# codex-storage/nim-groth16

Hardware: AMD Instinct MI355X
Metric: proofs/sec (BN254 Groth16, 2^20-constraint circuit) (higher is better)
Workload: dtype u32 (254-bit Montgomery: 8x32-bit limbs; 9x29-bit limbs in the bucket accumulation); 1 GPU; BN254 2^20-constraint synthetic R1CS (squaring chain, m=2^20-2), full prove: buildABC + 6 NTT + 4 G1 MSM + 1 G2 MSM, snarkjs flavour, 1 proof/step/GPU (3 proofs in flight per GPU, one shared key); mode=replica, nvars=1048576, domain_log2=20

## Files before the change

include/g16hip.h:

```cpp
#ifndef G16HIP_H
#define G16HIP_H

#include <stddef.h>
#include <stdint.h>

#ifdef __cplusplus
extern "C" {
#endif

#define G16_OK 0
#define G16_EINVAL (-1)
#define G16_ENODEV (-2)
#define G16_EHIP (-3)
#define G16_ENOMEM (-4)
#define G16_ESELFTEST (-5)

typedef struct g16_ctx g16_ctx;
typedef struct g16_points g16_points;

#define G16_SCALARS_MONT 1u
#define G16_SCALARS_STD 0u
#define G16_SCALARS_DEVICE 2u
#define G16_OUT_PARTIAL 4u
#define G16_OUT_DEVICE 8u
#define G16_NO_HOST_SYNC 32u

int32_t g16_ctx_create(int32_t device, g16_ctx** out);
void g16_ctx_destroy(g16_ctx* ctx);
const char* g16_last_error(const g16_ctx* ctx);
int32_t g16_ctx_set_stream(g16_ctx* ctx, void* hip_stream);
int32_t g16_ctx_synchronize(g16_ctx* ctx);
int32_t g16_ctx_cancel(g16_ctx* ctx);
int32_t g16_selftest(g16_ctx* ctx);

int32_t g16_msm_g1(g16_ctx* ctx, const void* scalars, uint32_t scalar_flags, const void* points, size_t n,
                   void* out_affine);
int32_t g16_msm_g2(g16_ctx* ctx, const void* scalars, uint32_t scalar_flags, const void* points, size_t n,
                   void* out_affine);
int32_t g16_msm_g1_dev(g16_ctx* ctx, const void* d_scalars, uint32_t scalar_flags, const void* d_points, size_t n,
                       void* out_affine);
int32_t g16_msm_g2_dev(g16_ctx* ctx, const void* d_scalars, uint32_t scalar_flags, const void* d_points, size_t n,
                       void* out_affine);
int32_t g16_msm_g1_partial_dev(g16_ctx* ctx, const void* d_scalars, uint32_t scalar_flags, const void* d_points,
                               size_t n, void* out_xyzz);
int32_t g16_msm_g2_partial_dev(g16_ctx* ctx, const void* d_scalars, uint32_t scalar_flags, const void* d_points,
                               size_t n, void* out_xyzz);
int32_t g16_g1_sum_partials(g16_ctx* ctx, const void* xyzz, size_t count, void* out_affine);
int32_t g16_g2_sum_partials(g16_ctx* ctx, const void* xyzz, size_t count, void* out_affine);

int32_t g16_points_register_g1(g16_ctx* ctx, const void* points, size_t n, g16_points** out);
int32_t g16_points_register_g2(g16_ctx* ctx, const void* points, size_t n, g16_points** out);
int32_t g16_points_register_g1_dev(g16_ctx* ctx, const void* d_points, size_t n, g16_points** out);
int32_t g16_points_register_g2_dev(g16_ctx* ctx, const void* d_points, size_t n, g16_points** out);
void g16_points_release(g16_points* pts);
size_t g16_points_count(const g16_points* pts);
size_t g16_points_inf_count(const g16_points* pts);
int32_t g16_points_info(const g16_points* pts, uint32_t* window_bits, uint32_t* ntables);

int32_t g16_points_register_g1_lean(g16_ctx* ctx, const void* points, size_t n, uint32_t table_stride, g16_points** out);
int32_t g16_points_register_g2_lean(g16_ctx* ctx, const void* points, size_t n, uint32_t table_stride, g16_points** out);
int32_t g16_points_register_g1_lean_dev(g16_ctx* ctx, const void* d_points, size_t n, uint32_t table_stride,
                                        g16_points** out);
int32_t g16_points_register_g2_lean_dev(g16_ctx* ctx, const void* d_points, size_t n, uint32_t table_stride,
                                        g16_points** out);
int32_t g16_points_table_bytes(const g16_points* pts, size_t* bytes);
int32_t g16_points_plan(int group, size_t n, uint32_t table_stride, uint32_t* window_bits, uint32_t* ntables,
                        size_t* bytes);
int32_t g16_msm_points(g16_ctx* ctx, const g16_points* pts, const void* scalars, uint32_t flags, void* out);

int32_t g16_points_check_g1(g16_ctx* ctx, const void* points, size_t n, size_t* first_bad);
int32_t g16_points_check_g2(g16_ctx* ctx, const void* points, size_t n, size_t* first_bad);

int32_t g16_fixed_base_g1(g16_ctx* ctx, const void* scalars, uint32_t scalar_flags, size_t n, void* out_points);
int32_t g16_fixed_base_g2(g16_ctx* ctx, const void* scalars, uint32_t scalar_flags, size_t n, void* out_points);

typedef struct {
  uint32_t nvars, npubs, nconstraints;
  uint32_t flavour;
  const uint32_t* row[3];
  const uint32_t* col[3];
  const void* val[3];
  size_t nnz[3];
  uint32_t flags;
  const void *alpha, *beta, *gamma, *delta, *tau;
} g16_setup_desc;
typedef struct {
  void *alpha1, *beta1, *delta1;
  void *beta2, *gamma2, *delta2;
  void* pointsIC;
  void *pointsA1, *pointsB1;
  void* pointsB2;
  void* pointsC1;
  void* pointsH1;
} g16_setup_points;
int32_t g16_setup_log2_domain(const g16_setup_desc* desc, uint32_t* log2_domain);
int32_t g16_fake_setup(g16_ctx* ctx, const g16_setup_desc* desc, g16_setup_points* out);
int32_t g16_lagrange_fr(g16_ctx* ctx, uint32_t log2n, uint32_t first, uint32_t step, size_t count, const void* tau,
                        const void* scale, void* out);
int32_t g16_powers_fr(g16_ctx* ctx, const void* base, const void* scale, size_t count, void* out);

typedef struct g16_r1cs_desc_s g16_r1cs_desc;
typedef struct g16_ptau_desc_s g16_ptau_desc;
int32_t g16_points_intt_g1(g16_ctx* ctx, const void* points, uint32_t log2n, void* out);
int32_t g16_points_intt_g2(g16_ctx* ctx, const void* points, uint32_t log2n, void* out);
int32_t g16_circuit_setup(g16_ctx* ctx, const g16_r1cs_desc* r1cs, const g16_ptau_desc* ptau, const void* delta,
                          g16_setup_points* out);

int32_t g16_ntt_fr(g16_ctx* ctx, const void* src, void* dst, uint32_t log2n, int32_t inverse);
int32_t g16_ntt_fr_dev(g16_ctx* ctx, const void* d_src, void* d_dst, uint32_t log2n, int32_t inverse);

#define G16_FLAVOUR_JENSGROTH 0u
#define G16_FLAVOUR_SNARKJS 1u
int32_t g16_quotient(g16_ctx* ctx, const void* Az, const void* Bz, const void* Cz, uint32_t log2n, uint32_t flavour,
                     void* out);
int32_t g16_quotient_dev(g16_ctx* ctx, const void* d_Az, const void* d_Bz, const void* d_Cz, uint32_t log2n,
                         uint32_t flavour, void* d_out);

typedef struct g16_pkey g16_pkey;
typedef struct {
  uint32_t matrix;
  uint32_t row;
  uint32_t col;
  uint32_t reserved;
  uint8_t value[32];
} g16_coeff;
typedef struct {
  uint32_t nvars, npubs;
  uint32_t log2_domain;
  uint32_t flavour;
  const void *pointsA1, *pointsB1;
  const void* pointsB2;
  const void* pointsC1;
  const void* pointsH1;
  const g16_coeff* coeffs;
  size_t ncoeffs;
  const void *alpha1, *beta1, *delta1;
  const void *beta2, *delta2;
  uint32_t shard_index, shard_count;
} g16_pkey_desc;
typedef struct {
  uint8_t pi_a[64];
  uint8_t pi_b[128];
  uint8_t pi_c[64];
} g16_proof;
int32_t g16_pkey_create(g16_ctx* ctx, const g16_pkey_desc* desc, g16_pkey** out);
int32_t g16_pkey_create_zkey(g16_ctx* ctx, const g16_pkey_desc* desc, const void* section4, size_t section4_bytes,
                             g16_pkey** out);
int32_t g16_pkey_create_lean(g16_ctx* ctx, const g16_pkey_desc* desc, uint32_t table_stride, g16_pkey** out);
int32_t g16_pkey_create_zkey_lean(g16_ctx* ctx, const g16_pkey_desc* desc, const void* section4, size_t section4_bytes,
                                  uint32_t table_stride, g16_pkey** out);
void g16_pkey_destroy(g16_pkey* key);
int32_t g16_pkey_inf_counts(const g16_pkey* key, size_t out[8]);
int32_t g16_pkey_b1_fold(const g16_pkey* key, size_t out[3]);
int32_t g16_pkey_b1_sparse(const g16_pkey* key, size_t out[3]);
int32_t g16_prove(g16_ctx* ctx, const g16_pkey* key, const void* witness, uint32_t flags, const void* mask_r,
                  const void* mask_s, g16_proof* out);
#define G16_PARTIALS_BYTES 768
int32_t g16_prove_partials(g16_ctx* ctx, const g16_pkey* key, const void* witness, uint32_t flags, void* out_partials);
int32_t g16_prove_combine(g16_ctx* ctx, const g16_pkey* key, const void* partials, size_t count, uint32_t flags,
                          const void* mask_r, const void* mask_s, g16_proof* out);
int32_t g16_prove_partials_begin(g16_ctx* ctx, const g16_pkey* key, const void* witness, uint32_t flags,
                                 uint32_t task_mask, void* d_task_out);
int32_t g16_prove_partials_end(g16_ctx* ctx, const g16_pkey* key, const void* d_a1_slice, const void* d_b1_slice,
                               const void* d_c1_slice, uint32_t flags, void* out_partials);
int32_t g16_build_abc(g16_ctx* ctx, const g16_pkey* key, const void* witness, uint32_t flags, void* out_abc);
int32_t g16_pkey_abc_info(const g16_pkey* key, size_t out[11]);
int32_t g16_spmv_fr(g16_ctx* ctx, const uint32_t* row, const uint32_t* col, const void* val, size_t nnz, const void* x,
                    size_t ncols, size_t nrows, void* y);

typedef struct g16_group g16_group;
typedef struct g16_group_pkey g16_group_pkey;
int32_t g16_group_create(const int32_t* devices, int32_t ndev, g16_group** out);
void g16_group_destroy(g16_group* group);
int32_t g16_group_size(const g16_group* group);
const char* g16_group_last_error(const g16_group* group);
int32_t g16_group_pkey_create(g16_group* group, const g16_pkey_desc* desc, g16_group_pkey** out);
int32_t g16_group_pkey_create_lean(g16_group* group, const g16_pkey_desc* desc, uint32_t table_stride,
                                   g16_group_pkey** out);
void g16_group_pkey_destroy(g16_group_pkey* key);
int32_t g16_group_prove(g16_group* group, const g16_group_pkey* key, const void* witness, uint32_t flags,
                        const void* mask_r, const void* mask_s, g16_proof* out);

#define G16_EBUSY (-6)
typedef struct g16_prover g16_prover;
int32_t g16_prover_create(int32_t device, const g16_pkey* key, uint32_t depth, g16_prover** out);
void g16_prover_destroy(g16_prover* p);
const char* g16_prover_last_error(const g16_prover* p);
int32_t g16_prover_submit(g16_prover* p, const void* witness, uint32_t flags, const void* mask_r, const void* mask_s,
                          uint64_t* ticket);
int32_t g16_prover_poll(g16_prover* p, uint64_t ticket);
int32_t g16_prover_collect(g16_prover* p, uint64_t ticket, g16_proof* out);
int32_t g16_host_alloc(int32_t device, size_t bytes, void** out);
void g16_host_free(void* p);

typedef struct g16_vkey g16_vkey;
typedef struct {
  uint32_t npubs;
  const void* alpha1;
  const void* beta2;
  const void* gamma2;
  const void* delta2;
  const void* pointsIC;
} g16_vkey_desc;
#define G16_VERIFY_SUBGROUP 16u
#define G16_GT_BYTES 384
int32_t g16_vkey_create(g16_ctx* ctx, const g16_vkey_desc* desc, g16_vkey** out);
void g16_vkey_destroy(g16_vkey* key);
int32_t g16_verify(g16_ctx* ctx, const g16_vkey* key, const g16_proof* proofs, const void* public_io, uint32_t flags,
                   size_t count, int32_t* status);
int32_t g16_pairing(g16_ctx* ctx, const void* g1_points, const void* g2_points, size_t n, void* out_gt);
int32_t g16_verify_batch(g16_ctx* ctx, const g16_vkey* key, const g16_proof* proofs, const void* public_io,
                         uint32_t flags, size_t count, const void* multipliers, int32_t* result, int32_t* status);

int32_t g16_points_audit_g1(g16_ctx* ctx, const void* points, size_t n, size_t first_bad[3], size_t bad_count[3]);
int32_t g16_points_audit_g2(g16_ctx* ctx, const void* points, size_t n, size_t first_bad[3], size_t bad_count[3]);
int32_t g16_points_pairs_check(g16_ctx* ctx, const void* g1_points, const void* g2_points, size_t n,
                               const void* multipliers, int32_t* result);
#define G16_AUDIT_SECTIONS 13
enum {
  G16_SEC_ALPHA1 = 0, G16_SEC_BETA1, G16_SEC_DELTA1, G16_SEC_BETA2, G16_SEC_GAMMA2, G16_SEC_DELTA2, G16_SEC_POINTS_IC,
  G16_SEC_POINTS_A1, G16_SEC_POINTS_B1, G16_SEC_POINTS_B2, G16_SEC_POINTS_C1, G16_SEC_POINTS_H1, G16_SEC_COEFFS
};
#define G16_AUDIT_CANONICAL 1u
#define G16_AUDIT_CURVE 2u
#define G16_AUDIT_SUBGROUP 4u
#define G16_AUDIT_RELATION 8u
#define G16_AUDIT_SPEC_INFINITY 16u
typedef struct {
  uint32_t failed;
  uint32_t spec_infinity;
  int32_t relation[3];
  uint32_t reserved;
  size_t first_bad[G16_AUDIT_SECTIONS][3];
  size_t bad_count[G16_AUDIT_SECTIONS][3];
} g16_key_report;
int32_t g16_key_audit(g16_ctx* ctx, const g16_pkey_desc* desc, const g16_vkey_desc* vk, const void* section4,
                      size_t section4_bytes, const void* multipliers, g16_key_report* out);

struct g16_r1cs_desc_s {
  uint32_t nvars, npubs, nconstraints;
  uint32_t flavour;
  const uint32_t* row[3];
  const uint32_t* col[3];
  const void* val[3];
  size_t nnz[3];
  uint32_t flags;
};
struct g16_ptau_desc_s {
  uint32_t power;
  const void *tauG1, *tauG2, *alphaTauG1, *betaTauG1, *betaG2;
};
#define G16_PTAU_SECTIONS 5
#define G16_CIRCUIT_RELATIONS 9
enum {
  G16_PTAU_TAU_G1 = 0, G16_PTAU_TAU_G2, G16_PTAU_ALPHA_TAU_G1, G16_PTAU_BETA_TAU_G1, G16_PTAU_BETA_G2
};
enum {
  G16_REL_COEFFS_A = 0, G16_REL_COEFFS_B, G16_REL_SPEC, G16_REL_A1, G16_REL_B1, G16_REL_B2, G16_REL_C1, G16_REL_IC,
  G16_REL_H1
};
#define G16_CIRCUIT_KEY 1u
#define G16_CIRCUIT_PTAU 2u
#define G16_CIRCUIT_COEFFS 4u
#define G16_CIRCUIT_SPEC 8u
#define G16_CIRCUIT_POINTS 16u
typedef struct {
  g16_key_report key;
  size_t ptau_first_bad[G16_PTAU_SECTIONS][3];
  size_t ptau_bad_count[G16_PTAU_SECTIONS][3];
  int32_t relation[G16_CIRCUIT_RELATIONS];
  uint32_t failed;
  size_t first_row[2];
} g16_circuit_report;
int32_t g16_circuit_audit(g16_ctx* ctx, const g16_pkey_desc* desc, const g16_vkey_desc* vk, const void* section4,
                          size_t section4_bytes, const g16_r1cs_desc* r1cs, const g16_ptau_desc* ptau,
                          const void* wire_multipliers, const void* h_multipliers, g16_circuit_report* out);

typedef struct g16_r1cs g16_r1cs;
int32_t g16_r1cs_create(g16_ctx* ctx, const g16_r1cs_desc* desc, g16_r1cs** out);
void g16_r1cs_destroy(g16_r1cs* r);
int32_t g16_r1cs_info(const g16_r1cs* r, size_t out[4]);

#define G16_WITNESS_CANONICAL 1u
#define G16_WITNESS_ONE 2u
#define G16_WITNESS_CONSTRAINTS 4u
#define G16_WITNESS_LIST 16
typedef struct {
  uint32_t failed;
  int32_t constraints;
  size_t noncanonical_count, first_noncanonical;
  size_t bad_count;
  size_t first_bad[G16_WITNESS_LIST];
  uint8_t az[32], bz[32], cz[32];
} g16_witness_report;
int32_t g16_witness_check(g16_ctx* ctx, const g16_r1cs* r, const void* witness, uint32_t flags, g16_witness_report* out);

int32_t g16_points_scale_g1(g16_ctx* ctx, const void* points, size_t n, const void* k, uint32_t flags, void* out);
int32_t g16_points_scale_g2(g16_ctx* ctx, const void* points, size_t n, const void* k, uint32_t flags, void* out);
int32_t g16_points_scale_each_g1(g16_ctx* ctx, const void* points, size_t n, const void* scalars, uint32_t flags,
                                 void* out);
int32_t g16_points_scale_each_g2(g16_ctx* ctx, const void* points, size_t n, const void* scalars, uint32_t flags,
                                 void* out);

typedef struct {
  const void *delta1, *delta2;
  const void *pointsC1, *pointsH1;
  size_t nc1, nh1;
} g16_phase2_key;
typedef struct {
  uint8_t delta_after[64];
  uint8_t g1_s[64], g1_sx[64];
  uint8_t g2_spx[128];
} g16_contribution;
typedef struct {
  void *delta1, *delta2, *pointsC1, *pointsH1;
  g16_contribution* record;
} g16_phase2_out;
int32_t g16_key_contribute(g16_ctx* ctx, const g16_phase2_key* key, const void* d, const void* s, uint32_t flags,
                           const void* challenge_g2, g16_phase2_out* out);

#define G16_CHAIN_ARRAYS 9
enum {
  G16_CHAIN_DELTA_AFTER = 0, G16_CHAIN_G1_S, G16_CHAIN_G1_SX, G16_CHAIN_G2_SPX, G16_CHAIN_CHALLENGES,
  G16_CHAIN_FINAL_DELTA1, G16_CHAIN_FINAL_DELTA2, G16_CHAIN_FINAL_POINTS_C1, G16_CHAIN_FINAL_POINTS_H1
};
#define G16_CHAIN_RELATIONS 7
enum {
  G16_CHAIN_ELEMENTS = 0, G16_CHAIN_POK, G16_CHAIN_STEP, G16_CHAIN_LAST, G16_CHAIN_DELTA, G16_CHAIN_C1, G16_CHAIN_H1
};
typedef struct {
  uint32_t failed;
  int32_t relation[G16_CHAIN_RELATIONS];
  size_t first_record[2];
  size_t first_bad[G16_CHAIN_ARRAYS][3];
  size_t bad_count[G16_CHAIN_ARRAYS][3];
  size_t first_infinity[G16_CHAIN_ARRAYS];
} g16_chain_report;
int32_t g16_contributions_verify(g16_ctx* ctx, const g16_phase2_key* initial, const g16_phase2_key* final_,
                                 const g16_contribution* records, const void* challenges_g2, size_t count,
                                 const void* c1_multipliers, const void* h1_multipliers, g16_chain_report* out);

typedef struct {
  void *tauG1, *tauG2, *alphaTauG1, *betaTauG1, *betaG2;
} g16_ptau_out;
typedef struct {
  uint8_t g1_s[64], g1_sx[64], g2_spx[128];
} g16_ptau_pok;
typedef struct {
  uint8_t tauG1[64], alphaG1[64], betaG1[64];
  uint8_t tauG2[128], betaG2[128];
  g16_ptau_pok pok[3];
} g16_ptau_contribution;
int32_t g16_ptau_contribute(g16_ctx* ctx, const g16_ptau_desc* ptau, const void* t, const void* a, const void* b,
                            const void* s3, uint32_t flags, const void* challenges_g2, g16_ptau_out* out,
                            g16_ptau_contribution* record);

#define G16_PTAU_REPORT_ARRAYS 14
enum {
  G16_PTAUV_REC_TAU_G1 = 5, G16_PTAUV_REC_ALPHA_G1, G16_PTAUV_REC_BETA_G1, G16_PTAUV_REC_TAU_G2, G16_PTAUV_REC_BETA_G2,
  G16_PTAUV_G1_S, G16_PTAUV_G1_SX, G16_PTAUV_G2_SPX, G16_PTAUV_CHALLENGES
};
#define G16_PTAU_RELATIONS 10
enum {
  G16_PTAUV_ELEMENTS = 0, G16_PTAUV_FIRST, G16_PTAUV_TAU_G1, G16_PTAUV_TAU_G2, G16_PTAUV_ALPHA, G16_PTAUV_BETA,
  G16_PTAUV_BETA_G2, G16_PTAUV_POK, G16_PTAUV_STEP, G16_PTAUV_LAST
};
typedef struct {
  uint32_t failed;
  int32_t relation[G16_PTAU_RELATIONS];
  size_t first_record[2];
  size_t first_bad[G16_PTAU_REPORT_ARRAYS][3];
  size_t bad_count[G16_PTAU_REPORT_ARRAYS][3];
  size_t first_infinity[G16_PTAU_REPORT_ARRAYS];
} g16_ptau_report;
int32_t g16_ptau_verify(g16_ctx* ctx, const g16_ptau_desc* ptau, const g16_ptau_contribution* records,
                        const void* challenges_g2, size_t count, const void* multipliers, g16_ptau_report* out);

int32_t g16_profile_enable(g16_ctx* ctx, int32_t on);
int32_t g16_profile_reset(g16_ctx* ctx);
int32_t g16_profile_report(g16_ctx* ctx, char* buf, size_t buflen);
int32_t g16_profile_clock(g16_ctx* ctx, double* ghz);

#ifdef __cplusplus
}
#endif
#endif
```

nim_groth16_amd/_lib.py:

```python
from __future__ import annotations

import ctypes
import json
import os
import weakref

_HERE = os.path.dirname(os.path.abspath(__file__))

_R = 21888242871839275222246405745257275088548364400416034343698204186575808495617
G16_OK, G16_EINVAL, G16_ENODEV, G16_EHIP, G16_ENOMEM, G16_ESELFTEST, G16_EBUSY = 0, -1, -2, -3, -4, -5, -6
SCALARS_MONT, SCALARS_STD, SCALARS_DEVICE, OUT_PARTIAL, OUT_DEVICE, NO_HOST_SYNC = 1, 0, 2, 4, 8, 32
PARTIALS_BYTES = 768

SYMBOLS = [
    "g16_ctx_create", "g16_ctx_destroy", "g16_last_error", "g16_ctx_set_stream", "g16_ctx_synchronize",
    "g16_selftest", "g16_msm_g1", "g16_msm_g2", "g16_msm_g1_dev", "g16_msm_g2_dev",
    "g16_msm_g1_partial_dev", "g16_msm_g2_partial_dev", "g16_g1_sum_partials", "g16_g2_sum_partials",
    "g16_points_register_g1", "g16_points_register_g2", "g16_points_register_g1_dev",
    "g16_points_register_g2_dev", "g16_points_release", "g16_points_count", "g16_points_inf_count", "g16_points_info", "g16_msm_points",
    "g16_points_check_g1", "g16_points_check_g2", "g16_fixed_base_g1", "g16_fixed_base_g2", "g16_quotient", "g16_quotient_dev", "g16_pkey_create",
    "g16_pkey_create_zkey", "g16_pkey_destroy", "g16_pkey_inf_counts", "g16_prove", "g16_build_abc", "g16_pkey_abc_info", "g16_spmv_fr", "g16_prove_partials", "g16_prove_combine",
    "g16_prove_partials_begin", "g16_prove_partials_end",
    "g16_ntt_fr", "g16_ntt_fr_dev", "g16_profile_enable", "g16_profile_reset", "g16_profile_report", "g16_profile_clock",
    "g16_vkey_create", "g16_vkey_destroy", "g16_verify", "g16_verify_batch", "g16_pairing",
    "g16_ctx_cancel", "g16_group_create", "g16_group_destroy", "g16_group_size", "g16_group_last_error",
    "g16_group_pkey_create", "g16_group_pkey_destroy", "g16_group_prove",
    "g16_prover_create", "g16_prover_destroy", "g16_prover_last_error", "g16_prover_submit", "g16_prover_poll",
    "g16_prover_collect", "g16_host_alloc", "g16_host_free",
    "g16_points_register_g1_lean", "g16_points_register_g2_lean", "g16_points_register_g1_lean_dev",
    "g16_points_register_g2_lean_dev", "g16_points_table_bytes", "g16_points_plan", "g16_pkey_create_lean",
    "g16_pkey_create_zkey_lean", "g16_group_pkey_create_lean",
    "g16_setup_log2_domain", "g16_fake_setup", "g16_lagrange_fr", "g16_powers_fr",
    "g16_points_audit_g1", "g16_points_audit_g2", "g16_points_pairs_check", "g16_key_audit",
    "g16_pkey_b1_fold", "g16_pkey_b1_sparse", "g16_circuit_audit",
    "g16_points_intt_g1", "g16_points_intt_g2", "g16_circuit_setup",
    "g16_points_scale_g1", "g16_points_scale_g2", "g16_points_scale_each_g1", "g16_points_scale_each_g2",
    "g16_key_contribute", "g16_contributions_verify", "g16_ptau_contribute", "g16_ptau_verify",
    "g16_r1cs_create", "g16_r1cs_destroy", "g16_r1cs_info", "g16_witness_check",
]
VERIFY_SUBGROUP = 16
GT_BYTES = 384


class PkeyDesc(ctypes.Structure):
    _fields_ = [("nvars", ctypes.c_uint32), ("npubs", ctypes.c_uint32), ("log2_domain", ctypes.c_uint32),
                ("flavour", ctypes.c_uint32),
                ("pointsA1", ctypes.c_void_p), ("pointsB1", ctypes.c_void_p), ("pointsB2", ctypes.c_void_p),
                ("pointsC1", ctypes.c_void_p), ("pointsH1", ctypes.c_void_p),
                ("coeffs", ctypes.c_void_p), ("ncoeffs", ctypes.c_size_t),
                ("alpha1", ctypes.c_void_p), ("beta1", ctypes.c_void_p), ("delta1", ctypes.c_void_p),
                ("beta2", ctypes.c_void_p), ("delta2", ctypes.c_void_p),
                ("shard_index", ctypes.c_uint32), ("shard_count", ctypes.c_uint32)]


class VkeyDesc(ctypes.Structure):
    _fields_ = [("npubs", ctypes.c_uint32), ("alpha1", ctypes.c_void_p), ("beta2", ctypes.c_void_p),
                ("gamma2", ctypes.c_void_p), ("delta2", ctypes.c_void_p), ("pointsIC", ctypes.c_void_p)]


class SetupDesc(ctypes.Structure):
    _fields_ = [("nvars", ctypes.c_uint32), ("npubs", ctypes.c_uint32), ("nconstraints", ctypes.c_uint32),
                ("flavour", ctypes.c_uint32),
                ("row", ctypes.c_void_p * 3), ("col", ctypes.c_void_p * 3), ("val", ctypes.c_void_p * 3),
                ("nnz", ctypes.c_size_t * 3), ("flags", ctypes.c_uint32),
                ("alpha", ctypes.c_void_p), ("beta", ctypes.c_void_p), ("gamma", ctypes.c_void_p),
                ("delta", ctypes.c_void_p), ("tau", ctypes.c_void_p)]


SETUP_POINTS = ("alpha1", "beta1", "delta1", "beta2", "gamma2", "delta2", "pointsIC", "pointsA1", "pointsB1", "pointsB2",
                "pointsC1", "pointsH1")


class SetupPoints(ctypes.Structure):
    _fields_ = [(name, ctypes.c_void_p) for name in SETUP_POINTS]


AUDIT_SECTIONS = ("alpha1", "beta1", "delta1", "beta2", "gamma2", "delta2", "pointsIC", "pointsA1", "pointsB1", "pointsB2",
                  "pointsC1", "pointsH1", "coeffs")
AUDIT_CHECKS = ("canonical", "curve", "subgroup")
AUDIT_RELATIONS = ("pointsB1~pointsB2", "beta1~beta2", "delta1~delta2")
AUDIT_CANONICAL, AUDIT_CURVE, AUDIT_SUBGROUP, AUDIT_RELATION, AUDIT_SPEC_INFINITY = 1, 2, 4, 8, 16
CHECK_TEXTS = ("is not a canonical encoding", "is not on the curve", "is not in the order-r subgroup")


def _element_findings(names, first_bad, bad_count, first_infinity=None, prefix=""):
    out = []
    for a, name in enumerate(names):
        for k, what in enumerate(CHECK_TEXTS):
            if bad_count[a][k]:
                more = bad_count[a][k] - 1
                out.append(f"{prefix}{name}[{first_bad[a][k]}] {what}" + (f" (and {more} more)" if more else ""))
        if first_infinity is not None and first_infinity[a] is not None:
            out.append(f"{prefix}{name}[{first_infinity[a]}] is the point at infinity")
    return out


class KeyReportC(ctypes.Structure):
    _fields_ = [("failed", ctypes.c_uint32), ("spec_infinity", ctypes.c_uint32), ("relation", ctypes.c_int32 * 3),
                ("reserved", ctypes.c_uint32),
                ("first_bad", (ctypes.c_size_t * 3) * len(AUDIT_SECTIONS)),
                ("bad_count", (ctypes.c_size_t * 3) * len(AUDIT_SECTIONS))]


class KeyReport:

    def __init__(self, failed, spec_infinity, relation, first_bad, bad_count):
        self.failed, self.spec_infinity, self.relation = failed, spec_infinity, list(relation)
        self.first_bad, self.bad_count = first_bad, bad_count

    @property
    def ok(self) -> bool:
        return self.failed == 0

    def as_dict(self) -> dict:
        return {"failed": self.failed, "spec_infinity": self.spec_infinity, "relation": self.relation,
                "first_bad": self.first_bad, "bad_count": self.bad_count}

    def findings(self):
        out = _element_findings(AUDIT_SECTIONS, self.first_bad, self.bad_count)
        for k, name in enumerate(AUDIT_RELATIONS):
            if self.relation[k] == 0:
                out.append(f"{name}: not the same multiples of the two generators")
        for s in range(6):
            if self.spec_infinity >> s & 1:
                out.append(f"{AUDIT_SECTIONS[s]} is the point at infinity")
        return out

    def __str__(self):
        if self.ok:
            skipped = [AUDIT_RELATIONS[k] for k in range(3) if self.relation[k] < 0]
            return "key audit: ok" + (f" (not run: {', '.join(skipped)})" if skipped else "")
        return "key audit: FAILED\n" + "\n".join("  " + f for f in self.findings())


class R1csDesc(ctypes.Structure):
    _fields_ = [("nvars", ctypes.c_uint32), ("npubs", ctypes.c_uint32), ("nconstraints", ctypes.c_uint32),
                ("flavour", ctypes.c_uint32),
                ("row", ctypes.c_void_p * 3), ("col", ctypes.c_void_p * 3), ("val", ctypes.c_void_p * 3),
                ("nnz", ctypes.c_size_t * 3), ("flags", ctypes.c_uint32)]


class PtauDesc(ctypes.Structure):
    _fields_ = [("power", ctypes.c_uint32), ("tauG1", ctypes.c_void_p), ("tauG2", ctypes.c_void_p),
                ("alphaTauG1", ctypes.c_void_p), ("betaTauG1", ctypes.c_void_p), ("betaG2", ctypes.c_void_p)]


PTAU_SECTIONS = ("tauG1", "tauG2", "alphaTauG1", "betaTauG1", "betaG2")
PTAU_GROUP = {"tauG1": 1, "tauG2": 2, "alphaTauG1": 1, "betaTauG1": 1, "betaG2": 2}
CIRCUIT_RELATIONS = ("COEFFS_A", "COEFFS_B", "SPEC", "A1", "B1", "B2", "C1", "IC", "H1")
CIRCUIT_KEY, CIRCUIT_PTAU, CIRCUIT_COEFFS, CIRCUIT_SPEC, CIRCUIT_POINTS = 1, 2, 4, 8, 16


class CircuitReportC(ctypes.Structure):
    _fields_ = [("key", KeyReportC),
                ("ptau_first_bad", (ctypes.c_size_t * 3) * len(PTAU_SECTIONS)),
                ("ptau_bad_count", (ctypes.c_size_t * 3) * len(PTAU_SECTIONS)),
                ("relation", ctypes.c_int32 * len(CIRCUIT_RELATIONS)), ("failed", ctypes.c_uint32),
                ("first_row", ctypes.c_size_t * 2)]


class CircuitReport:

    def __init__(self, key: KeyReport, ptau_first_bad, ptau_bad_count, relation, failed, first_row):
        self.key, self.ptau_first_bad, self.ptau_bad_count = key, ptau_first_bad, ptau_bad_count
        self.relation, self.failed, self.first_row = list(relation), failed, list(first_row)

    @property
    def ok(self) -> bool:
        return self.failed == 0

    def as_dict(self) -> dict:
        return {"key": self.key.as_dict(), "ptau_first_bad": self.ptau_first_bad, "ptau_bad_count": self.ptau_bad_count,
                "relation": self.relation, "failed": self.failed, "first_row": self.first_row}

    def findings(self):
        out = self.key.findings() + _element_findings(PTAU_SECTIONS, self.ptau_first_bad, self.ptau_bad_count, prefix="ptau ")
        for m in range(2):
            if self.relation[m] == 0:
                out.append(f"coeffs: matrix {'AB'[m]} differs from the r1cs first at row {self.first_row[m]}")
        if self.relation[2] == 0:
            out.append("alpha1 / beta1 / beta2 are not those of the powers of tau (or its first powers are not the generators)")
        for k in range(3, len(CIRCUIT_RELATIONS)):
            if self.relation[k] == 0:
                out.append(f"points{CIRCUIT_RELATIONS[k]} does not belong to the circuit")
        return out

    def __str__(self):
        if self.ok:
            skipped = [AUDIT_RELATIONS[k] for k in range(3) if self.key.relation[k] < 0]
            skipped += [CIRCUIT_RELATIONS[k] for k in range(len(CIRCUIT_RELATIONS)) if self.relation[k] < 0]
            return "circuit audit: ok" + (f" (not run: {', '.join(skipped)})" if skipped else "")
        return "circuit audit: FAILED\n" + "\n".join("  " + f for f in self.findings())


WITNESS_CANONICAL, WITNESS_ONE, WITNESS_CONSTRAINTS = 1, 2, 4
WITNESS_LIST = 16


class WitnessReportC(ctypes.Structure):
    _fields_ = [("failed", ctypes.c_uint32), ("constraints", ctypes.c_int32),
                ("noncanonical_count", ctypes.c_size_t), ("first_noncanonical", ctypes.c_size_t),
                ("bad_count", ctypes.c_size_t), ("first_bad", ctypes.c_size_t * WITNESS_LIST),
                ("az", ctypes.c_uint8 * 32), ("bz", ctypes.c_uint8 * 32), ("cz", ctypes.c_uint8 * 32)]


class WitnessReport:

    def __init__(self, failed, constraints, noncanonical_count, first_noncanonical, bad_count, first_bad, az, bz, cz):
        self.failed, self.constraints = failed, constraints
        self.noncanonical_count, self.first_noncanonical = noncanonical_count, first_noncanonical
        self.bad_count, self.first_bad = bad_count, list(first_bad)
        self.az, self.bz, self.cz = az, bz, cz

    @property
    def ok(self) -> bool:
        return self.failed == 0

    def as_dict(self) -> dict:
        return {"failed": self.failed, "constraints": self.constraints, "noncanonical_count": self.noncanonical_count,
                "first_noncanonical": self.first_noncanonical, "bad_count": self.bad_count, "first_bad": self.first_bad,
                "az": self.az, "bz": self.bz, "cz": self.cz}

    def findings(self):
        out = []
        if self.noncanonical_count:
            more = self.noncanonical_count - 1
            out.append(f"witness[{self.first_noncanonical}] is not canonical (>= r)" + (f" (and {more} more)" if more else ""))
        if self.failed & WITNESS_ONE:
            out.append("witness[0] is not 1")
        if self.bad_count:
            ab = self.az * self.bz % _R
            out.append(f"constraint {self.first_bad[0]}: (A z)(B z) = {ab:#x}, C z = {self.cz:#x}")
            rest = self.first_bad[1:]
            if rest:
                more = self.bad_count - len(self.first_bad)
                out.append("also failing: constraints " + ", ".join(map(str, rest)) + (f" (and {more} more)" if more else ""))
        return out

    def __str__(self):
        if self.ok:
            return "witness check: ok"
        return "witness check: FAILED\n" + "\n".join("  " + f for f in self.findings())


class Phase2Key(ctypes.Structure):
    _fields_ = [("delta1", ctypes.c_void_p), ("delta2", ctypes.c_void_p), ("pointsC1", ctypes.c_void_p),
                ("pointsH1", ctypes.c_void_p), ("nc1", ctypes.c_size_t), ("nh1", ctypes.c_size_t)]


class ContributionC(ctypes.Structure):
    _fields_ = [("delta_after", ctypes.c_uint8 * 64), ("g1_s", ctypes.c_uint8 * 64), ("g1_sx", ctypes.c_uint8 * 64),
                ("g2_spx", ctypes.c_uint8 * 128)]


CONTRIBUTION_BYTES = 320
assert ctypes.sizeof(ContributionC) == CONTRIBUTION_BYTES


class Phase2Out(ctypes.Structure):
    _fields_ = [("delta1", ctypes.c_void_p), ("delta2", ctypes.c_void_p), ("pointsC1", ctypes.c_void_p),
                ("pointsH1", ctypes.c_void_p), ("record", ctypes.POINTER(ContributionC))]


class PtauOut(ctypes.Structure):
    _fields_ = [(name, ctypes.c_void_p) for name in PTAU_SECTIONS]


class PtauPokC(ctypes.Structure):
    _fields_ = [("g1_s", ctypes.c_uint8 * 64), ("g1_sx", ctypes.c_uint8 * 64), ("g2_spx", ctypes.c_uint8 * 128)]


class PtauContributionC(ctypes.Structure):
    _fields_ = [("tauG1", ctypes.c_uint8 * 64), ("alphaG1", ctypes.c_uint8 * 64), ("betaG1", ctypes.c_uint8 * 64),
                ("tauG2", ctypes.c_uint8 * 128), ("betaG2", ctypes.c_uint8 * 128), ("pok", PtauPokC * 3)]


PTAU_CONTRIBUTION_BYTES = 1216
assert ctypes.sizeof(PtauContributionC) == PTAU_CONTRIBUTION_BYTES


PTAU_REPORT_ARRAYS = PTAU_SECTIONS + ("record tauG1", "record alphaG1", "record betaG1", "record tauG2", "record betaG2",
                                      "g1_s", "g1_sx", "g2_spx", "challenges")
PTAU_RELATIONS = ("ELEMENTS", "FIRST", "TAU_G1", "TAU_G2", "ALPHA", "BETA", "BETA_G2", "POK", "STEP", "LAST")


class PtauReportC(ctypes.Structure):
    _fields_ = [("failed", ctypes.c_uint32), ("relation", ctypes.c_int32 * len(PTAU_RELATIONS)),
                ("first_record", ctypes.c_size_t * 2),
                ("first_bad", (ctypes.c_size_t * 3) * len(PTAU_REPORT_ARRAYS)),
                ("bad_count", (ctypes.c_size_t * 3) * len(PTAU_REPORT_ARRAYS)),
                ("first_infinity", ctypes.c_size_t * len(PTAU_REPORT_ARRAYS))]


class PtauReport:

    def __init__(self, failed, relation, first_record, first_bad, bad_count, first_infinity):
        self.failed, self.relation, self.first_record = failed, list(relation), list(first_record)
        self.first_bad, self.bad_count, self.first_infinity = first_bad, bad_count, list(first_infinity)

    @property
    def ok(self) -> bool:
        return self.failed == 0

    def as_dict(self) -> dict:
        return {"failed": self.failed, "relation": self.relation, "first_record": self.first_record,
                "first_bad": self.first_bad, "bad_count": self.bad_count, "first_infinity": self.first_infinity}

    def findings(self):
        out = _element_findings(PTAU_REPORT_ARRAYS, self.first_bad, self.bad_count, self.first_infinity)
        for k, name in enumerate(PTAU_RELATIONS):
            if k and self.relation[k] == 0:
                rec = f" (first at record {self.first_record[k - 7]})" if name in ("POK", "STEP") else ""
                out.append(f"{name} fails{rec}")
        return out

    def __str__(self):
        rel = "  ".join(f"{n} {'ok' if v == 1 else 'FAILS' if v == 0 else 'not run'}" for n, v in zip(PTAU_RELATIONS, self.relation))
        return rel + "".join("\n  " + f for f in self.findings())


CHAIN_ARRAYS = ("delta_after", "g1_s", "g1_sx", "g2_spx", "challenges", "final delta1", "final delta2", "final pointsC1",
                "final pointsH1")
CHAIN_RELATIONS = ("ELEMENTS", "POK", "STEP", "LAST", "DELTA", "C1", "H1")


class ChainReportC(ctypes.Structure):
    _fields_ = [("failed", ctypes.c_uint32), ("relation", ctypes.c_int32 * len(CHAIN_RELATIONS)),
                ("first_record", ctypes.c_size_t * 2),
                ("first_bad", (ctypes.c_size_t * 3) * len(CHAIN_ARRAYS)),
                ("bad_count", (ctypes.c_size_t * 3) * len(CHAIN_ARRAYS)),
                ("first_infinity", ctypes.c_size_t * len(CHAIN_ARRAYS))]


class ChainReport:

    def __init__(self, failed, relation, first_record, first_bad, bad_count, first_infinity, transcript=None):
        self.failed, self.relation, self.first_record = failed, list(relation), list(first_record)
        self.first_bad, self.bad_count, self.first_infinity = first_bad, bad_count, list(first_infinity)
        self.transcript = transcript

    @property
    def ok(self) -> bool:
        return self.failed == 0 and self.transcript != 0

    def as_dict(self) -> dict:
        return {"failed": self.failed, "relation": self.relation, "first_record": self.first_record,
                "first_bad": self.first_bad, "bad_count": self.bad_count, "first_infinity": self.first_infinity,
                "transcript": self.transcript}

    def findings(self):
        out = []
        if self.transcript == 0:
            out.append("the transcript hashes are not those of the initial key and the records")
        out += _element_findings(CHAIN_ARRAYS, self.first_bad, self.bad_count, self.first_infinity)
        if self.relation[1] == 0:
            out.append(f"record {self.first_record[0]}: the proof of knowledge does not hold")
        if self.relation[2] == 0:
            out.append(f"record {self.first_record[1]}: delta_after is not the contribution's multiple of the delta before")
        if self.relation[3] == 0:
            out.append("the final delta1 is not the last record's delta_after")
        if self.relation[4] == 0:
            out.append("the final delta1 / delta2 are not the same multiple of the two generators")
        for k in (5, 6):
            if self.relation[k] == 0:
                out.append(f"the final points{CHAIN_RELATIONS[k]} is not the initial one rescaled by the deltas")
        return out

    def __str__(self):
        if self.ok:
            skipped = [CHAIN_RELATIONS[k] for k in range(len(CHAIN_RELATIONS)) if self.relation[k] < 0]
            return "contribution chain: ok" + (f" (not run: {', '.join(skipped)})" if skipped else "")
        return "contribution chain: FAILED\n" + "\n".join("  " + f for f in self.findings())


class G16Error(RuntimeError):
    def __init__(self, code, msg):
        super().__init__(f"g16hip error {code}: {msg}")
        self.code = code


def lib_path() -> str:
    return os.environ.get("G16HIP_LIB", os.path.join(_HERE, "csrc", "libg16hip.so"))


def device_code_sha16(path: str = None) -> str:
    import hashlib
    import struct
    b = open(path or lib_path(), "rb").read()
    h = hashlib.sha256()
    try:
        assert b[:4] == b"\x7fELF" and b[4] == 2
        shoff = struct.unpack_from("<Q", b, 0x28)[0]
        shentsize, shnum, shstrndx = struct.unpack_from("<HHH", b, 0x3A)

        def sh(i):
            name, _typ, _flags, _addr, off, size = struct.unpack_from("<IIQQQQ", b, shoff + i * shentsize)
            return name, off, size
        _, stro, _ = sh(shstrndx)
        hit = False
        for i in range(shnum):
            n, off, size = sh(i)
            if b[stro + n: b.index(b"\0", stro + n)] == b".hip_fatbin":
                h.update(b[off: off + size])
                hit = True
        assert hit
    except Exception:
        h = hashlib.sha256(b)
    return h.hexdigest()[:16]


_lib = None


def load_library():
    global _lib
    if _lib is not None:
        return _lib
    path = lib_path()
    if not os.path.exists(path):
        raise G16Error(G16_ENODEV, f"{path} not found: build it with `make -C nim_groth16_amd/csrc` "
                                   "(or __graft_entry__.build()); there is no CPU fallback")
    try:
        import torch
    except ImportError:
        pass
    lib = ctypes.CDLL(path)
    vp, u32, i32, sz = ctypes.c_void_p, ctypes.c_uint32, ctypes.c_int32, ctypes.c_size_t
    lib.g16_ctx_create.argtypes = [i32, ctypes.POINTER(vp)]
    lib.g16_ctx_destroy.argtypes = [vp]
    lib.g16_ctx_destroy.restype = None
    lib.g16_last_error.argtypes = [vp]
    lib.g16_last_error.restype = ctypes.c_char_p
    lib.g16_ctx_set_stream.argtypes = [vp, vp]
    lib.g16_ctx_synchronize.argtypes = [vp]
    lib.g16_selftest.argtypes = [vp]
    for name in ("g16_msm_g1", "g16_msm_g2", "g16_msm_g1_dev", "g16_msm_g2_dev",
                 "g16_msm_g1_partial_dev", "g16_msm_g2_partial_dev"):
        getattr(lib, name).argtypes = [vp, vp, u32, vp, sz, vp]
    for name in ("g16_g1_sum_partials", "g16_g2_sum_partials"):
        getattr(lib, name).argtypes = [vp, vp, sz, vp]
    for name in ("g16_points_register_g1", "g16_points_register_g2", "g16_points_register_g1_dev",
                 "g16_points_register_g2_dev"):
        getattr(lib, name).argtypes = [vp, vp, sz, ctypes.POINTER(vp)]
    for name in ("g16_points_register_g1_lean", "g16_points_register_g2_lean", "g16_points_register_g1_lean_dev",
                 "g16_points_register_g2_lean_dev"):
        getattr(lib, name).argtypes = [vp, vp, sz, u32, ctypes.POINTER(vp)]
    lib.g16_points_table_bytes.argtypes = [vp, ctypes.POINTER(sz)]
    lib.g16_points_plan.argtypes = [ctypes.c_int, sz, u32, ctypes.POINTER(u32), ctypes.POINTER(u32), ctypes.POINTER(sz)]
    lib.g16_pkey_create_lean.argtypes = [vp, ctypes.POINTER(PkeyDesc), u32, ctypes.POINTER(vp)]
    lib.g16_pkey_create_zkey_lean.argtypes = [vp, ctypes.POINTER(PkeyDesc), vp, sz, u32, ctypes.POINTER(vp)]
    lib.g16_group_pkey_create_lean.argtypes = [vp, ctypes.POINTER(PkeyDesc), u32, ctypes.POINTER(vp)]
    lib.g16_points_release.argtypes = [vp]
    lib.g16_points_release.restype = None
    lib.g16_points_count.argtypes = [vp]
    lib.g16_points_count.restype = sz
    lib.g16_points_inf_count.argtypes = [vp]
    lib.g16_points_inf_count.restype = sz
    lib.g16_pkey_inf_counts.argtypes = [vp, ctypes.POINTER(sz)]
    lib.g16_pkey_b1_fold.argtypes = [vp, ctypes.POINTER(sz)]
    lib.g16_pkey_b1_sparse.argtypes = [vp, ctypes.POINTER(sz)]
    lib.g16_points_info.argtypes = [vp, ctypes.POINTER(u32), ctypes.POINTER(u32)]
    lib.g16_msm_points.argtypes = [vp, vp, vp, u32, vp]
    lib.g16_points_check_g1.argtypes = [vp, vp, sz, ctypes.POINTER(sz)]
    lib.g16_points_check_g2.argtypes = [vp, vp, sz, ctypes.POINTER(sz)]
    lib.g16_fixed_base_g1.argtypes = [vp, vp, u32, sz, vp]
    lib.g16_fixed_base_g2.argtypes = [vp, vp, u32, sz, vp]
    lib.g16_quotient.argtypes = [vp, vp, vp, vp, u32, u32, vp]
    lib.g16_quotient_dev.argtypes = [vp, vp, vp, vp, u32, u32, vp]
    lib.g16_pkey_create.argtypes = [vp, ctypes.POINTER(PkeyDesc), ctypes.POINTER(vp)]
    lib.g16_pkey_create_zkey.argtypes = [vp, ctypes.POINTER(PkeyDesc), vp, sz, ctypes.POINTER(vp)]
    lib.g16_pkey_destroy.argtypes = [vp]
    lib.g16_pkey_destroy.restype = None
    lib.g16_prove.argtypes = [vp, vp, vp, u32, vp, vp, vp]
    lib.g16_build_abc.argtypes = [vp, vp, vp, u32, vp]
    lib.g16_pkey_abc_info.argtypes = [vp, ctypes.POINTER(sz)]
    lib.g16_spmv_fr.argtypes = [vp, vp, vp, vp, sz, vp, sz, sz, vp]
    lib.g16_prove_partials.argtypes = [vp, vp, vp, u32, vp]
    lib.g16_prove_combine.argtypes = [vp, vp, vp, sz, u32, vp, vp, vp]
    lib.g16_prove_partials_begin.argtypes = [vp, vp, vp, u32, u32, vp]
    lib.g16_prove_partials_end.argtypes = [vp, vp, vp, vp, vp, u32, vp]
    lib.g16_ntt_fr.argtypes = [vp, vp, vp, u32, i32]
    lib.g16_ntt_fr_dev.argtypes = [vp, vp, vp, u32, i32]
    lib.g16_vkey_create.argtypes = [vp, ctypes.POINTER(VkeyDesc), ctypes.POINTER(vp)]
    lib.g16_vkey_destroy.argtypes = [vp]
    lib.g16_vkey_destroy.restype = None
    lib.g16_verify.argtypes = [vp, vp, vp, vp, u32, sz, ctypes.POINTER(i32)]
    lib.g16_verify_batch.argtypes = [vp, vp, vp, vp, u32, sz, vp, ctypes.POINTER(i32), ctypes.POINTER(i32)]
    lib.g16_pairing.argtypes = [vp, vp, vp, sz, vp]
    lib.g16_ctx_cancel.argtypes = [vp]
    lib.g16_group_create.argtypes = [ctypes.POINTER(i32), i32, ctypes.POINTER(vp)]
    lib.g16_group_destroy.argtypes = [vp]
    lib.g16_group_destroy.restype = None
    lib.g16_group_size.argtypes = [vp]
    lib.g16_group_last_error.argtypes = [vp]
    lib.g16_group_last_error.restype = ctypes.c_char_p
    lib.g16_group_pkey_create.argtypes = [vp, ctypes.POINTER(PkeyDesc), ctypes.POINTER(vp)]
    lib.g16_group_pkey_destroy.argtypes = [vp]
    lib.g16_group_pkey_destroy.restype = None
    lib.g16_group_prove.argtypes = [vp, vp, vp, u32, vp, vp, vp]
    lib.g16_prover_create.argtypes = [i32, vp, u32, ctypes.POINTER(vp)]
    lib.g16_prover_destroy.argtypes = [vp]
    lib.g16_prover_destroy.restype = None
    lib.g16_prover_last_error.argtypes = [vp]
    lib.g16_prover_last_error.restype = ctypes.c_char_p
    lib.g16_prover_submit.argtypes = [vp, vp, u32, vp, vp, ctypes.POINTER(ctypes.c_uint64)]
    lib.g16_prover_poll.argtypes = [vp, ctypes.c_uint64]
    lib.g16_prover_collect.argtypes = [vp, ctypes.c_uint64, vp]
    lib.g16_host_alloc.argtypes = [i32, sz, ctypes.POINTER(vp)]
    lib.g16_host_free.argtypes = [vp]
    lib.g16_host_free.restype = None
    lib.g16_profile_enable.argtypes = [vp, i32]
    lib.g16_profile_reset.argtypes = [vp]
    lib.g16_profile_report.argtypes = [vp, ctypes.c_char_p, sz]
    lib.g16_profile_clock.argtypes = [vp, ctypes.POINTER(ctypes.c_double)]
    lib.g16_setup_log2_domain.argtypes = [ctypes.POINTER(SetupDesc), ctypes.POINTER(u32)]
    lib.g16_fake_setup.argtypes = [vp, ctypes.POINTER(SetupDesc), ctypes.POINTER(SetupPoints)]
    lib.g16_lagrange_fr.argtypes = [vp, u32, u32, u32, sz, vp, vp, vp]
    lib.g16_powers_fr.argtypes = [vp, vp, vp, sz, vp]
    lib.g16_points_audit_g1.argtypes = [vp, vp, sz, ctypes.POINTER(sz), ctypes.POINTER(sz)]
    lib.g16_points_audit_g2.argtypes = [vp, vp, sz, ctypes.POINTER(sz), ctypes.POINTER(sz)]
    lib.g16_points_pairs_check.argtypes = [vp, vp, vp, sz, vp, ctypes.POINTER(i32)]
    lib.g16_key_audit.argtypes = [vp, ctypes.POINTER(PkeyDesc), ctypes.POINTER(VkeyDesc), vp, sz, vp,
                                  ctypes.POINTER(KeyReportC)]
    lib.g16_circuit_audit.argtypes = [vp, ctypes.POINTER(PkeyDesc), ctypes.POINTER(VkeyDesc), vp, sz,
                                      ctypes.POINTER(R1csDesc), ctypes.POINTER(PtauDesc), vp, vp,
                                      ctypes.POINTER(CircuitReportC)]
    lib.g16_points_intt_g1.argtypes = [vp, vp, u32, vp]
    lib.g16_points_intt_g2.argtypes = [vp, vp, u32, vp]
    lib.g16_circuit_setup.argtypes = [vp, ctypes.POINTER(R1csDesc), ctypes.POINTER(PtauDesc), vp,
                                      ctypes.POINTER(SetupPoints)]
    lib.g16_points_scale_g1.argtypes = [vp, vp, sz, vp, u32, vp]
    lib.g16_points_scale_g2.argtypes = [vp, vp, sz, vp, u32, vp]
    lib.g16_points_scale_each_g1.argtypes = [vp, vp, sz, vp, u32, vp]
    lib.g16_points_scale_each_g2.argtypes = [vp, vp, sz, vp, u32, vp]
    lib.g16_key_contribute.argtypes = [vp, ctypes.POINTER(Phase2Key), vp, vp, u32, vp, ctypes.POINTER(Phase2Out)]
    lib.g16_contributions_verify.argtypes = [vp, ctypes.POINTER(Phase2Key), ctypes.POINTER(Phase2Key),
                                             ctypes.POINTER(ContributionC), vp, sz, vp, vp, ctypes.POINTER(ChainReportC)]
    lib.g16_ptau_contribute.argtypes = [vp, ctypes.POINTER(PtauDesc), vp, vp, vp, vp, u32, vp, ctypes.POINTER(PtauOut),
                                        ctypes.POINTER(PtauContributionC)]
    lib.g16_ptau_verify.argtypes = [vp, ctypes.POINTER(PtauDesc), ctypes.POINTER(PtauContributionC), vp, sz, vp,
                                    ctypes.POINTER(PtauReportC)]
    lib.g16_r1cs_create.argtypes = [vp, ctypes.POINTER(R1csDesc), ctypes.POINTER(vp)]
    lib.g16_r1cs_destroy.argtypes = [vp]
    lib.g16_r1cs_destroy.restype = None
    lib.g16_r1cs_info.argtypes = [vp, ctypes.POINTER(sz)]
    lib.g16_witness_check.argtypes = [vp, vp, vp, u32, ctypes.POINTER(WitnessReportC)]
    for name in SYMBOLS:
        if name not in ("g16_ctx_destroy", "g16_r1cs_destroy", "g16_last_error", "g16_points_release", "g16_points_count",
                        "g16_points_inf_count",
                        "g16_pkey_destroy", "g16_vkey_destroy", "g16_group_destroy", "g16_group_last_error",
                        "g16_group_pkey_destroy", "g16_prover_destroy", "g16_prover_last_error", "g16_host_free"):
            getattr(lib, name).restype = i32
    _lib = lib
    return lib


def _buf(b):
    if isinstance(b, int):
        return ctypes.c_void_p(b)
    if isinstance(b, (bytes, bytearray)):
        return ctypes.cast(ctypes.c_char_p(bytes(b)), ctypes.c_void_p) if isinstance(b, bytes) else \
            ctypes.cast((ctypes.c_char * len(b)).from_buffer(b), ctypes.c_void_p)
    if hasattr(b, "ctypes"):
        return ctypes.c_void_p(b.ctypes.data)
    raise TypeError(type(b))


class Context:

    def __init__(self, device: int = 0):
        self._lib = load_library()
        h = ctypes.c_void_p()
        rc = self._lib.g16_ctx_create(device, ctypes.byref(h))
        if rc != G16_OK:
            raise G16Error(rc, "g16_ctx_create failed (no usable HIP device?)")
        self._h = h
        self.device = device
        self._children = weakref.WeakSet()

    def close(self, release_children: bool = False):
        if getattr(self, "_h", None):
            if release_children:
                for child in list(self._children):
                    child._free()
            self._lib.g16_ctx_destroy(self._h)
            self._h = None

    def __del__(self):
        try:
            self.close()
        except Exception:
            pass

    def _check(self, rc):
        if rc != G16_OK:
            raise G16Error(rc, self._lib.g16_last_error(self._h).decode())

    def selftest(self):
        self._check(self._lib.g16_selftest(self._h))

    def set_stream(self, stream_ptr):
        self._check(self._lib.g16_ctx_set_stream(self._h, ctypes.c_void_p(stream_ptr)))

    def synchronize(self):
        self._check(self._lib.g16_ctx_synchronize(self._h))

    def cancel(self):
        self._check(self._lib.g16_ctx_cancel(self._h))

    def msm(self, group: int, scalars, points, n: int, mont: bool = True, device: bool = False,
            partial: bool = False) -> bytes:
        psz = 64 if group == 1 else 128
        out = ctypes.create_string_buffer(2 * psz if partial else psz)
        if partial:
            fn = self._lib.g16_msm_g1_partial_dev if group == 1 else self._lib.g16_msm_g2_partial_dev
        elif device:
            fn = self._lib.g16_msm_g1_dev if group == 1 else self._lib.g16_msm_g2_dev
        else:
            fn = self._lib.g16_msm_g1 if group == 1 else self._lib.g16_msm_g2
        s = _buf(scalars) if n else None
        p = _buf(points) if n else None
        self._check(fn(self._h, s, SCALARS_MONT if mont else SCALARS_STD, p, n, out))
        return out.raw

    def register_points(self, group: int, points, n: int, device: bool = False, table_stride: int = 0) -> "PointSet":
        h = ctypes.c_void_p()
        p = _buf(points) if n else None
        if table_stride:
            name = f"g16_points_register_g{group}_lean" + ("_dev" if device else "")
            self._check(getattr(self._lib, name)(self._h, p, n, table_stride, ctypes.byref(h)))
        else:
            name = f"g16_points_register_g{group}" + ("_dev" if device else "")
            self._check(getattr(self._lib, name)(self._h, p, n, ctypes.byref(h)))
        return PointSet(self, h, group, n)

    def msm_points(self, pts: "PointSet", scalars, mont: bool = True, device: bool = False,
                   partial: bool = False) -> bytes:
        psz = 64 if pts.group == 1 else 128
        out = ctypes.create_string_buffer(2 * psz if partial else psz)
        flags = (SCALARS_MONT if mont else 0) | (SCALARS_DEVICE if device else 0) | (OUT_PARTIAL if partial else 0)
        self._check(self._lib.g16_msm_points(self._h, pts._h, _buf(scalars) if pts.n else None, flags, out))
        return out.raw

    def points_check(self, group: int, points: bytes):
        psz = 64 if group == 1 else 128
        n = len(points) // psz
        bad = ctypes.c_size_t()
        fn = self._lib.g16_points_check_g1 if group == 1 else self._lib.g16_points_check_g2
        self._check(fn(self._h, _buf(points) if n else None, n, ctypes.byref(bad)))
        return None if bad.value == ctypes.c_size_t(-1).value else bad.value

    def points_audit(self, group: int, points: bytes):
        psz = 64 if group == 1 else 128
        assert len(points) % psz == 0
        n = len(points) // psz
        first, count = (ctypes.c_size_t * 3)(), (ctypes.c_size_t * 3)()
        fn = self._lib.g16_points_audit_g1 if group == 1 else self._lib.g16_points_audit_g2
        self._check(fn(self._h, _buf(points) if n else None, n, first, count))
        none = ctypes.c_size_t(-1).value
        return [None if f == none else f for f in first], list(count)

    def pairs_check(self, g1_points: bytes, g2_points: bytes, multipliers) -> bool:
        n = len(g1_points) // 64
        assert len(g1_points) == 64 * n and len(g2_points) == 128 * n and len(multipliers) == n
        zs = b"".join(int(z).to_bytes(16, "little") for z in multipliers)
        res = ctypes.c_int32(-1)
        self._check(self._lib.g16_points_pairs_check(self._h, _buf(g1_points) if n else None,
                                                     _buf(g2_points) if n else None, n, _buf(zs) if n else None,
                                                     ctypes.byref(res)))
        return res.value == 1

    def key_audit(self, desc: PkeyDesc, vk: VkeyDesc = None, section4: bytes = None, multipliers=None) -> KeyReport:
        zs = None
        if isinstance(multipliers, (bytes, bytearray)):
            assert len(multipliers) == 16 * desc.nvars, "one multiplier per wire"
            zs = bytes(multipliers)
        elif multipliers is not None:
            assert len(multipliers) == desc.nvars, "one multiplier per wire"
            zs = b"".join(int(z).to_bytes(16, "little") for z in multipliers)
        rep = KeyReportC()
        self._check(self._lib.g16_key_audit(self._h, ctypes.byref(desc), ctypes.byref(vk) if vk is not None else None,
                                            _buf(section4) if section4 is not None else None,
                                            len(section4) if section4 is not None else 0,
                                            _buf(zs) if zs is not None else None, ctypes.byref(rep)))
        none = ctypes.c_size_t(-1).value
        return KeyReport(rep.failed, rep.spec_infinity, list(rep.relation),
                         [[None if f == none else f for f in row] for row in rep.first_bad],
                         [list(row) for row in rep.bad_count])

    def circuit_audit(self, desc: PkeyDesc, vk, section4, r1cs: R1csDesc, ptau: PtauDesc, wire_multipliers,
                      h_multipliers) -> CircuitReport:
        def enc(zs, n, what):
            if isinstance(zs, (bytes, bytearray)):
                assert len(zs) == 16 * n, f"one {what} multiplier of 16 bytes each"
                return bytes(zs)
            assert len(zs) == n, f"{n} {what} multipliers"
            return b"".join(int(z).to_bytes(16, "little") for z in zs)
        zw = enc(wire_multipliers, desc.nvars, "wire")
        zh = enc(h_multipliers, 1 << min(desc.log2_domain, 28), "h")
        rep = CircuitReportC()
        self._check(self._lib.g16_circuit_audit(self._h, ctypes.byref(desc), ctypes.byref(vk) if vk is not None else None,
                                                _buf(section4) if section4 is not None else None,
                                                len(section4) if section4 is not None else 0,
                                                ctypes.byref(r1cs), ctypes.byref(ptau), _buf(zw), _buf(zh),
                                                ctypes.byref(rep)))
        none = ctypes.c_size_t(-1).value
        fix = lambda rows: [[None if f == none else f for f in row] for row in rows]
        key = KeyReport(rep.key.failed, rep.key.spec_infinity, list(rep.key.relation), fix(rep.key.first_bad),
                        [list(row) for row in rep.key.bad_count])
        return CircuitReport(key, fix(rep.ptau_first_bad), [list(row) for row in rep.ptau_bad_count], list(rep.relation),
                             rep.failed, [None if f == none else f for f in rep.first_row])

    def r1cs_load(self, desc: R1csDesc, keepalive=None) -> "R1csSystem":
        return R1csSystem(self, desc, keepalive)

    def fixed_base(self, group: int, scalars: bytes, mont: bool = True) -> bytes:
        n = len(scalars) // 32
        psz = 64 if group == 1 else 128
        out = ctypes.create_string_buffer(max(n, 1) * psz)
        fn = self._lib.g16_fixed_base_g1 if group == 1 else self._lib.g16_fixed_base_g2
        self._check(fn(self._h, _buf(scalars) if n else None, SCALARS_MONT if mont else 0, n, out))
        return out.raw[: n * psz]

    def spmv(self, row, col, val, x: bytes, nrows: int) -> bytes:
        import numpy as np
        row = np.ascontiguousarray(row, dtype=np.uint32)
        col = np.ascontiguousarray(col, dtype=np.uint32)
        nnz = len(row)
        if not isinstance(val, (bytes, bytearray)):
            val = np.ascontiguousarray(val, dtype=np.uint8)
        assert len(col) == nnz and (len(val) if isinstance(val, (bytes, bytearray)) else val.size) == 32 * nnz
        out = ctypes.create_string_buffer(max(1, 32 * nrows))
        self._check(self._lib.g16_spmv_fr(self._h, _buf(row) if nnz else None, _buf(col) if nnz else None,
                                          _buf(val) if nnz else None, nnz, _buf(x) if len(x) else None, len(x) // 32,
                                          nrows, out))
        return out.raw[: 32 * nrows]

    def lagrange(self, log2n: int, tau: bytes, first: int = 0, step: int = 1, count: int = None,
                 scale: bytes = None) -> bytes:
        if count is None:
            count = ((1 << log2n) - first + step - 1) // step if step else 1
        out = ctypes.create_string_buffer(max(1, 32 * count))
        self._check(self._lib.g16_lagrange_fr(self._h, log2n, first, step, count, _buf(tau),
                                              _buf(scale) if scale is not None else None, out))
        return out.raw[: 32 * count]

    def powers(self, base: bytes, count: int, scale: bytes = None) -> bytes:
        out = ctypes.create_string_buffer(max(1, 32 * count))
        self._check(self._lib.g16_powers_fr(self._h, _buf(base), _buf(scale) if scale is not None else None, count, out))
        return out.raw[: 32 * count]

    def fake_setup(self, nvars: int, npubs: int, nconstraints: int, flavour: int, matrices, toxic, mont: bool = True):
        import numpy as np
        d = SetupDesc()
        d.nvars, d.npubs, d.nconstraints, d.flavour = nvars, npubs, nconstraints, flavour
        d.flags = SCALARS_MONT if mont else SCALARS_STD
        keep = []
        for k, (rows, wires, vals) in enumerate(matrices):
            rows = np.ascontiguousarray(rows, dtype=np.uint32)
            wires = np.ascontiguousarray(wires, dtype=np.uint32)
            if not isinstance(vals, (bytes, bytearray)):
                vals = np.ascontiguousarray(vals, dtype=np.uint8)
            nnz = len(rows)
            assert len(wires) == nnz and (len(vals) if isinstance(vals, (bytes, bytearray)) else vals.size) == 32 * nnz
            keep += [rows, wires, vals]
            d.nnz[k] = nnz
            if nnz:
                d.row[k], d.col[k], d.val[k] = (_buf(x).value for x in (rows, wires, vals))
        toxic = [bytes(t) for t in toxic]
        d.alpha, d.beta, d.gamma, d.delta, d.tau = (_buf(t).value for t in toxic)
        log2 = ctypes.c_uint32()
        rc = self._lib.g16_setup_log2_domain(ctypes.byref(d), ctypes.byref(log2))
        if rc != G16_OK:
            raise G16Error(rc, "g16_setup_log2_domain failed")
        sizes = dict(alpha1=64, beta1=64, delta1=64, beta2=128, gamma2=128, delta2=128, pointsIC=64 * (npubs + 1),
                     pointsA1=64 * nvars, pointsB1=64 * nvars, pointsB2=128 * nvars,
                     pointsC1=64 * max(0, nvars - npubs - 1), pointsH1=64 << min(log2.value, 40))
        if log2.value + (1 if flavour == 1 else 0) > 28:
            sizes = dict.fromkeys(sizes, 0)
        o = SetupPoints()
        bufs = {}
        for name, nbytes in sizes.items():
            bufs[name] = ctypes.create_string_buffer(max(1, nbytes))
            setattr(o, name, ctypes.cast(bufs[name], ctypes.c_void_p).value)
        self._check(self._lib.g16_fake_setup(self._h, ctypes.byref(d), ctypes.byref(o)))
        return log2.value, {name: bufs[name].raw[: sizes[name]] for name in SETUP_POINTS}

    def points_intt(self, group: int, points: bytes, log2n: int) -> bytes:
        psz = 64 if group == 1 else 128
        assert len(points) == psz << log2n, f"2^{log2n} points of {psz} bytes"
        out = ctypes.create_string_buffer(len(points))
        fn = self._lib.g16_points_intt_g1 if group == 1 else self._lib.g16_points_intt_g2
        self._check(fn(self._h, _buf(points), log2n, out))
        return out.raw

    def circuit_setup(self, r1cs: R1csDesc, ptau: PtauDesc, delta: bytes = None):
        nvars, npubs = r1cs.nvars, r1cs.npubs
        log2 = max(0, (r1cs.nconstraints + npubs).bit_length())
        sizes = dict(alpha1=64, beta1=64, delta1=64, beta2=128, gamma2=128, delta2=128, pointsIC=64 * (npubs + 1),
                     pointsA1=64 * nvars, pointsB1=64 * nvars, pointsB2=128 * nvars,
                     pointsC1=64 * max(0, nvars - npubs - 1), pointsH1=64 << log2)
        if log2 > 24:
            sizes = dict.fromkeys(sizes, 0)
        o = SetupPoints()
        bufs = {}
        for name, nbytes in sizes.items():
            bufs[name] = ctypes.create_string_buffer(max(1, nbytes))
            setattr(o, name, ctypes.cast(bufs[name], ctypes.c_void_p).value)
        self._check(self._lib.g16_circuit_setup(self._h, ctypes.byref(r1cs), ctypes.byref(ptau),
                                                _buf(bytes(delta)) if delta is not None else None, ctypes.byref(o)))
        return log2, {name: bufs[name].raw[: sizes[name]] for name in SETUP_POINTS}

    def points_scale(self, group: int, points: bytes, k: bytes, mont: bool = True) -> bytes:
        psz = 64 if group == 1 else 128
        assert len(points) % psz == 0 and len(k) == 32, f"points of {psz} bytes and a 32-byte scalar"
        out = ctypes.create_string_buffer(max(1, len(points)))
        fn = self._lib.g16_points_scale_g1 if group == 1 else self._lib.g16_points_scale_g2
        self._check(fn(self._h, _buf(bytes(points)), len(points) // psz, _buf(bytes(k)),
                       SCALARS_MONT if mont else SCALARS_STD, out))
        return out.raw[: len(points)]

    def points_scale_each(self, group: int, points: bytes, scalars: bytes, mont: bool = True) -> bytes:
        psz = 64 if group == 1 else 128
        assert len(points) % psz == 0 and len(scalars) == 32 * (len(points) // psz), \
            f"points of {psz} bytes and one 32-byte scalar for each"
        out = ctypes.create_string_buffer(max(1, len(points)))
        fn = self._lib.g16_points_scale_each_g1 if group == 1 else self._lib.g16_points_scale_each_g2
        self._check(fn(self._h, _buf(bytes(points)), len(points) // psz, _buf(bytes(scalars)),
                       SCALARS_MONT if mont else SCALARS_STD, out))
        return out.raw[: len(points)]

    @staticmethod
    def _phase2_key(key: dict):
        assert len(key["delta1"]) == 64 and len(key["delta2"]) == 128, "delta1: 64 bytes, delta2: 128 bytes"
        assert len(key["pointsC1"]) % 64 == 0 and len(key["pointsH1"]) % 64 == 0, "G1 points of 64 bytes"
        keep = {name: bytes(key[name]) for name in ("delta1", "delta2", "pointsC1", "pointsH1")}
        pk = Phase2Key()
        for name, b in keep.items():
            setattr(pk, name, ctypes.cast(ctypes.c_char_p(b), ctypes.c_void_p).value if b else None)
        pk.nc1, pk.nh1 = len(keep["pointsC1"]) // 64, len(keep["pointsH1"]) // 64
        return pk, keep

    def key_contribute(self, key: dict, d: bytes, s: bytes, challenge_g2: bytes, mont: bool = True):
        assert len(d) == 32 and len(s) == 32 and len(challenge_g2) == 128
        pk, keep = self._phase2_key(key)
        bufs = {name: ctypes.create_string_buffer(max(1, len(b))) for name, b in keep.items()}
        rec = ContributionC()
        o = Phase2Out()
        for name in bufs:
            setattr(o, name, ctypes.cast(bufs[name], ctypes.c_void_p).value)
        o.record = ctypes.pointer(rec)
        self._check(self._lib.g16_key_contribute(self._h, ctypes.byref(pk), _buf(bytes(d)), _buf(bytes(s)),
                                                 SCALARS_MONT if mont else SCALARS_STD, _buf(bytes(challenge_g2)),
                                                 ctypes.byref(o)))
        return {name: bufs[name].raw[: len(keep[name])] for name in keep}, bytes(rec)

    def ptau_contribute(self, ptau: dict, t: bytes, a: bytes, b: bytes, s3: bytes, challenges_g2: bytes, mont: bool = True,
                        power: int = None):
        assert len(t) == len(a) == len(b) == 32 and len(s3) == 96 and len(challenges_g2) == 384
        keep = {name: bytes(ptau[name]) for name in PTAU_SECTIONS}
        if power is None:
            power = max(0, (len(keep["tauG2"]) // 128).bit_length() - 1)
            assert [len(keep[n]) for n in PTAU_SECTIONS] == [64 * ((2 << power) - 1), 128 << power, 64 << power,
                                                             64 << power, 128], "not the arrays of one power"
        desc = PtauDesc(power, *[ctypes.cast(ctypes.c_char_p(keep[n]), ctypes.c_void_p) if keep[n] else None
                                 for n in PTAU_SECTIONS])
        bufs = {name: ctypes.create_string_buffer(max(1, len(v))) for name, v in keep.items()}
        o = PtauOut(*[ctypes.cast(bufs[n], ctypes.c_void_p) for n in PTAU_SECTIONS])
        rec = PtauContributionC()
        self._check(self._lib.g16_ptau_contribute(self._h, ctypes.byref(desc), _buf(bytes(t)), _buf(bytes(a)), _buf(bytes(b)),
                                                  _buf(bytes(s3)), SCALARS_MONT if mont else SCALARS_STD,
                                                  _buf(bytes(challenges_g2)), ctypes.byref(o), ctypes.byref(rec)))
        return {name: bufs[name].raw[: len(keep[name])] for name in PTAU_SECTIONS}, bytes(rec)

    def ptau_verify(self, ptau: dict, records, challenges_g2, multipliers, power: int = None) -> PtauReport:
        keep = {name: bytes(ptau[name]) for name in PTAU_SECTIONS}
        if power is None:
            power = max(0, (len(keep["tauG2"]) // 128).bit_length() - 1)
            assert [len(keep[n]) for n in PTAU_SECTIONS] == [64 * ((2 << power) - 1), 128 << power, 64 << power,
                                                             64 << power, 128], "not the arrays of one power"
        desc = PtauDesc(power, *[ctypes.cast(ctypes.c_char_p(keep[n]), ctypes.c_void_p) for n in PTAU_SECTIONS])
        m = (2 << power) - 2
        if isinstance(multipliers, (bytes, bytearray)):
            zs = bytes(multipliers)
        else:
            zs = b"".join(int(z).to_bytes(16, "little") for z in multipliers)
        assert len(zs) == 16 * m or not 1 <= power <= 25, f"{m} multipliers of 16 bytes each"
        recs, ch, count = None, None, 0
        if records is not None:
            count = len(records)
            assert all(len(r) == PTAU_CONTRIBUTION_BYTES for r in records)
            recs = (PtauContributionC * max(1, count)).from_buffer_copy(b"".join(records) or bytes(PTAU_CONTRIBUTION_BYTES))
            ch = b"".join(challenges_g2)
            assert len(ch) == 384 * count, "three 128-byte challenge points per record"
        rep = PtauReportC()
        self._check(self._lib.g16_ptau_verify(self._h, ctypes.byref(desc), recs, _buf(ch) if ch else None, count, _buf(zs),
                                              ctypes.byref(rep)))
        none = ctypes.c_size_t(-1).value
        opt = lambda row: [None if f == none else f for f in row]
        return PtauReport(rep.failed, list(rep.relation), opt(rep.first_record), [opt(row) for row in rep.first_bad],
                          [list(row) for row in rep.bad_count], opt(rep.first_infinity))

    def contributions_verify(self, initial: dict, final: dict, records, challenges_g2, c1_multipliers,
                             h1_multipliers) -> ChainReport:
        def enc(zs, n, what):
            if isinstance(zs, (bytes, bytearray)):
                assert len(zs) == 16 * n, f"one {what} multiplier of 16 bytes each"
                return bytes(zs)
            assert len(zs) == n, f"{n} {what} multipliers"
            return b"".join(int(z).to_bytes(16, "little") for z in zs)
        records, challenges_g2 = list(records), list(challenges_g2)
        assert len(records) == len(challenges_g2) and all(len(r) == CONTRIBUTION_BYTES for r in records) and \
            all(len(c) == 128 for c in challenges_g2), "one 320-byte record and one 128-byte challenge per contribution"
        ki, keep_i = self._phase2_key(initial)
        kf, keep_f = self._phase2_key(final)
        zc, zh = enc(c1_multipliers, kf.nc1, "c1"), enc(h1_multipliers, kf.nh1, "h1")
        recs = (ContributionC * max(1, len(records))).from_buffer_copy(b"".join(records) or bytes(CONTRIBUTION_BYTES))
        ch = b"".join(challenges_g2)
        rep = ChainReportC()
        self._check(self._lib.g16_contributions_verify(self._h, ctypes.byref(ki), ctypes.byref(kf), recs,
                                                       _buf(ch) if ch else None, len(records),
                                                       _buf(zc) if zc else None, _buf(zh) if zh else None,
                                                       ctypes.byref(rep)))
        none = ctypes.c_size_t(-1).value
        opt = lambda row: [None if f == none else f for f in row]
        return ChainReport(rep.failed, list(rep.relation), opt(rep.first_record), [opt(row) for row in rep.first_bad],
                           [list(row) for row in rep.bad_count], opt(rep.first_infinity))

    def quotient(self, Az, Bz, Cz, log2n: int, flavour: int, out=None, device: bool = False):
        if device:
            self._check(self._lib.g16_quotient_dev(self._h, _buf(Az), _buf(Bz), _buf(Cz), log2n, flavour, _buf(out)))
            return None
        res = ctypes.create_string_buffer(32 << log2n)
        self._check(self._lib.g16_quotient(self._h, _buf(Az), _buf(Bz), _buf(Cz), log2n, flavour, res))
        return res.raw

    def sum_partials(self, group: int, xyzz: bytes, count: int) -> bytes:
        psz = 64 if group == 1 else 128
        out = ctypes.create_string_buffer(psz)
        fn = self._lib.g16_g1_sum_partials if group == 1 else self._lib.g16_g2_sum_partials
        self._check(fn(self._h, _buf(xyzz) if count else None, count, out))
        return out.raw

    def ntt(self, src, log2n: int, inverse: bool, dst=None, device: bool = False):
        n = 1 << log2n
        if device:
            self._check(self._lib.g16_ntt_fr_dev(self._h, _buf(src), _buf(dst), log2n, 1 if inverse else 0))
            return None
        out = ctypes.create_string_buffer(32 * n)
        self._check(self._lib.g16_ntt_fr(self._h, _buf(src), out, log2n, 1 if inverse else 0))
        return out.raw

    def pairing(self, g1_points: bytes, g2_points: bytes) -> bytes:
        n = len(g1_points) // 64
        assert len(g1_points) == 64 * n and len(g2_points) == 128 * n
        out = ctypes.create_string_buffer(max(1, GT_BYTES * n))
        self._check(self._lib.g16_pairing(self._h, _buf(g1_points) if n else None, _buf(g2_points) if n else None,
                                          n, out))
        return out.raw[:GT_BYTES * n]

    def profile(self, on):
        self._check(self._lib.g16_profile_enable(self._h, int(on)))

    def profile_reset(self):
        self._check(self._lib.g16_profile_reset(self._h))

    def profile_clock(self) -> float:
        g = ctypes.c_double()
        self._check(self._lib.g16_profile_clock(self._h, ctypes.byref(g)))
        return g.value

    def profile_report(self) -> dict:
        buf = ctypes.create_string_buffer(1 << 16)
        self._check(self._lib.g16_profile_report(self._h, buf, len(buf)))
        return json.loads(buf.value.decode())


class ProvingKey:

    def __init__(self, ctx: Context, desc: PkeyDesc, keepalive, section4: bytes = None, table_stride: int = 0):
        self.ctx = ctx
        h = ctypes.c_void_p()
        if table_stride and section4 is not None:
            ctx._check(ctx._lib.g16_pkey_create_zkey_lean(ctx._h, ctypes.byref(desc), _buf(section4), len(section4),
                                                          table_stride, ctypes.byref(h)))
        elif table_stride:
            ctx._check(ctx._lib.g16_pkey_create_lean(ctx._h, ctypes.byref(desc), table_stride, ctypes.byref(h)))
        elif section4 is not None:
            ctx._check(ctx._lib.g16_pkey_create_zkey(ctx._h, ctypes.byref(desc), _buf(section4), len(section4),
                                                     ctypes.byref(h)))
        else:
            ctx._check(ctx._lib.g16_pkey_create(ctx._h, ctypes.byref(desc), ctypes.byref(h)))
        self._h = h
        self.nvars, self.npubs, self.log2n = desc.nvars, desc.npubs, desc.log2_domain
        ctx._children.add(self)
        del keepalive

    def _check_len(self, witness):
        if isinstance(witness, (bytes, bytearray)) and len(witness) != 32 * self.nvars:
            raise ValueError(f"wrong witness length: {len(witness)} bytes, expected {32 * self.nvars}")

    def prove(self, witness, mont: bool = True, r: bytes = None, s: bytes = None, device: bool = False, ctx=None):
        c = ctx or self.ctx
        self._check_len(witness)
        out = ctypes.create_string_buffer(256)
        flags = (SCALARS_MONT if mont else 0) | (SCALARS_DEVICE if device else 0)
        c._check(c._lib.g16_prove(c._h, self._h, _buf(witness), flags, _buf(r) if r else None,
                                  _buf(s) if s else None, out))
        raw = out.raw
        return raw[0:64], raw[64:192], raw[192:256]

    def prove_partials(self, witness, mont: bool = True, device: bool = False, out=None, ctx=None):
        c = ctx or self.ctx
        self._check_len(witness)
        flags = (SCALARS_MONT if mont else 0) | (SCALARS_DEVICE if device else 0)
        if out is not None:
            c._check(c._lib.g16_prove_partials(c._h, self._h, _buf(witness), flags | OUT_DEVICE, _buf(out)))
            return None
        buf = ctypes.create_string_buffer(PARTIALS_BYTES)
        c._check(c._lib.g16_prove_partials(c._h, self._h, _buf(witness), flags, buf))
        return buf.raw

    def prove_partials_begin(self, witness, task_mask: int, task_out=None, mont: bool = True, device: bool = False,
                             ctx=None, nosync: bool = False):
        c = ctx or self.ctx
        self._check_len(witness)
        flags = (SCALARS_MONT if mont else 0) | (SCALARS_DEVICE if device else 0) | (NO_HOST_SYNC if nosync else 0)
        c._check(c._lib.g16_prove_partials_begin(c._h, self._h, _buf(witness), flags, task_mask,
                                                 _buf(task_out) if task_out is not None else None))

    def prove_partials_end(self, a1, b1, c1, out=None, ctx=None, nosync: bool = False):
        c = ctx or self.ctx
        ptr = lambda x: _buf(x) if x is not None else None
        if out is not None:
            c._check(c._lib.g16_prove_partials_end(c._h, self._h, ptr(a1), ptr(b1), ptr(c1),
                                                   OUT_DEVICE | (NO_HOST_SYNC if nosync else 0), _buf(out)))
            return None
        buf = ctypes.create_string_buffer(PARTIALS_BYTES)
        c._check(c._lib.g16_prove_partials_end(c._h, self._h, ptr(a1), ptr(b1), ptr(c1), 0, buf))
        return buf.raw

    def prove_combine(self, partials, count: int, r: bytes = None, s: bytes = None, device: bool = False, ctx=None):
        c = ctx or self.ctx
        out = ctypes.create_string_buffer(256)
        c._check(c._lib.g16_prove_combine(c._h, self._h, _buf(partials), count, SCALARS_DEVICE if device else 0,
                                          _buf(r) if r else None, _buf(s) if s else None, out))
        raw = out.raw
        return raw[0:64], raw[64:192], raw[192:256]

    def inf_counts(self) -> dict:
        out = (ctypes.c_size_t * 8)()
        self.ctx._check(self.ctx._lib.g16_pkey_inf_counts(self._h, out))
        v = list(out)
        return {"A1": v[0], "B1": v[1], "B2": v[2], "C1": v[3], "H1": v[4], "B1_and_B2": v[5],
                "compact_A": bool(v[6]), "compact_B": bool(v[7])}

    def b1_fold(self) -> dict:
        out = (ctypes.c_size_t * 3)()
        self.ctx._check(self.ctx._lib.g16_pkey_b1_fold(self._h, out))
        return {"form": ("PLAIN", "EMPTY", "DELTA")[out[0]], "live_b1": out[1], "live_delta": out[2]}

    def b1_sparse(self) -> dict:
        out = (ctypes.c_size_t * 3)()
        self.ctx._check(self.ctx._lib.g16_pkey_b1_sparse(self._h, out))
        return {"sparse": bool(out[0]), "live": out[1], "max": out[2]}

    def abc_info(self) -> dict:
        out = (ctypes.c_size_t * 11)()
        self.ctx._check(self.ctx._lib.g16_pkey_abc_info(self._h, out))
        v = list(out)
        names = ("L<=1", "L=2", "L<=4", "L<=8", "L<=16", "L<=32", "L<=64", "L<=128", "L>128")
        return {"ncoeffs": v[0], "dict_values": v[1], "rows_by_terms": dict(zip(names, v[2:]))}

    def build_abc(self, witness: bytes, mont: bool = True, ctx=None):
        c = ctx or self.ctx
        self._check_len(witness)
        n = 1 << self.log2n
        out = ctypes.create_string_buffer(3 * n * 32)
        c._check(c._lib.g16_build_abc(c._h, self._h, _buf(witness), SCALARS_MONT if mont else 0, out))
        raw = out.raw
        return raw[: 32 * n], raw[32 * n: 64 * n], raw[64 * n:]

    def _free(self):
        if self._h:
            self.ctx._lib.g16_pkey_destroy(self._h)
        self._h = None

    destroy = _free

    def __del__(self):
        try:
            self._free()
        except Exception:
            pass


class R1csSystem:

    def __init__(self, ctx: Context, desc: R1csDesc, keepalive=None):
        self.ctx = ctx
        self._h = None
        h = ctypes.c_void_p()
        ctx._check(ctx._lib.g16_r1cs_create(ctx._h, ctypes.byref(desc), ctypes.byref(h)))
        self._h = h
        self.nvars, self.nconstraints = desc.nvars, desc.nconstraints
        ctx._children.add(self)
        del keepalive

    def info(self) -> dict:
        out = (ctypes.c_size_t * 4)()
        self.ctx._check(self.ctx._lib.g16_r1cs_info(self._h, out))
        return {"nvars": out[0], "nconstraints": out[1], "nnz": out[2], "dict_values": out[3]}

    def check(self, witness, mont: bool = True, device: bool = False, ctx=None) -> WitnessReport:
        c = ctx or self.ctx
        if isinstance(witness, (bytes, bytearray)) and len(witness) != 32 * self.nvars:
            raise ValueError(f"wrong witness length: {len(witness)} bytes, expected {32 * self.nvars}")
        rep = WitnessReportC()
        flags = (SCALARS_MONT if mont else 0) | (SCALARS_DEVICE if device else 0)
        c._check(c._lib.g16_witness_check(c._h, self._h, _buf(witness), flags, ctypes.byref(rep)))
        none = ctypes.c_size_t(-1).value
        le = lambda a: int.from_bytes(bytes(a), "little")
        return WitnessReport(rep.failed, rep.constraints, rep.noncanonical_count,
                             None if rep.first_noncanonical == none else rep.first_noncanonical, rep.bad_count,
                             [f for f in rep.first_bad if f != none], le(rep.az), le(rep.bz), le(rep.cz))

    def _free(self):
        if self._h:
            self.ctx._lib.g16_r1cs_destroy(self._h)
        self._h = None

    destroy = _free

    def __del__(self):
        try:
            self._free()
        except Exception:
            pass


class DeviceGroup:

    def __init__(self, devices):
        self._lib = load_library()
        arr = (ctypes.c_int32 * len(devices))(*devices)
        h = ctypes.c_void_p()
        rc = self._lib.g16_group_create(arr, len(devices), ctypes.byref(h))
        if rc != G16_OK:
            raise G16Error(rc, "g16_group_create failed")
        self._h, self.devices = h, list(devices)

    def _check(self, rc):
        if rc != G16_OK:
            raise G16Error(rc, self._lib.g16_group_last_error(self._h).decode())

    def size(self) -> int:
        return self._lib.g16_group_size(self._h)

    def load_key(self, desc: PkeyDesc, keepalive=None, table_stride: int = 0) -> "GroupKey":
        h = ctypes.c_void_p()
        if table_stride:
            self._check(self._lib.g16_group_pkey_create_lean(self._h, ctypes.byref(desc), table_stride, ctypes.byref(h)))
        else:
            self._check(self._lib.g16_group_pkey_create(self._h, ctypes.byref(desc), ctypes.byref(h)))
        return GroupKey(self, h, desc.nvars)

    def close(self):
        if getattr(self, "_h", None):
            self._lib.g16_group_destroy(self._h)
            self._h = None

    def __del__(self):
        try:
            self.close()
        except Exception:
            pass


class GroupKey:
    def __init__(self, group: DeviceGroup, handle, nvars: int):
        self.group, self._h, self.nvars = group, handle, nvars

    def prove(self, witness: bytes, mont: bool = True, r: bytes = None, s: bytes = None):
        if len(witness) != 32 * self.nvars:
            raise ValueError(f"wrong witness length: {len(witness)} bytes, expected {32 * self.nvars}")
        out = ctypes.create_string_buffer(256)
        g = self.group
        g._check(g._lib.g16_group_prove(g._h, self._h, _buf(witness), SCALARS_MONT if mont else 0,
                                        _buf(r) if r else None, _buf(s) if s else None, out))
        raw = out.raw
        return raw[0:64], raw[64:192], raw[192:256]

    def destroy(self):
        if self._h:
            self.group._lib.g16_group_pkey_destroy(self._h)
        self._h = None

    def __del__(self):
        try:
            self.destroy()
        except Exception:
            pass


class ProverPool:

    def __init__(self, pkey: ProvingKey, depth: int = 3, device: int = 0):
        self._lib = load_library()
        self.pkey, self.depth, self.device = pkey, depth, device
        h = ctypes.c_void_p()
        rc = self._lib.g16_prover_create(device, pkey._h, depth, ctypes.byref(h))
        if rc != G16_OK:
            raise G16Error(rc, "g16_prover_create failed (sharded key, key of another device, or depth not in 1..8)")
        self._h = h
        self._witness = {}

    def _check(self, rc):
        if rc == G16_EBUSY:
            raise G16Error(rc, f"{self.depth + 1} proofs outstanding: collect one first")
        if rc < 0:
            raise G16Error(rc, self._lib.g16_prover_last_error(self._h).decode())
        return rc

    def submit(self, witness, mont: bool = True, r: bytes = None, s: bytes = None, device: bool = False) -> int:
        self.pkey._check_len(witness)
        if isinstance(witness, HostBuffer) and witness.nbytes < 32 * self.pkey.nvars:
            raise ValueError("host buffer shorter than the witness")
        ptr = ctypes.c_void_p(witness.data_ptr()) if device and hasattr(witness, "data_ptr") else _buf(witness)
        t = ctypes.c_uint64()
        flags = (SCALARS_MONT if mont else 0) | (SCALARS_DEVICE if device else 0)
        self._check(self._lib.g16_prover_submit(self._h, ptr, flags, _buf(r) if r else None,
                                                _buf(s) if s else None, ctypes.byref(t)))
        self._witness[t.value] = witness
        return t.value

    def poll(self, ticket: int) -> bool:
        return self._check(self._lib.g16_prover_poll(self._h, ticket)) == 1

    def collect(self, ticket: int):
        out = ctypes.create_string_buffer(256)
        self._check(self._lib.g16_prover_collect(self._h, ticket, out))
        self._witness.pop(ticket, None)
        raw = out.raw
        return raw[0:64], raw[64:192], raw[192:256]

    def close(self):
        if getattr(self, "_h", None):
            self._lib.g16_prover_destroy(self._h)
            self._h = None
            self._witness.clear()

    def __del__(self):
        try:
            self.close()
        except Exception:
            pass


class HostBuffer:

    def __init__(self, nbytes: int, device: int = 0):
        import numpy as np
        self._lib = load_library()
        p = ctypes.c_void_p()
        rc = self._lib.g16_host_alloc(device, nbytes, ctypes.byref(p))
        if rc != G16_OK:
            raise G16Error(rc, "g16_host_alloc failed")
        self._p, self.nbytes = p, nbytes
        self.array = np.ctypeslib.as_array((ctypes.c_uint8 * nbytes).from_address(p.value))
        self.ctypes = self.array.ctypes

    @classmethod
    def from_bytes(cls, data: bytes, device: int = 0) -> "HostBuffer":
        import numpy as np
        b = cls(len(data), device)
        b.array[:] = np.frombuffer(data, dtype=np.uint8)
        return b

    def __len__(self):
        return self.nbytes

    def free(self):
        if getattr(self, "_p", None):
            self.array = self.ctypes = None
            self._lib.g16_host_free(self._p)
            self._p = None

    def __del__(self):
        try:
            self.free()
        except Exception:
            pass


class VerifyingKey:

    def __init__(self, ctx: Context, npubs: int, alpha1: bytes, beta2: bytes, gamma2: bytes, delta2: bytes,
                 pointsIC: bytes):
        assert len(alpha1) == 64 and len(beta2) == len(gamma2) == len(delta2) == 128
        assert len(pointsIC) == 64 * (npubs + 1), "pointsIC must hold npubs + 1 points"
        self.ctx, self.npubs = ctx, npubs
        bufs = [ctypes.create_string_buffer(x, len(x)) for x in (alpha1, beta2, gamma2, delta2, pointsIC)]
        a = [ctypes.cast(b, ctypes.c_void_p) for b in bufs]
        desc = VkeyDesc(npubs, a[0], a[1], a[2], a[3], a[4])
        h = ctypes.c_void_p()
        ctx._check(ctx._lib.g16_vkey_create(ctx._h, ctypes.byref(desc), ctypes.byref(h)))
        self._h = h
        ctx._children.add(self)

    def verify(self, proofs, public_io: bytes, mont: bool = True, subgroup: bool = False):
        n = len(proofs)
        assert len(public_io) == 32 * n * (self.npubs + 1)
        raw = b"".join(a + b + c for a, b, c in proofs)
        assert len(raw) == 256 * n
        st = (ctypes.c_int32 * max(n, 1))()
        flags = (SCALARS_MONT if mont else 0) | (VERIFY_SUBGROUP if subgroup else 0)
        self.ctx._check(self.ctx._lib.g16_verify(self.ctx._h, self._h, _buf(raw) if n else None,
                                                 _buf(public_io) if n else None, flags, n, st))
        return list(st)[:n]

    def verify_batch(self, proofs, public_io: bytes, mont: bool = True, multipliers=None, want_status: bool = False):
        n = len(proofs)
        assert len(public_io) == 32 * n * (self.npubs + 1)
        raw = b"".join(a + b + c for a, b, c in proofs)
        assert len(raw) == 256 * n
        if multipliers is None:
            import secrets
            multipliers = [secrets.randbelow((1 << 128) - 1) + 1 for _ in range(n)]
        assert len(multipliers) == n, "one multiplier per proof"
        zs = b"".join(int(z).to_bytes(16, "little") for z in multipliers)
        res = ctypes.c_int32(-1)
        st = (ctypes.c_int32 * max(n, 1))() if want_status else None
        flags = SCALARS_MONT if mont else 0
        self.ctx._check(self.ctx._lib.g16_verify_batch(self.ctx._h, self._h, _buf(raw) if n else None,
                                                       _buf(public_io) if n else None, flags, n,
                                                       _buf(zs) if n else None, ctypes.byref(res), st))
        return (res.value == 1, list(st)[:n]) if want_status else res.value == 1

    def _free(self):
        if self._h:
            self.ctx._lib.g16_vkey_destroy(self._h)
        self._h = None

    destroy = _free

    def __del__(self):
        try:
            self._free()
        except Exception:
            pass


def points_plan(group: int, n: int, table_stride: int = 0):
    lib = load_library()
    c, t, b = ctypes.c_uint32(), ctypes.c_uint32(), ctypes.c_size_t()
    rc = lib.g16_points_plan(group, n, table_stride, ctypes.byref(c), ctypes.byref(t), ctypes.byref(b))
    if rc != G16_OK:
        raise G16Error(rc, "g16_points_plan: bad group, or too many points for 31-bit entry indices")
    return c.value, t.value, b.value


class PointSet:

    def __init__(self, ctx: Context, handle, group: int, n: int):
# ... 40 lines not shown
```

nim_groth16_amd/csrc/g16_env.hpp:

```cpp
#pragma once

struct G16Env {
  int msm_window = 0;
  int table_window = 0;
  int msm_seg = 0;
  char msm_sort = 0;
  int g1_lanes[3] = {3, 2, 0};
  char stream_prio[7] = "lhllln";
  int red_slice_log2 = 0;
  int inf_compact_pct = 10;
  int r2_width = -1;
  int ntt_tile = 2048;
  int quotient_first = 1;
  int lanes_after_quotient = 0;
  int g1_batch = 0;
  int mtab = 2;
  int chain_ch = 1;
  int tail_quad = 1;
  int red_chunk = 0;
  int cu_split = 0;
  int heavy_grid = 0;
  int cz_on_the_fly = 1;
  int abc_dict = 1;
  int g2_first = -1;
  int b1_fold = 1;
};
```

nim_groth16_amd/csrc/g16_internal.hpp:

```cpp
#pragma once
#include "../../include/g16hip.h"

#include <hip/hip_runtime.h>

#include <cstdio>
#include <cstring>
#include <map>
#include <string>
#include <vector>


#include "g16_env.hpp"
#include "hip_owners.hpp"
#include "msm_params.hpp"
#include "circuit_setup_plan.hpp"
#include "msm_plan.hpp"
#include "proof_plan.hpp"

const G16Env& g16_env();

struct ProfEntry {
  const char* name;
  Event e0, e1;
};

struct g16_ctx {
  int device = 0;
  hipStream_t stream = nullptr;
  Stream own_stream;
  std::string err;
  struct Buf {
    DevMem<> mem;
    size_t bytes = 0;
    void* p() const { return mem.get(); }
  };
  struct MsmSort {
    Buf buf;
    g16::MsmParams P;
    bool narrow_tail = false;
    uint32_t *count = nullptr, *cursor = nullptr, *offset = nullptr, *xoff = nullptr, *heavy = nullptr,
             *info = nullptr, *entries = nullptr, *perm = nullptr, *ghist = nullptr, *blk_base = nullptr, *tile_hist = nullptr;
    uint2* tmp = nullptr;
    uint32_t* slice_hist = nullptr;
    uint2* tiles2 = nullptr;
    uint2* tiles = nullptr;
    uint2* xseg = nullptr;
  };
  struct MsmLane {
    Stream stream;
    Event done;
    Buf acc;
  };
  MsmSort sort[4];
  MsmLane lane[5];
  Event ev[g16::EV_COUNT];
  Buf stage_s;
  Buf stage_p;
  Buf stage_p29;
  Buf stage_o;
  Buf ntt_tw;
  Buf ntt_tmp;
  Buf coset[2];
  Buf quot;
  Buf prove;
  Buf fb_table[2];
  bool fb_ready[2] = {false, false};
  DevMem<unsigned long long> clk_buf;
  const void* shard_begun = nullptr;
  uint32_t tw_log2n = 0xffffffffu;
  uint32_t coset_log2n[2] = {0xffffffffu, 0xffffffffu};
  bool profiling = false;
  bool prof_accum_only = false;
  std::vector<ProfEntry> prof;
  std::vector<Event> free_events;
};

inline int32_t g16_hip_check(std::string& err, const char* call, hipError_t e) {
  if (e == hipSuccess) return G16_OK;
  err = std::string(call) + ": " + hipGetErrorString(e);
  (void)hipGetLastError();
  return e == hipErrorOutOfMemory ? G16_ENOMEM : G16_EHIP;
}
#define HIPCHK(ctx, call)                                                          \
  do {                                                                             \
    if (int32_t hiprc__ = g16_hip_check((ctx)->err, #call, (call))) return hiprc__; \
  } while (0)

inline void ctx_quiesce(g16_ctx* ctx) {
  if (ctx->stream) (void)hipStreamSynchronize(ctx->stream);
  for (auto& l : ctx->lane)
    if (l.stream) (void)hipStreamSynchronize(l.stream.get());
}
struct SyncOnExit {
  hipStream_t stream;
  ~SyncOnExit() { (void)hipStreamSynchronize(stream); }
};

inline int32_t ctx_enter(g16_ctx* ctx, bool keep_shard = false) {
  HIPCHK(ctx, hipSetDevice(ctx->device));
  if (ctx->shard_begun && !keep_shard) {
    ctx_quiesce(ctx);
    ctx->shard_begun = nullptr;
  }
  return G16_OK;
}
#define CTX_ENTER(ctx)                              \
  do {                                              \
    if (int32_t rc__ = ctx_enter(ctx)) return rc__; \
  } while (0)
#define CTX_ENTER_KEEP(ctx)                               \
  do {                                                    \
    if (int32_t rc__ = ctx_enter(ctx, true)) return rc__; \
  } while (0)

inline int32_t ensure(g16_ctx* ctx, g16_ctx::Buf& b, size_t bytes) {
  if (b.bytes >= bytes) return G16_OK;
  HIPCHK(ctx, hipSetDevice(ctx->device));
  if (b.mem) {
    ctx_quiesce(ctx);
    b.mem.reset();
    b.bytes = 0;
  }
  size_t want = bytes + bytes / 8 + 4096;
  HIPCHK(ctx, dev_alloc(b.mem, want));
  b.bytes = want;
  return G16_OK;
}

#define G16_COMBINE_RES_BYTES 384
constexpr size_t STAGE_O_RESULT = 0, STAGE_O_RESULT_BYTES = G16_PARTIALS_BYTES;
constexpr size_t STAGE_O_COUNTERS = STAGE_O_RESULT + STAGE_O_RESULT_BYTES, STAGE_O_COUNTER_WORDS = 2;
constexpr size_t STAGE_O_COMBINE = 1024;
constexpr size_t STAGE_O_BYTES = 2048;
static_assert(STAGE_O_COUNTERS % 4 == 0 && STAGE_O_COUNTERS + 4 * STAGE_O_COUNTER_WORDS <= STAGE_O_COMBINE &&
                  STAGE_O_COMBINE % 128 == 0 && STAGE_O_COMBINE + G16_COMBINE_RES_BYTES <= STAGE_O_BYTES,
              "the pieces of stage_o overlap or do not fit");
inline int32_t ensure_stage_o(g16_ctx* ctx) { return ensure(ctx, ctx->stage_o, STAGE_O_BYTES); }
inline char* stage_o_at(g16_ctx* ctx, size_t offset) { return (char*)ctx->stage_o.p() + offset; }

template <class Launch>
inline int32_t counted_launch(g16_ctx* ctx, int fill, uint32_t* words, size_t nwords, Launch&& launch) {
  if (int32_t rc = ensure_stage_o(ctx)) return rc;
  uint32_t* d_words = (uint32_t*)stage_o_at(ctx, STAGE_O_COUNTERS);
  HIPCHK(ctx, hipMemsetAsync(d_words, fill, 4 * nwords, ctx->stream));
  if (int32_t rc = launch(d_words)) return rc;
  HIPCHK(ctx, hipMemcpyAsync(words, d_words, 4 * nwords, hipMemcpyDeviceToHost, ctx->stream));
  HIPCHK(ctx, hipStreamSynchronize(ctx->stream));
  return G16_OK;
}

struct ProfScope {
  g16_ctx* ctx;
  bool on;
  ProfEntry e;
  hipStream_t st;
  ProfScope(g16_ctx* c, const char* name, hipStream_t stream = nullptr)
      : ctx(c), on(c->profiling && (!c->prof_accum_only || strncmp(name, "msm_accum", 9) == 0)),
        st(stream ? stream : c->stream) {
    if (!on) return;
    e.name = name;
    auto get = [&](Event& ev) {
      if (!ctx->free_events.empty()) {
        ev = std::move(ctx->free_events.back());
        ctx->free_events.pop_back();
      } else {
        (void)event_create(ev, hipEventDefault);
      }
    };
    get(e.e0);
    get(e.e1);
    (void)hipEventRecord(e.e0.get(), st);
  }
  ~ProfScope() {
    if (!on) return;
    (void)hipEventRecord(e.e1.get(), st);
    ctx->prof.push_back(std::move(e));
  }
};
#define KLAUNCH_ON(ctx, stream_, name, kernel, grid, block, shmem, ...)                        \
  do {                                                                                         \
    ProfScope ps__(ctx, name, stream_);                                                        \
    hipLaunchKernelGGL(kernel, dim3(grid), dim3(block), shmem, stream_, __VA_ARGS__);          \
  } while (0)
#define KLAUNCH(ctx, name, kernel, grid, block, shmem, ...) \
  KLAUNCH_ON(ctx, (ctx)->stream, name, kernel, grid, block, shmem, __VA_ARGS__)


struct g16_points {
  int device = 0;
  int group = 1;
  size_t n = 0;
  uint32_t c = 0, nwin = 0;
  uint32_t mtab = 1;
  uint32_t stride = 1;
  uint32_t ntables() const { return mtab * ((nwin + stride - 1) / stride); }
  uint32_t cfg() const { return g16::msm_table_cfg(c, mtab, stride); }
  DevMem<> d_tables;
  DevMem<uint32_t> d_live;
  size_t n_inf = 0;
};
const uint32_t* g16_points_live_if_sparse(const g16_points* p);
int32_t g16_msm_sort(g16_ctx* ctx, hipStream_t stream, const void* d_scalars, uint32_t flags, size_t n,
                     uint32_t table_c, g16_ctx::MsmSort& sort, const uint32_t* d_live = nullptr);
struct g16_msm_sparse {
  const void* d_scalars;
  const uint32_t* d_wires;
  uint32_t nlive;
  const uint32_t* d_info;
};
struct g16_msm_run {
  const g16_ctx::MsmSort* sort;
  g16_ctx::Buf* acc;
  const void* d_points;
  void* d_out_aff;
  void* d_out_acc;
  const void* init_partial;
  const g16_msm_sparse* sparse = nullptr;
};
int32_t g16_msm_batch(g16_ctx* ctx, hipStream_t stream, int group, const g16_msm_run* runs, int n_accum, int n_tail,
                      hipEvent_t after_heavy);
inline const void* g16_msm_partial_ptr(const g16_ctx::Buf& acc) { return acc.p(); }
int32_t g16_lanes_init(g16_ctx* ctx);
int32_t g16_bitmap_or_device(g16_ctx* ctx, uint32_t* d_out, const uint32_t* d_a, const uint32_t* d_b, size_t n,
                             uint32_t* d_n_dead);

namespace g16 {
template <class C>
struct MsmBatch;
}
template <class C>
int32_t msm_device(g16_ctx* ctx, const void* d_scalars, uint32_t flags, const void* d_points, size_t n, void* d_out_aff,
                   void* d_out_acc, uint32_t table_c, const uint32_t* d_live = nullptr);
template <class C>
int32_t stage_accum(g16_ctx* ctx, hipStream_t st, const g16::MsmParams& P, const g16::MsmBatch<C>& B, uint32_t ny);
template <class C>
int32_t stage_accum_sparse(g16_ctx* ctx, hipStream_t st, const g16::MsmParams& P, const g16_msm_sparse& sp,
                           const void* d_points, void* d_partial, bool own_entry);
template <class C>
int32_t stage_heavy(g16_ctx* ctx, hipStream_t st, const g16::MsmParams& P, const g16::MsmTailPlan& T,
                    const g16::MsmBatch<C>& B, uint32_t ny);
template <class C>
int32_t stage_reduce1(g16_ctx* ctx, hipStream_t st, const g16::MsmParams& P, const g16::MsmTailPlan& T,
                      const g16::MsmBatch<C>& B, uint32_t ny);
template <class C>
int32_t stage_reduce2_fold(g16_ctx* ctx, hipStream_t st, const g16::MsmParams& P, const g16::MsmTailPlan& T,
                           const g16::MsmBatch<C>& B, uint32_t ny);
template <class C>
int32_t to29_device(g16_ctx* ctx, hipStream_t st, const void* d_points, size_t n, void* d_out);
template <class C>
int32_t precompute_device(g16_ctx* ctx, const void* d_points, size_t n, uint32_t c, uint32_t mtab, uint32_t stride,
                          void* d_tables);
template <class C>
int32_t fixed_base_device(g16_ctx* ctx, void* d_table, bool table_ready, const void* d_scalars, uint32_t mont, size_t n,
                          void* d_out);
template <class C>
int32_t on_curve_device(g16_ctx* ctx, const void* d_points, size_t n, uint32_t* d_first_bad);
template <class C>
int32_t live_bitmap_device(g16_ctx* ctx, const void* d_points, size_t n, uint32_t* d_bitmap, uint32_t* d_n_inf);
template <class C>
int32_t sum_partials_device(g16_ctx* ctx, const void* d_parts, uint32_t count, void* d_out_aff);

struct g16_spmat;
int32_t g16_spmat_create(g16_ctx* ctx, uint32_t nmat, uint32_t nrows, size_t nnz, const uint32_t* vrow,
                         size_t vrow_stride, const uint32_t* col, size_t col_stride, const void* val_base,
                         size_t val_stride, g16_spmat** out, bool values_r2 = false);
void g16_spmat_destroy(g16_spmat* m);
void g16_spmat_info(const g16_spmat* m, size_t out[10]);
int32_t g16_spmat_apply(g16_ctx* ctx, const g16_spmat* m, const void* d_x, uint32_t x_mont, void* d_out,
                        bool need_cz = true);
int32_t g16_ntt_device(g16_ctx* ctx, const void* d_src, void* d_dst, uint32_t log2n, int inverse);
int32_t g16_quotient_device(g16_ctx* ctx, const void* d_a, const void* d_b, const void* d_c, uint32_t log2n,
                            int flavour, void* d_out, int c_from_ab = 0);
int32_t g16_coset_pipeline_device(g16_ctx* ctx, const void* d_in, uint32_t log2n, void* d_out);
int32_t g16_abc_pointwise_device(g16_ctx* ctx, const void* d_a, const void* d_b, const void* d_c, size_t count,
                                 void* d_out);

int32_t g16_widen_multipliers(g16_ctx* ctx, const char* who, const void* multipliers, size_t n, std::vector<uint64_t>& out);
int32_t g16_key_audit_body(g16_ctx* ctx, const g16_pkey_desc* d, const g16_vkey_desc* vk, const void* section4,
                           size_t section4_bytes, const void* multipliers, g16_key_report* out);
struct g16_audit_section {
  int group;
  const void* p;
  size_t n;
};
struct g16_audit_coeffs {
  const void* base;
  size_t count, stride, value_offset;
};
int32_t g16_audit_sections(g16_ctx* ctx, const g16_audit_section* sec, int nsec, size_t (*first_bad)[3],
                           size_t (*bad_count)[3], const g16_audit_coeffs* coeffs = nullptr);

int32_t g16_pairing_products4(g16_ctx* ctx, const void* d_P, const void* d_Q, uint32_t count, uint32_t neg_mask,
                              int32_t* d_result);

namespace g16 {
struct u256;
}
int32_t g16_setup_geometric(g16_ctx* ctx, bool lagrange, const g16::u256& w0, const g16::u256& s, const g16::u256& c,
                            const g16::u256& tau, size_t count, g16::u256* d_out, uint32_t* d_first_zero);
namespace g16 {
template <class C>
int32_t cs_term_device(g16_ctx* ctx, const void* d_pts, const uint32_t* d_src, const void* d_val, const uint32_t* d_ord,
                       uint32_t vstride, uint32_t mont, uint32_t log2rev, size_t count, void* d_out_acc);
template <class C>
int32_t cs_butterflies_device(g16_ctx* ctx, void* d_v, const void* d_tw, uint32_t log2n);
template <class C>
int32_t cs_segsum_device(g16_ctx* ctx, const void* d_terms, const uint32_t* d_off, const uint32_t* d_wires,
                         const CsSumPlan& plan, void* d_out_aff);
template <class C>
int32_t cs_to_affine_device(g16_ctx* ctx, const void* d_acc, size_t count, void* d_out_aff);
template <class C>
int32_t cs_diff_device(g16_ctx* ctx, const void* d_p, const void* d_q, size_t count, void* d_out_aff);
}

namespace g16 {
struct ScalePlan;
struct ScaleJob;
template <class C>
int32_t scale_uniform_device(g16_ctx* ctx, const void* d_pts, size_t n, const ScaleJob& job, void* d_out_aff);
template <class C>
int32_t scale_each_device(g16_ctx* ctx, const void* d_pts, size_t n, const void* d_scalars, uint32_t mont, void* d_out_aff);
}
int32_t g16_scale_job(g16_ctx* ctx, const g16::u256& k_std, g16::ScalePlan& plan, uint32_t* d_steps, g16::ScaleJob& job);

struct g16_combine_pre {
  unsigned char r_std[32], s_std[32];
  unsigned char a_pre[64], b_pre[128], c_pre[64];
};
int32_t g16_combine_enqueue(g16_ctx* ctx, const g16_pkey* k, const void* partials, size_t count, uint32_t flags,
                            const void* mask_r, const void* mask_s, void* res_host, hipEvent_t done,
                            g16_combine_pre* pre);
void g16_combine_finish(const g16_combine_pre* pre, const void* res_host, g16_proof* out);
```

nim_groth16_amd/csrc/g16hip.hip:

```cpp
#include "g16_internal.hpp"
#include "ec.cuh"

using namespace g16;

static G16Env read_env() {
  G16Env e;
  auto num = [](const char* name, int lo, int hi) {
    const char* v = getenv(name);
    if (!v) return 0;
    int x = atoi(v);
    return x >= lo && x <= hi ? x : 0;
  };
  e.msm_window = num("G16_MSM_WINDOW", 5, 22);
  e.table_window = num("G16_TABLE_WINDOW", 5, 22);
  e.msm_seg = num("G16_MSM_SEG", 8, 4096);
  e.red_slice_log2 = num("G16_RED_SLICE", 8, 11);
  e.cu_split = num("G16_CU_SPLIT", 1, 24);
  e.heavy_grid = num("G16_HEAVY_GRID", 1, 4096);
  if (const char* v = getenv("G16_INF_COMPACT")) e.inf_compact_pct = atoi(v) < 0 ? 0 : atoi(v) > 101 ? 101 : atoi(v);
  if (const char* v = getenv("G16_R2_WIDTH")) e.r2_width = v[0] == '0' ? 0 : v[0] == '2' ? 2 : 1;
  if (const char* v = getenv("G16_LANES_AFTER_QUOTIENT")) e.lanes_after_quotient = v[0] != '0';
  if (const char* v = getenv("G16_QUOTIENT_FIRST")) e.quotient_first = v[0] != '0';
  if (const char* v = getenv("G16_G1_BATCH")) e.g1_batch = v[0] != '0';
  if (const char* v = getenv("G16_CHAIN_CH")) e.chain_ch = v[0] != '0';
  if (const char* v = getenv("G16_ABC_DICT")) e.abc_dict = v[0] != '0';
  if (const char* v = getenv("G16_CZ_FLY")) e.cz_on_the_fly = v[0] != '0';
  if (const char* v = getenv("G16_RED_CHUNK")) e.red_chunk = atoi(v) == 2 || atoi(v) == 4 || atoi(v) == 8 || atoi(v) == 16 ? atoi(v) : 0;
  if (const char* v = getenv("G16_TAIL_QUAD")) e.tail_quad = v[0] != '0';
  if (const char* v = getenv("G16_G2_FIRST")) e.g2_first = v[0] == '2' ? 2 : v[0] != '0';
  if (const char* v = getenv("G16_B1_FOLD")) e.b1_fold = v[0] != '0';
  if (const char* v = getenv("G16_MTAB")) e.mtab = v[0] == '1' ? 1 : 2;
  if (const char* v = getenv("G16_NTT_TILE")) e.ntt_tile = atoi(v) == 1024 ? 1024 : atoi(v) == 4096 ? 4096 : 2048;
  if (const char* v = getenv("G16_MSM_SORT")) e.msm_sort = v[0];
  if (const char* v = getenv("G16_G1_LANES"))
    if (strlen(v) == 3 && strspn(v, "023") == 3)
      for (int i = 0; i < 3; ++i) e.g1_lanes[i] = v[i] - '0';
  if (const char* v = getenv("G16_STREAM_PRIO"))
    if (strlen(v) >= 6 && strspn(v, "hnl") >= 6) memcpy(e.stream_prio, v, 6);
  return e;
}
const G16Env& g16_env() {
  static const G16Env env = read_env();
  return env;
}

static hipError_t ctx_stream_create(Stream& out, int prio_index, bool front) {
  hipStream_t st = nullptr;
  hipError_t e;
  if (g16_env().cu_split <= 0) {
    int lo = 0, hi = 0;
    (void)hipDeviceGetStreamPriorityRange(&lo, &hi);
    e = hipStreamCreateWithPriority(&st, hipStreamNonBlocking, stream_priority(g16_env(), prio_index, lo, hi));
  } else {
    uint32_t mask[8];
    stream_cu_mask(g16_env(), front, mask);
    e = hipExtStreamCreateWithCUMask(&st, 8, mask);
  }
  out.reset(st);
  return e;
}

extern "C" int32_t g16_ctx_create(int32_t device, g16_ctx** out) {
  if (!out) return G16_EINVAL;
  *out = nullptr;
  (void)g16_env();
  int ndev = 0;
  if (hipGetDeviceCount(&ndev) != hipSuccess || ndev <= 0) return G16_ENODEV;
  if (device < 0 || device >= ndev) return G16_EINVAL;
  if (hipSetDevice(device) != hipSuccess) return G16_ENODEV;
  Building<g16_ctx, g16_ctx_destroy> ctx(new (std::nothrow) g16_ctx());
  if (!ctx) return G16_ENOMEM;
  ctx->device = device;
  if (ctx_stream_create(ctx->own_stream, 5, true) != hipSuccess) return G16_ENODEV;
  ctx->stream = ctx->own_stream.get();
  if (g16_lanes_init(ctx.get()) != G16_OK) return G16_ENODEV;
  *out = ctx.release();
  return G16_OK;
}

int32_t g16_lanes_init(g16_ctx* ctx) {
  for (int i = 0; i < 5; ++i) {
    auto& l = ctx->lane[i];
    HIPCHK(ctx, ctx_stream_create(l.stream, i, false));
    HIPCHK(ctx, event_create(l.done));
  }
  for (Event& e : ctx->ev) HIPCHK(ctx, event_create(e));
  return G16_OK;
}

extern "C" void g16_ctx_destroy(g16_ctx* ctx) {
  if (!ctx) return;
  (void)hipSetDevice(ctx->device);
  ctx_quiesce(ctx);
  delete ctx;
}

extern "C" const char* g16_last_error(const g16_ctx* ctx) { return ctx ? ctx->err.c_str() : "null context"; }

extern "C" int32_t g16_ctx_set_stream(g16_ctx* ctx, void* hip_stream) {
  if (!ctx) return G16_EINVAL;
  CTX_ENTER(ctx);
  HIPCHK(ctx, hipStreamSynchronize(ctx->stream));
  ctx->own_stream.reset();
  if (!hip_stream) HIPCHK(ctx, stream_create(ctx->own_stream));
  ctx->stream = hip_stream ? (hipStream_t)hip_stream : ctx->own_stream.get();
  return G16_OK;
}

extern "C" int32_t g16_ctx_cancel(g16_ctx* ctx) {
  if (!ctx) return G16_EINVAL;
  HIPCHK(ctx, hipSetDevice(ctx->device));
  ctx_quiesce(ctx);
  ctx->shard_begun = nullptr;
  return G16_OK;
}

extern "C" int32_t g16_ctx_synchronize(g16_ctx* ctx) {
  if (!ctx) return G16_EINVAL;
  CTX_ENTER_KEEP(ctx);
  HIPCHK(ctx, hipStreamSynchronize(ctx->stream));
  return G16_OK;
}

extern "C" int32_t g16_profile_enable(g16_ctx* ctx, int32_t on) {
  if (!ctx) return G16_EINVAL;
  CTX_ENTER_KEEP(ctx);
  if (on && !ctx->clk_buf) {
    HIPCHK(ctx, dev_alloc(ctx->clk_buf, 16));
    HIPCHK(ctx, hipMemset(ctx->clk_buf.get(), 0, 16));
  }
  ctx->profiling = on != 0;
  ctx->prof_accum_only = on == 2;
  return G16_OK;
}
extern "C" int32_t g16_profile_reset(g16_ctx* ctx) {
  if (!ctx) return G16_EINVAL;
  CTX_ENTER_KEEP(ctx);
  HIPCHK(ctx, hipStreamSynchronize(ctx->stream));
  for (auto& e : ctx->prof) {
    ctx->free_events.push_back(std::move(e.e0));
    ctx->free_events.push_back(std::move(e.e1));
  }
  ctx->prof.clear();
  return G16_OK;
}
extern "C" int32_t g16_profile_report(g16_ctx* ctx, char* buf, size_t buflen) {
  if (!ctx || !buf || buflen < 3) return G16_EINVAL;
  CTX_ENTER_KEEP(ctx);
  HIPCHK(ctx, hipStreamSynchronize(ctx->stream));
  std::map<std::string, std::pair<int, double>> agg;
  for (auto& e : ctx->prof) {
    float ms = 0;
    if (hipEventElapsedTime(&ms, e.e0.get(), e.e1.get()) == hipSuccess) {
      auto& a = agg[e.name];
      a.first++;
      a.second += ms;
    }
  }
  std::string s = "{";
  bool first = true;
  for (auto& kv : agg) {
    char tmp[256];
    snprintf(tmp, sizeof tmp, "%s\"%s\": {\"calls\": %d, \"total_ms\": %.6f}", first ? "" : ", ", kv.first.c_str(),
             kv.second.first, kv.second.second);
    s += tmp;
    first = false;
  }
  s += "}";
  if (s.size() + 1 > buflen) return G16_EINVAL;
  memcpy(buf, s.c_str(), s.size() + 1);
  return G16_OK;
}

extern "C" int32_t g16_profile_clock(g16_ctx* ctx, double* ghz) {
  if (!ctx || !ghz) return G16_EINVAL;
  CTX_ENTER_KEEP(ctx);
  *ghz = 0.0;
  if (!ctx->clk_buf) return G16_OK;
  ctx_quiesce(ctx);
  unsigned long long h[2] = {0, 0};
  HIPCHK(ctx, hipMemcpy(h, ctx->clk_buf.get(), 16, hipMemcpyDeviceToHost));
  HIPCHK(ctx, hipMemset(ctx->clk_buf.get(), 0, 16));
  if (h[1]) *ghz = (double)h[0] / (double)h[1] * 0.1;
  return G16_OK;
}

template <class C>
constexpr int group_of = sizeof(typename C::Aff) == sizeof(g1_aff) ? 1 : 2;

template <class C>
static int32_t msm_entry(g16_ctx* ctx, const void* scalars, uint32_t flags, const void* points, size_t n, void* out,
                         bool on_device, bool partial) {
  if (!ctx) return G16_EINVAL;
  if (!out || (n > 0 && (!scalars || !points))) {
    ctx->err = "null pointer argument";
    return G16_EINVAL;
  }
  if (n >= (size_t(1) << 27)) {
    ctx->err = "n too large (must be < 2^27)";
    return G16_EINVAL;
  }
  CTX_ENTER(ctx);
  const size_t out_bytes = partial ? sizeof(typename C::Acc) : sizeof(typename C::Aff);
  if (n == 0) {
    memset(out, 0, out_bytes);
    return G16_OK;
  }
  const void* d_s = scalars;
  const void* d_p = points;
  int32_t rc;
  if (!on_device) {
    if ((rc = ensure(ctx, ctx->stage_s, n * 32))) return rc;
    if ((rc = ensure(ctx, ctx->stage_p, n * sizeof(typename C::Aff)))) return rc;
    HIPCHK(ctx, hipMemcpyAsync(ctx->stage_s.p(), scalars, n * 32, hipMemcpyHostToDevice, ctx->stream));
    HIPCHK(ctx, hipMemcpyAsync(ctx->stage_p.p(), points, n * sizeof(typename C::Aff), hipMemcpyHostToDevice,
                               ctx->stream));
    d_s = ctx->stage_s.p();
    d_p = ctx->stage_p.p();
  }
  if ((rc = ensure_stage_o(ctx))) return rc;
  auto* d_aff = partial ? nullptr : (typename C::Aff*)ctx->stage_o.p();
  auto* d_acc = partial ? (typename C::Acc*)ctx->stage_o.p() : nullptr;
  if ((rc = msm_device<C>(ctx, d_s, flags, d_p, n, d_aff, d_acc, 0))) return rc;
  HIPCHK(ctx, hipMemcpyAsync(out, ctx->stage_o.p(), out_bytes, hipMemcpyDeviceToHost, ctx->stream));
  HIPCHK(ctx, hipStreamSynchronize(ctx->stream));
  return G16_OK;
}

template <class C>
static int32_t points_register(g16_ctx* ctx, const void* points, size_t n, bool on_device, uint32_t table_stride,
                               g16_points** out) {
  if (!ctx) return G16_EINVAL;
  if (!out || (n && !points) || n >= (size_t(1) << 26)) {
    ctx->err = "bad argument";
    return G16_EINVAL;
  }
  *out = nullptr;
  CTX_ENTER(ctx);
  Building<g16_points, g16_points_release> h(new (std::nothrow) g16_points());
  if (!h) return G16_ENOMEM;
  h->device = ctx->device;
  h->group = group_of<C>;
  h->n = n;
  const MsmTableChoice choice = msm_table_choice(n, table_stride, g16_env());
  h->c = choice.c;
  h->nwin = 254 / h->c + 1;
  h->mtab = choice.mtab;
  h->stride = choice.stride;
  constexpr size_t psz = sizeof(typename C::Aff);
  if (!choice.fits) {
    ctx->err = "point set too large for 31-bit table indices";
    return G16_EINVAL;
  }
  if (n) {
    if (h->mtab == 2 && dev_alloc(h->d_tables, (size_t)h->ntables() * n * psz) != hipSuccess) {
      (void)hipGetLastError();
      h->mtab = 1;
    }
    if (!h->d_tables) HIPCHK(ctx, dev_alloc(h->d_tables, (size_t)h->ntables() * n * psz));
    const void* d_src = points;
    int32_t rc;
    if (!on_device) {
      if ((rc = ensure(ctx, ctx->stage_p, n * psz))) return rc;
      HIPCHK(ctx, hipMemcpyAsync(ctx->stage_p.p(), points, n * psz, hipMemcpyHostToDevice, ctx->stream));
      d_src = ctx->stage_p.p();
    }
    if ((rc = precompute_device<C>(ctx, d_src, n, h->c, h->mtab, h->stride, h->d_tables.get()))) return rc;
    uint32_t n_inf = 0;
    HIPCHK(ctx, dev_alloc(h->d_live, ((n + 31) / 32 + 1) * 4));
    rc = counted_launch(ctx, 0, &n_inf, 1, [&](uint32_t* d_n_inf) {
      return live_bitmap_device<C>(ctx, d_src, n, h->d_live.get(), d_n_inf);
    });
    if (rc) return rc;
    h->n_inf = n_inf;
  }
  *out = h.release();
  return G16_OK;
}
extern "C" int32_t g16_points_register_g1(g16_ctx* ctx, const void* points, size_t n, g16_points** out) {
  return points_register<G1>(ctx, points, n, false, 0, out);
}
extern "C" int32_t g16_points_register_g2(g16_ctx* ctx, const void* points, size_t n, g16_points** out) {
  return points_register<G2>(ctx, points, n, false, 0, out);
}
extern "C" int32_t g16_points_register_g1_dev(g16_ctx* ctx, const void* d_points, size_t n, g16_points** out) {
  return points_register<G1>(ctx, d_points, n, true, 0, out);
}
extern "C" int32_t g16_points_register_g2_dev(g16_ctx* ctx, const void* d_points, size_t n, g16_points** out) {
  return points_register<G2>(ctx, d_points, n, true, 0, out);
}
extern "C" int32_t g16_points_register_g1_lean(g16_ctx* ctx, const void* points, size_t n, uint32_t table_stride,
                                               g16_points** out) {
  return points_register<G1>(ctx, points, n, false, table_stride, out);
}
extern "C" int32_t g16_points_register_g2_lean(g16_ctx* ctx, const void* points, size_t n, uint32_t table_stride,
                                               g16_points** out) {
  return points_register<G2>(ctx, points, n, false, table_stride, out);
}
extern "C" int32_t g16_points_register_g1_lean_dev(g16_ctx* ctx, const void* d_points, size_t n, uint32_t table_stride,
                                                   g16_points** out) {
  return points_register<G1>(ctx, d_points, n, true, table_stride, out);
}
extern "C" int32_t g16_points_register_g2_lean_dev(g16_ctx* ctx, const void* d_points, size_t n, uint32_t table_stride,
                                                   g16_points** out) {
  return points_register<G2>(ctx, d_points, n, true, table_stride, out);
}
extern "C" int32_t g16_points_plan(int group, size_t n, uint32_t table_stride, uint32_t* window_bits, uint32_t* ntables,
                                   size_t* bytes) {
  if ((group != 1 && group != 2) || n >= (size_t(1) << 26)) return G16_EINVAL;
  const MsmTableChoice choice = msm_table_choice(n, table_stride, g16_env());
  if (!choice.fits) return G16_EINVAL;
  if (window_bits) *window_bits = choice.c;
  if (ntables) *ntables = choice.ntables;
  if (bytes) *bytes = (size_t)choice.ntables * n * (group == 1 ? sizeof(g1_aff) : sizeof(g2_aff));
  return G16_OK;
}
extern "C" int32_t g16_points_table_bytes(const g16_points* h, size_t* bytes) {
  if (!h || !bytes) return G16_EINVAL;
  *bytes = (size_t)h->ntables() * h->n * (h->group == 1 ? sizeof(g1_aff) : sizeof(g2_aff));
  return G16_OK;
}
extern "C" void g16_points_release(g16_points* h) {
  if (!h) return;
  if (h->d_tables) {
    (void)hipSetDevice(h->device);
    (void)hipDeviceSynchronize();
  }
  delete h;
}
extern "C" size_t g16_points_inf_count(const g16_points* h) { return h ? h->n_inf : 0; }
const uint32_t* g16_points_live_if_sparse(const g16_points* p) {
  return p && p->d_live && p->n && points_sparse(p->n_inf, p->n, g16_env()) ? p->d_live.get() : nullptr;
}
// ... 250 lines not shown
```

nim_groth16_amd/csrc/ntt.cuh:

```cuda
#pragma once
#include "ff.cuh"

namespace g16 {

__device__ __forceinline__ u256 ntt_gen28() {
  u256 g;
  g.v[0] = 0x725b19f0u; g.v[1] = 0x9bd61b6eu; g.v[2] = 0x41112ed4u; g.v[3] = 0x402d111eu;
  g.v[4] = 0x8ef62abcu; g.v[5] = 0x00e0a7ebu; g.v[6] = 0xa58a7e85u; g.v[7] = 0x2a3c09f0u;
  return Fr::to_mont(g);
}
__device__ __forceinline__ u256 ntt_omega(uint32_t log2n) {
  u256 w = ntt_gen28();
  for (uint32_t i = log2n; i < 28; ++i) w = Fr::sqr(w);
  return w;
}
__device__ __forceinline__ u256 fr_pow_u32(u256 b, uint32_t e) {
  u256 r = Fr::one();
  while (e) {
    if (e & 1) r = Fr::mul(r, b);
    b = Fr::sqr(b);
    e >>= 1;
  }
  return r;
}

static __global__ void __launch_bounds__(256) ntt_make_twiddles(u256* __restrict__ tw, uint32_t log2n) {
  const uint32_t half = log2n ? (1u << (log2n - 1)) : 0u;
  uint32_t i = blockIdx.x * 256 + threadIdx.x;
  if (i < half) {
    tw[i] = fr_pow_u32(ntt_omega(log2n), i);
  } else if (i == half) {
    u256 h = Fr::one();
    for (uint32_t k = 0; k < log2n; ++k) h = Fr::div2(h);
    tw[half] = h;
  }
}

__device__ __forceinline__ u256 ntt_tw(const u256* __restrict__ tw, uint32_t e, uint32_t log2n, int inverse) {
  const uint32_t n = 1u << log2n, half = n >> 1;
  if (inverse && e) e = n - e;
  if (e < half) return tw[e];
  return Fr::neg(tw[e - half]);
}

constexpr int NTT_BLOCK = 1024;
constexpr int NTT_TILE = 4096;
constexpr uint32_t NTT_MAX_RHO = 10;
constexpr int NTT_BLOCK_SMALL = 256;
constexpr int NTT_TILE_SMALL = 1024;
constexpr uint32_t NTT_MAX_RHO_SMALL = 8;
constexpr int NTT_BLOCK_MID = 512;
constexpr int NTT_TILE_MID = 2048;

__device__ __forceinline__ uint32_t bitrev(uint32_t x, uint32_t bits) { return bits ? __brev(x) >> (32 - bits) : 0u; }

__device__ __forceinline__ uint32_t ntt_tile_of_block(uint32_t bid, uint32_t ntiles) {
  return (ntiles & 7u) ? bid : (bid & 7u) * (ntiles >> 3) + (bid >> 3);
}

template <int BLOCK>
__device__ __forceinline__ void ntt_tile_stages(u256* lds, const u256* twl, uint32_t rho, uint32_t log2b,
                                                uint32_t tile) {
  const uint32_t tid = threadIdx.x, B = 1u << log2b;
  uint32_t lh = rho;
  if (lh & 1u) {
    --lh;
    const uint32_t h = 1u << lh;
    for (uint32_t bf = tid; bf < (tile >> 1); bf += BLOCK) {
      uint32_t b = bf & (B - 1), pi = bf >> log2b;
      uint32_t p = pi & (h - 1);
      uint32_t i = ((pi >> lh) << (lh + 1)) | p;
      uint32_t ia = (i << log2b) | b, ib = ((i + h) << log2b) | b;
      u256 a = lds[ia], c = lds[ib];
      u256 sum = Fr::add(a, c), dif = Fr::sub(a, c);
      if (p) dif = Fr::mul(dif, twl[p << (rho - lh - 1)]);
      lds[ia] = sum;
      lds[ib] = dif;
    }
    __syncthreads();
  }
  while (lh >= 2) {
    lh -= 2;
    const uint32_t hh = 1u << lh, h = hh << 1;
    const uint32_t sA = rho - lh - 2;
    for (uint32_t g = tid; g < (tile >> 2); g += BLOCK) {
      const uint32_t b = g & (B - 1), pi = g >> log2b;
      const uint32_t p = pi & (hh - 1);
      const uint32_t i = ((pi >> lh) << (lh + 2)) | p;
      const uint32_t i0 = (i << log2b) | b, i1 = ((i + hh) << log2b) | b, i2 = ((i + h) << log2b) | b,
                     i3 = ((i + h + hh) << log2b) | b;
      const u256 x0 = lds[i0], x1 = lds[i1], x2 = lds[i2], x3 = lds[i3];
      u256 a0 = Fr::add(x0, x2), a2 = Fr::sub(x0, x2);
      u256 a1 = Fr::add(x1, x3), a3 = Fr::sub(x1, x3);
      if (p) a2 = Fr::mul(a2, twl[p << sA]);
      a3 = Fr::mul(a3, twl[(p + hh) << sA]);
      u256 b0 = Fr::add(a0, a1), b1 = Fr::sub(a0, a1);
      u256 b2 = Fr::add(a2, a3), b3 = Fr::sub(a2, a3);
      if (p) {
        const u256 tb = twl[p << (sA + 1)];
        b1 = Fr::mul(b1, tb);
        b3 = Fr::mul(b3, tb);
      }
      lds[i0] = b0;
      lds[i1] = b1;
      lds[i2] = b2;
      lds[i3] = b3;
    }
    __syncthreads();
  }
}

template <int BLOCK>
static __global__ void __launch_bounds__(BLOCK) ntt_pass(const u256* __restrict__ x, u256* __restrict__ y,
                                                      const u256* __restrict__ tw, uint32_t log2n, uint32_t log2s,
                                                      uint32_t rho, uint32_t log2b, int inverse, int last,
                                                      size_t xstride, size_t ystride,
                                                      const u256* __restrict__ scale, int mul_src) {
  extern __shared__ __align__(16) unsigned char smem[];
  u256* lds = reinterpret_cast<u256*>(smem);
  x += xstride * blockIdx.y;
  y += ystride * blockIdx.y;
  const uint32_t R = 1u << rho, B = 1u << log2b;
  const uint32_t nR = 1u << (log2n - rho);
  const uint32_t base0 = ntt_tile_of_block(blockIdx.x, gridDim.x) << log2b;
  const uint32_t tile = R << log2b;
  const uint32_t tid = threadIdx.x;

  u256* twl = lds + tile;
  for (uint32_t t = tid; t < (R >> 1); t += BLOCK) twl[t] = ntt_tw(tw, t << (log2n - rho), log2n, inverse);
  if (mul_src && blockIdx.y == 2) {
    const u256* xa = x - 2 * xstride;
    const u256* xb = x - xstride;
    for (uint32_t e = tid; e < tile; e += BLOCK) {
      uint32_t b = e & (B - 1), r = e >> log2b;
      const size_t gi = (size_t)base0 + b + (size_t)nR * r;
      lds[e] = Fr::mul(xa[gi], xb[gi]);
    }
  } else {
    for (uint32_t e = tid; e < tile; e += BLOCK) {
      uint32_t b = e & (B - 1), r = e >> log2b;
      lds[e] = x[(size_t)base0 + b + (size_t)nR * r];
    }
  }
  __syncthreads();

  ntt_tile_stages<BLOCK>(lds, twl, rho, log2b, tile);

  const uint32_t s_mask = (1u << log2s) - 1;
  for (uint32_t e = tid; e < tile; e += BLOCK) {
    uint32_t b = e & (B - 1), q = e >> log2b;
    uint32_t base = base0 + b;
    uint32_t k = base & s_mask, j = base >> log2s;
    u256 v = lds[(bitrev(q, rho) << log2b) | b];
    if (!last) {
      uint64_t ex = ((uint64_t)j * q) << log2s;
      uint32_t em = (uint32_t)(ex & ((1ull << log2n) - 1));
      if (em) v = Fr::mul(v, ntt_tw(tw, em, log2n, inverse));
    }
    const size_t oi = (size_t)k + ((size_t)(((size_t)j << rho) + q) << log2s);
    if (last) {
      if (scale) v = Fr::mul(v, scale[oi]);
      else if (inverse) v = Fr::mul(v, tw[(1u << log2n) >> 1]);
    }
    y[oi] = v;
  }
}

template <int BLOCK, int TILE>
static __global__ void __launch_bounds__(BLOCK) ntt_last_pass_abc(const u256* __restrict__ x, u256* __restrict__ out,
                                                               const u256* __restrict__ tw, uint32_t log2n,
                                                               uint32_t log2s, uint32_t rho, uint32_t log2b,
                                                               size_t xstride, int mul_invz) {
  extern __shared__ __align__(16) unsigned char smem[];
  u256* lds = reinterpret_cast<u256*>(smem);
  constexpr int PER = TILE / BLOCK;
  const uint32_t R = 1u << rho, B = 1u << log2b;
  const uint32_t nR = 1u << (log2n - rho);
  const uint32_t base0 = ntt_tile_of_block(blockIdx.x, gridDim.x) << log2b;
  const uint32_t tile = R << log2b;
  const uint32_t tid = threadIdx.x;
  u256* twl = lds + tile;
  for (uint32_t t = tid; t < (R >> 1); t += BLOCK) twl[t] = ntt_tw(tw, t << (log2n - rho), log2n, 0);
  u256 acc[PER];
#pragma unroll 1
  for (int v = 0; v < 3; ++v) {
    const u256* xv = x + xstride * v;
    for (uint32_t e = tid; e < tile; e += BLOCK) {
      uint32_t b = e & (B - 1), r = e >> log2b;
      lds[e] = xv[(size_t)base0 + b + (size_t)nR * r];
    }
    __syncthreads();
    ntt_tile_stages<BLOCK>(lds, twl, rho, log2b, tile);
#pragma unroll
    for (int i = 0; i < PER; ++i) {
      const uint32_t e = tid + i * BLOCK;
      if (e < tile) {
        uint32_t b = e & (B - 1), q = e >> log2b;
        u256 z = lds[(bitrev(q, rho) << log2b) | b];
        acc[i] = v == 0 ? z : v == 1 ? Fr::mul(acc[i], z) : Fr::sub(acc[i], z);
      }
    }
    __syncthreads();
  }
  const uint32_t s_mask = (1u << log2s) - 1;
#pragma unroll
  for (int i = 0; i < PER; ++i) {
    const uint32_t e = tid + i * BLOCK;
    if (e < tile) {
      uint32_t b = e & (B - 1), q = e >> log2b;
      uint32_t base = base0 + b;
      uint32_t k = base & s_mask, j = base >> log2s;
      const size_t oi = (size_t)k + ((size_t)(((size_t)j << rho) + q) << log2s);
      u256 r = acc[i];
      if (mul_invz) r = Fr::neg(Fr::div2(r));
      out[oi] = r;
    }
  }
}

static __global__ void __launch_bounds__(256) ntt_make_coset_table(u256* __restrict__ tab, uint32_t log2n, int mode) {
  uint32_t i = blockIdx.x * 256 + threadIdx.x;
  const uint32_t n = 1u << log2n;
  if (i >= n) return;
  u256 ninv = Fr::one();
  for (uint32_t k = 0; k < log2n; ++k) ninv = Fr::div2(ninv);
  u256 eta = ntt_omega(log2n + 1);
  uint32_t e = mode ? (2 * n - i) % (2 * n) : i;
  tab[i] = Fr::mul(fr_pow_u32(eta, e), ninv);
}

static __global__ void __launch_bounds__(256) fr_abc_pointwise(const u256* __restrict__ a, const u256* __restrict__ b,
                                                        const u256* __restrict__ c, u256* __restrict__ out,
                                                        uint32_t n) {
  uint32_t j = blockIdx.x * 256 + threadIdx.x;
  if (j >= n) return;
  out[j] = Fr::sub(Fr::mul(a[j], b[j]), c[j]);
}

}
```

nim_groth16_amd/csrc/ntt.hip:

```cpp
#include <atomic>
#include <mutex>

#include "g16_internal.hpp"
#include "ntt.cuh"
#include "ntt_plan.hpp"

using namespace g16;

static int32_t ensure_twiddles(g16_ctx* ctx, uint32_t log2n) {
  if (ctx->tw_log2n == log2n) return G16_OK;
  const size_t n = size_t(1) << log2n;
  int32_t rc;
  if ((rc = ensure(ctx, ctx->ntt_tw, (n / 2 + 1) * 32))) return rc;
  KLAUNCH(ctx, "ntt_twiddles", ntt_make_twiddles, (uint32_t)((n / 2 + 1 + 255) / 256), 256, 0, (u256*)ctx->ntt_tw.p(),
          log2n);
  ctx->tw_log2n = log2n;
  return G16_OK;
}

static_assert(ntt_geom(NTT_TILE_SMALL).max_rho == NTT_MAX_RHO_SMALL &&
                  (1 << ntt_geom(NTT_TILE_SMALL).log2tile) == NTT_TILE_SMALL,
              "ntt_plan.hpp and ntt.cuh disagree on the 1024 geometry");
static_assert(ntt_geom(NTT_TILE_MID).max_rho == NTT_MAX_RHO && (1 << ntt_geom(NTT_TILE_MID).log2tile) == NTT_TILE_MID,
              "ntt_plan.hpp and ntt.cuh disagree on the 2048 geometry");
static_assert(ntt_geom(NTT_TILE).max_rho == NTT_MAX_RHO && (1 << ntt_geom(NTT_TILE).log2tile) == NTT_TILE,
              "ntt_plan.hpp and ntt.cuh disagree on the 4096 geometry");
static_assert(ntt_optin_shmem() == ntt_pass_shmem(NTT_MAX_RHO, 2), "the opt-in covers the largest pass");
static int32_t ntt_kernels_init(g16_ctx* ctx) {
  static std::atomic<bool> done_on[64];
  static std::mutex mu;
  std::atomic<bool>& done = done_on[ctx->device & 63];
  if (done.load(std::memory_order_acquire)) return G16_OK;
  std::lock_guard<std::mutex> lock(mu);
  if (done.load(std::memory_order_relaxed)) return G16_OK;
  const int max_shmem = (int)ntt_optin_shmem();
  static_assert((size_t(32) * NTT_TILE) + (size_t(16) << NTT_MAX_RHO) <= 160 * 1024, "tile + twiddles must fit the LDS");
  HIPCHK(ctx, hipFuncSetAttribute(reinterpret_cast<const void*>(&ntt_pass<NTT_BLOCK>),
                                  hipFuncAttributeMaxDynamicSharedMemorySize, max_shmem));
  HIPCHK(ctx, hipFuncSetAttribute(reinterpret_cast<const void*>(&ntt_last_pass_abc<NTT_BLOCK, NTT_TILE>),
                                  hipFuncAttributeMaxDynamicSharedMemorySize, max_shmem));
  HIPCHK(ctx, hipFuncSetAttribute(reinterpret_cast<const void*>(&ntt_pass<NTT_BLOCK_MID>),
                                  hipFuncAttributeMaxDynamicSharedMemorySize, max_shmem));
  HIPCHK(ctx, hipFuncSetAttribute(reinterpret_cast<const void*>(&ntt_last_pass_abc<NTT_BLOCK_MID, NTT_TILE_MID>),
                                  hipFuncAttributeMaxDynamicSharedMemorySize, max_shmem));
  done.store(true, std::memory_order_release);
  return G16_OK;
}

struct NttKernels {
  uint32_t block;
  decltype(&ntt_last_pass_abc<NTT_BLOCK, NTT_TILE>) last_pass_abc;
  decltype(&ntt_pass<NTT_BLOCK>) pass;
};
static const NttKernels ntt_kernels[3] = {
    {NTT_BLOCK_SMALL, ntt_last_pass_abc<NTT_BLOCK_SMALL, NTT_TILE_SMALL>, ntt_pass<NTT_BLOCK_SMALL>},
    {NTT_BLOCK_MID, ntt_last_pass_abc<NTT_BLOCK_MID, NTT_TILE_MID>, ntt_pass<NTT_BLOCK_MID>},
    {NTT_BLOCK, ntt_last_pass_abc<NTT_BLOCK, NTT_TILE>, ntt_pass<NTT_BLOCK>},
};

static int32_t ntt_batched(g16_ctx* ctx, const u256* in, size_t in_stride, u256* out, size_t out_stride,
                           uint32_t batch, uint32_t log2n, int inverse, const u256* scale, int fuse_abc = 0,
                           int c_from_ab = 0) {
  const size_t n = size_t(1) << log2n;
  int32_t rc;
  if ((rc = ensure_twiddles(ctx, log2n))) return rc;
  if ((rc = ntt_kernels_init(ctx))) return rc;
  if (log2n == 0 && !fuse_abc) {
    for (uint32_t b = 0; b < batch; ++b)
      HIPCHK(ctx, hipMemcpyAsync(out + b * out_stride, in + b * in_stride, 32, hipMemcpyDeviceToDevice, ctx->stream));
    return G16_OK;
  }
  const int tile = g16_env().ntt_tile;
  const NttGeom geom = ntt_geom(tile);
  const NttKernels& K = ntt_kernels[tile == NTT_TILE_SMALL ? 0 : tile == NTT_TILE_MID ? 1 : 2];
  const uint32_t npass = ntt_npass(geom, log2n);
  u256 *tmpA = nullptr, *tmpB = nullptr;
  if (npass > 1) {
    if ((rc = ensure(ctx, ctx->ntt_tmp, (npass > 2 ? 2 : 1) * n * 32 * batch))) return rc;
    tmpA = (u256*)ctx->ntt_tmp.p();
    tmpB = tmpA + n * batch;
  }
  const u256* src = in;
  size_t src_stride = in_stride;
  for (uint32_t p = 0; p < npass; ++p) {
    const NttPass plan = ntt_pass_plan(geom, log2n, p);
    const bool last = p + 1 == npass;
    if (last && fuse_abc) {
      KLAUNCH(ctx, "ntt_last_pass_abc", K.last_pass_abc, plan.ntiles, K.block, plan.shmem, src, out,
              (const u256*)ctx->ntt_tw.p(), log2n, plan.log2s, plan.rho, plan.log2b, src_stride, fuse_abc == 2 ? 1 : 0);
      break;
    }
    u256* dst = last ? out : ((p & 1) ? tmpB : tmpA);
    const size_t dst_stride = last ? out_stride : n;
    KLAUNCH(ctx, inverse ? "ntt_pass_inv" : "ntt_pass_fwd", K.pass, dim3(plan.ntiles, batch), K.block, plan.shmem, src, dst,
            (const u256*)ctx->ntt_tw.p(), log2n, plan.log2s, plan.rho, plan.log2b, inverse, last ? 1 : 0, src_stride,
            dst_stride, last ? scale : (const u256*)nullptr, p == 0 ? c_from_ab : 0);
    src = dst;
    src_stride = dst_stride;
  }
  HIPCHK(ctx, hipGetLastError());
  return G16_OK;
}

int32_t g16_ntt_device(g16_ctx* ctx, const void* d_src, void* d_dst, uint32_t log2n, int inverse) {
  if (d_src == d_dst && ntt_one_pass(ntt_geom(g16_env().ntt_tile), log2n) && log2n > 0) {
    int32_t rc = ensure(ctx, ctx->ntt_tmp, (size_t(32) << log2n));
    if (rc) return rc;
    if ((rc = ntt_batched(ctx, (const u256*)d_src, 0, (u256*)ctx->ntt_tmp.p(), 0, 1, log2n, inverse, nullptr))) return rc;
    HIPCHK(ctx, hipMemcpyAsync(d_dst, ctx->ntt_tmp.p(), size_t(32) << log2n, hipMemcpyDeviceToDevice, ctx->stream));
    return G16_OK;
  }
  return ntt_batched(ctx, (const u256*)d_src, 0, (u256*)d_dst, 0, 1, log2n, inverse, nullptr);
}

static int32_t ensure_coset(g16_ctx* ctx, uint32_t log2n, int mode) {
  if (ctx->coset_log2n[mode] == log2n) return G16_OK;
  const size_t n = size_t(1) << log2n;
  int32_t rc;
  if ((rc = ensure(ctx, ctx->coset[mode], n * 32))) return rc;
  KLAUNCH(ctx, "ntt_coset_table", ntt_make_coset_table, (uint32_t)((n + 255) / 256), 256, 0,
          (u256*)ctx->coset[mode].p(), log2n, mode);
  ctx->coset_log2n[mode] = log2n;
  return G16_OK;
}

int32_t g16_quotient_device(g16_ctx* ctx, const void* d_a, const void* d_b, const void* d_c, uint32_t log2n,
                            int flavour, void* d_out, int c_from_ab) {
  if (log2n > 27) {
    ctx->err = "quotient needs the 2n domain: log2n <= 27";
    return G16_EINVAL;
  }
  const size_t n = size_t(1) << log2n;
  int32_t rc;
  if ((rc = ensure(ctx, ctx->quot, 4 * n * 32))) return rc;
  if ((rc = ensure_coset(ctx, log2n, 0))) return rc;
  u256* X = (u256*)ctx->quot.p();
  u256* Y = X + 3 * n;
  const u256* in = (const u256*)d_a;
  if (c_from_ab && ((const u256*)d_b != in + n || (const u256*)d_c != in + 2 * n || log2n == 0)) {
    ctx->err = "quotient: Cz can only be formed on the fly from contiguous Az | Bz | Cz";
    return G16_EINVAL;
  }
  if ((const u256*)d_b != in + n || (const u256*)d_c != in + 2 * n) {
    HIPCHK(ctx, hipMemcpyAsync(X, d_a, n * 32, hipMemcpyDeviceToDevice, ctx->stream));
    HIPCHK(ctx, hipMemcpyAsync(X + n, d_b, n * 32, hipMemcpyDeviceToDevice, ctx->stream));
    HIPCHK(ctx, hipMemcpyAsync(X + 2 * n, d_c, n * 32, hipMemcpyDeviceToDevice, ctx->stream));
    in = X;
    if (ntt_one_pass(ntt_geom(g16_env().ntt_tile), log2n)) {
      if ((rc = ensure(ctx, ctx->ntt_tmp, 3 * n * 32))) return rc;
      HIPCHK(ctx, hipMemcpyAsync(ctx->ntt_tmp.p(), X, 3 * n * 32, hipMemcpyDeviceToDevice, ctx->stream));
      in = (const u256*)ctx->ntt_tmp.p();
    }
  }
  if ((rc = ntt_batched(ctx, in, n, X, n, 3, log2n, 1, (const u256*)ctx->coset[0].p(), 0, c_from_ab))) return rc;
  if (flavour == 1) {
    if ((rc = ntt_batched(ctx, X, n, (u256*)d_out, 0, 3, log2n, 0, nullptr, 1))) return rc;
  } else {
    if ((rc = ensure_coset(ctx, log2n, 1))) return rc;
    if ((rc = ntt_batched(ctx, X, n, Y, 0, 3, log2n, 0, nullptr, 2))) return rc;
    if ((rc = ntt_batched(ctx, Y, n, (u256*)d_out, n, 1, log2n, 1, (const u256*)ctx->coset[1].p()))) return rc;
  }
  HIPCHK(ctx, hipGetLastError());
  return G16_OK;
}

int32_t g16_coset_pipeline_device(g16_ctx* ctx, const void* d_in, uint32_t log2n, void* d_out) {
  if (log2n > 27) {
    ctx->err = "quotient needs the 2n domain: log2n <= 27";
    return G16_EINVAL;
  }
  const size_t n = size_t(1) << log2n;
  int32_t rc;
  if ((rc = ensure(ctx, ctx->quot, 4 * n * 32))) return rc;
  if ((rc = ensure_coset(ctx, log2n, 0))) return rc;
  u256* X = (u256*)ctx->quot.p();
  if ((rc = ntt_batched(ctx, (const u256*)d_in, n, X, n, 1, log2n, 1, (const u256*)ctx->coset[0].p()))) return rc;
  return ntt_batched(ctx, X, n, (u256*)d_out, n, 1, log2n, 0, nullptr);
}

int32_t g16_abc_pointwise_device(g16_ctx* ctx, const void* d_a, const void* d_b, const void* d_c, size_t count,
                                 void* d_out) {
  if (count)
    KLAUNCH(ctx, "fr_abc_pointwise", fr_abc_pointwise, (uint32_t)((count + 255) / 256), 256, 0, (const u256*)d_a,
            (const u256*)d_b, (const u256*)d_c, (u256*)d_out, (uint32_t)count);
  HIPCHK(ctx, hipGetLastError());
  return G16_OK;
}
```

nim_groth16_amd/csrc/pkey.hip:

```cpp
#include <algorithm>
#include <cstddef>
#include <new>

#include "pkey.hpp"
#include "b1_fold.cuh"

using namespace g16;

extern "C" void g16_pkey_destroy(g16_pkey* k) {
  if (!k) return;
  for (g16_points* p : {k->A1, k->B1, k->B2, k->C1, k->H1}) g16_points_release(p);
  (void)hipSetDevice(k->device);
  (void)hipDeviceSynchronize();
  g16_spmat_destroy(k->abc);
  delete k;
}

extern "C" int32_t g16_pkey_inf_counts(const g16_pkey* k, size_t out[8]) {
  if (!k || !out) return G16_EINVAL;
  out[0] = k->A1->n_inf, out[1] = k->b1_inf, out[2] = k->B2->n_inf, out[4] = k->H1->n_inf;
  out[3] = k->C1->n_inf - c1_padding(k->w, k->npubs);
  out[5] = k->deadB, out[6] = k->liveA ? 1 : 0, out[7] = k->liveB ? 1 : 0;
  return G16_OK;
}

extern "C" int32_t g16_pkey_b1_fold(const g16_pkey* k, size_t out[3]) {
  if (!k || !out) return G16_EINVAL;
  out[0] = (size_t)k->b1_form, out[1] = k->live_b1, out[2] = k->live_delta;
  return G16_OK;
}

extern "C" int32_t g16_pkey_b1_sparse(const g16_pkey* k, size_t out[3]) {
  if (!k || !out) return G16_EINVAL;
  out[0] = k->b1_sparse ? 1 : 0, out[1] = k->b1_nlive, out[2] = B1_SPARSE_MAX;
  return G16_OK;
}

extern "C" int32_t g16_pkey_abc_info(const g16_pkey* k, size_t out[11]) {
  if (!k || !out) return G16_EINVAL;
  out[0] = k->ncoeffs;
  g16_spmat_info(k->abc, out + 1);
  return G16_OK;
}

struct CoeffSource {
  const unsigned char* base = nullptr;
  size_t count = 0, stride = 0, value_off = 0;
  bool values_r2 = false;
};
static inline uint32_t rd32(const unsigned char* p) {
  uint32_t v;
  memcpy(&v, p, 4);
  return v;
}

static __global__ void __launch_bounds__(256) b1_compare_kernel(const uint4* __restrict__ a1, const uint4* __restrict__ b1,
                                                                uint32_t n, uint32_t* __restrict__ cnt) {
  const uint32_t i = blockIdx.x * 256 + threadIdx.x;
  bool live = false, differs = false;
  if (i < n) {
    uint32_t any = 0, diff = 0;
#pragma unroll
    for (int q = 0; q < 4; ++q) {
      const uint4 a = a1[(size_t)i * 4 + q], b = b1[(size_t)i * 4 + q];
      any |= b.x | b.y | b.z | b.w;
      diff |= (a.x ^ b.x) | (a.y ^ b.y) | (a.z ^ b.z) | (a.w ^ b.w);
    }
    live = any != 0, differs = diff != 0;
  }
  const uint32_t nl = (uint32_t)__popcll(__ballot(live)), nd = (uint32_t)__popcll(__ballot(differs));
  if ((threadIdx.x & 63) == 0) {
    if (nl) atomicAdd(&cnt[0], nl);
    if (nd) atomicAdd(&cnt[1], nd);
  }
}
static __global__ void __launch_bounds__(256) b1_delta_kernel(const g1_aff* __restrict__ a1, g1_aff* __restrict__ b1,
                                                              uint32_t n) {
  const uint32_t i = blockIdx.x * 256 + threadIdx.x;
  if (i >= n) return;
  b1[i] = point_difference<G1>(b1[i], a1[i]);
}

static bool desc_well_formed(const g16_pkey_desc* d) {
  return d->log2_domain <= 27 && d->nvars != 0 && d->npubs + 1 <= d->nvars && d->flavour <= 1 && d->pointsA1 &&
         d->pointsB1 && d->pointsB2 && d->pointsH1 && (d->nvars - d->npubs - 1 == 0 || d->pointsC1) && d->alpha1 &&
         d->beta1 && d->delta1 && d->beta2 && d->delta2;
}

static int32_t key_layout(g16_ctx* ctx, const g16_pkey_desc* d, g16_pkey* k) {
  k->device = ctx->device;
  k->nvars = d->nvars;
  k->npubs = d->npubs;
  k->log2n = d->log2_domain;
  k->flavour = d->flavour;
  memcpy(&k->alpha1, d->alpha1, 64);
  memcpy(&k->beta1, d->beta1, 64);
  memcpy(&k->delta1, d->delta1, 64);
  memcpy(&k->beta2, d->beta2, 128);
  memcpy(&k->delta2, d->delta2, 128);
  k->shard_count = d->shard_count ? d->shard_count : 1;
  k->shard_index = d->shard_index;
  if (k->shard_index >= k->shard_count) {
    ctx->err = "shard_index >= shard_count";
    return G16_EINVAL;
  }
  k->w = shard_range(d->nvars, k->shard_index, k->shard_count);
  k->h = shard_range(size_t(1) << d->log2_domain, k->shard_index, k->shard_count);
  return G16_OK;
}

static int32_t b1_form_of_whole_arrays(g16_ctx* ctx, const g16_pkey_desc* d, g16_pkey* k) {
  const size_t nv = d->nvars;
  uint32_t cnt[2] = {0, 0};
  if (g16_env().b1_fold) {
    constexpr size_t CHUNK = size_t(1) << 16;
    const size_t step = std::min(nv, CHUNK);
    DevMem<g1_aff> c_a1, c_b1;
    SyncOnExit sync{ctx->stream};
    HIPCHK(ctx, dev_alloc(c_a1, step * sizeof(g1_aff)));
    HIPCHK(ctx, dev_alloc(c_b1, step * sizeof(g1_aff)));
    const int32_t rc = counted_launch(ctx, 0, cnt, 2, [&](uint32_t* d_cnt) -> int32_t {
      for (size_t lo = 0; lo < nv; lo += step) {
        const size_t m = std::min(step, nv - lo);
        HIPCHK(ctx, hipMemcpyAsync(c_a1.get(), (const char*)d->pointsA1 + 64 * lo, m * 64, hipMemcpyHostToDevice, ctx->stream));
        HIPCHK(ctx, hipMemcpyAsync(c_b1.get(), (const char*)d->pointsB1 + 64 * lo, m * 64, hipMemcpyHostToDevice, ctx->stream));
        hipLaunchKernelGGL(b1_compare_kernel, dim3((uint32_t)((m + 255) / 256)), dim3(256), 0, ctx->stream,
                           (const uint4*)c_a1.get(), (const uint4*)c_b1.get(), (uint32_t)m, d_cnt);
        HIPCHK(ctx, hipGetLastError());
      }
      return G16_OK;
    });
    if (rc) return rc;
  }
  k->live_b1 = cnt[0], k->live_delta = cnt[1];
  k->b1_form = b1_fold_form(cnt[0], cnt[1], nv, g16_env());
  return G16_OK;
}

static int32_t b1_live_wires(g16_ctx* ctx, g16_pkey* k) {
  if (!b1_sparse_run(k->live_delta)) return G16_OK;
  const size_t nw = k->w.size(), words = (nw + 31) / 32;
  std::vector<uint32_t> bitmap(words), list(g16_pkey::B1_VIEW_WORDS, 0u);
  HIPCHK(ctx, hipMemcpyAsync(bitmap.data(), k->B1->d_live.get(), words * 4, hipMemcpyDeviceToHost, ctx->stream));
  HIPCHK(ctx, hipStreamSynchronize(ctx->stream));
  for (size_t i = 0; i < nw; ++i)
    if ((bitmap[i >> 5] >> (i & 31)) & 1u) list.push_back((uint32_t)i);
  const size_t nlive = list.size() - g16_pkey::B1_VIEW_WORDS;
  if (nlive > B1_SPARSE_MAX || nlive != nw - k->B1->n_inf) {
    ctx->err = "the live differences of pointsB1 do not match their count";
    return G16_EINVAL;
  }
  list.push_back(0u);
  HIPCHK(ctx, dev_alloc(k->b1_sparse, list.size() * 4));
  HIPCHK(ctx, hipMemcpyAsync(k->b1_sparse.get(), list.data(), list.size() * 4, hipMemcpyHostToDevice, ctx->stream));
  HIPCHK(ctx, hipStreamSynchronize(ctx->stream));
  k->b1_nlive = (uint32_t)nlive;
  return G16_OK;
}

static int32_t register_b1(g16_ctx* ctx, const g16_pkey_desc* d, uint32_t table_stride, g16_pkey* k) {
  const size_t nw = k->w.size();
  int32_t rc;
  if (k->b1_form != B1_DELTA || !nw) {
    if ((rc = g16_points_register_g1_lean(ctx, (const char*)d->pointsB1 + 64 * k->w.lo, nw, table_stride, &k->B1))) return rc;
    k->b1_inf = k->B1->n_inf;
    return G16_OK;
  }
  DevMem<g1_aff> d_a1, d_b1;
  DevMem<uint32_t> scratch_live;
  SyncOnExit sync{ctx->stream};
  HIPCHK(ctx, dev_alloc(d_a1, nw * sizeof(g1_aff)));
  HIPCHK(ctx, dev_alloc(d_b1, nw * sizeof(g1_aff)));
  HIPCHK(ctx, hipMemcpyAsync(d_a1.get(), (const char*)d->pointsA1 + 64 * k->w.lo, nw * 64, hipMemcpyHostToDevice, ctx->stream));
  HIPCHK(ctx, hipMemcpyAsync(d_b1.get(), (const char*)d->pointsB1 + 64 * k->w.lo, nw * 64, hipMemcpyHostToDevice, ctx->stream));
  HIPCHK(ctx, dev_alloc(scratch_live, ((nw + 31) / 32 + 1) * 4));
  uint32_t n_inf = 0;
  rc = counted_launch(ctx, 0, &n_inf, 1, [&](uint32_t* d_n_inf) -> int32_t {
    if (int32_t e = live_bitmap_device<G1>(ctx, d_b1.get(), nw, scratch_live.get(), d_n_inf)) return e;
    hipLaunchKernelGGL(b1_delta_kernel, dim3((uint32_t)((nw + 255) / 256)), dim3(256), 0, ctx->stream,
                       (const g1_aff*)d_a1.get(), d_b1.get(), (uint32_t)nw);
    HIPCHK(ctx, hipGetLastError());
    return G16_OK;
  });
  if (rc) return rc;
  k->b1_inf = n_inf;
  if ((rc = g16_points_register_g1_lean_dev(ctx, d_b1.get(), nw, table_stride, &k->B1))) return rc;
  return b1_live_wires(ctx, k);
}

static std::vector<unsigned char> c1_wire_aligned(const g16_pkey_desc* d, const g16_pkey* k) {
  std::vector<unsigned char> c1pad(k->w.size() * 64, 0);
  for (size_t wI = k->w.lo + c1_padding(k->w, d->npubs); wI < k->w.hi; ++wI)
    memcpy(&c1pad[(wI - k->w.lo) * 64], (const char*)d->pointsC1 + 64 * (wI - d->npubs - 1), 64);
  return c1pad;
}

static int32_t live_lists(g16_ctx* ctx, g16_pkey* k) {
  const size_t nw = k->w.size(), bitmap_bytes = ((nw + 31) / 32 + 1) * 4;
  k->liveA = g16_points_live_if_sparse(k->A1);
  const LiveSource source = live_b_source(k->b1_form, nw, (bool)k->B1->d_live, (bool)k->B2->d_live);
  if (source == LIVE_B2) {
    k->deadB = k->B2->n_inf;
    if (live_b_kept(source, k->deadB, nw, g16_env())) {
      HIPCHK(ctx, dev_alloc(k->liveB, bitmap_bytes));
      HIPCHK(ctx, hipMemcpyAsync(k->liveB.get(), k->B2->d_live.get(), bitmap_bytes, hipMemcpyDeviceToDevice, ctx->stream));
      HIPCHK(ctx, hipStreamSynchronize(ctx->stream));
    }
  } else if (source == LIVE_UNION) {
    uint32_t dead = 0;
    HIPCHK(ctx, dev_alloc(k->liveB, bitmap_bytes));
    const int32_t rc = counted_launch(ctx, 0, &dead, 1, [&](uint32_t* d_dead) {
      return g16_bitmap_or_device(ctx, k->liveB.get(), k->B1->d_live.get(), k->B2->d_live.get(), nw, d_dead);
    });
    if (rc) return rc;
    k->deadB = dead;
    if (!live_b_kept(source, dead, nw, g16_env())) k->liveB.reset();
  }
  return G16_OK;
}

static int32_t bin_coefficients(g16_ctx* ctx, const g16_pkey_desc* d, const CoeffSource& cs, g16_pkey* k) {
  const size_t n = size_t(1) << d->log2_domain;
  std::vector<uint32_t> vrow;
  try {
    vrow.resize(cs.count ? cs.count : 1);
  } catch (const std::bad_alloc&) {
    ctx->err = "out of host memory";
    return G16_ENOMEM;
  }
  for (size_t e = 0; e < cs.count; ++e) {
    const unsigned char* ent = cs.base + e * cs.stride;
    const uint32_t matrix = rd32(ent), row = rd32(ent + 4), col = rd32(ent + 8);
    if (matrix > 1 || row >= n || col >= d->nvars) {
      ctx->err = "coefficient entry out of range (matrix must be 0=A or 1=B)";
      return G16_EINVAL;
    }
    vrow[e] = 2 * row + matrix;
  }
  k->ncoeffs = cs.count;
  return g16_spmat_create(ctx, 2, (uint32_t)n, cs.count, vrow.data(), 4, (const uint32_t*)(cs.count ? cs.base + 8 : nullptr),
                          cs.stride, cs.count ? cs.base + cs.value_off : nullptr, cs.stride, &k->abc, cs.values_r2);
}

static int32_t pkey_create(g16_ctx* ctx, const g16_pkey_desc* d, const CoeffSource& cs, uint32_t table_stride,
                           g16_pkey** out) {
  if (!desc_well_formed(d)) {
    ctx->err = "bad proving-key description";
    return G16_EINVAL;
  }
  CTX_ENTER(ctx);
  Building<g16_pkey, g16_pkey_destroy> k(new (std::nothrow) g16_pkey());
  if (!k) return G16_ENOMEM;
  const uint32_t ts = table_stride;
  int32_t rc;
  if ((rc = key_layout(ctx, d, k.get()))) return rc;
  const std::vector<unsigned char> c1pad = c1_wire_aligned(d, k.get());
  if ((rc = g16_points_register_g1_lean(ctx, (const char*)d->pointsA1 + 64 * k->w.lo, k->w.size(), ts, &k->A1))) return rc;
  if ((rc = b1_form_of_whole_arrays(ctx, d, k.get()))) return rc;
  if ((rc = register_b1(ctx, d, ts, k.get()))) return rc;
  if ((rc = g16_points_register_g2_lean(ctx, (const char*)d->pointsB2 + 128 * k->w.lo, k->w.size(), ts, &k->B2))) return rc;
  if ((rc = g16_points_register_g1_lean(ctx, c1pad.data(), k->w.size(), ts, &k->C1))) return rc;
  if ((rc = g16_points_register_g1_lean(ctx, (const char*)d->pointsH1 + 64 * k->h.lo, k->h.size(), ts, &k->H1))) return rc;
  if ((rc = live_lists(ctx, k.get()))) return rc;
  if ((rc = bin_coefficients(ctx, d, cs, k.get()))) return rc;
  *out = k.release();
  return G16_OK;
}

extern "C" int32_t g16_pkey_create_lean(g16_ctx* ctx, const g16_pkey_desc* d, uint32_t table_stride, g16_pkey** out) {
  if (!ctx) return G16_EINVAL;
  if (!d || !out || (d->ncoeffs && !d->coeffs)) {
    ctx->err = "null argument";
    return G16_EINVAL;
  }
  *out = nullptr;
  static_assert(sizeof(g16_coeff) == 48 && offsetof(g16_coeff, value) == 16, "g16_coeff layout");
  CoeffSource cs;
  cs.base = (const unsigned char*)d->coeffs, cs.count = d->ncoeffs, cs.stride = sizeof(g16_coeff), cs.value_off = 16;
  return pkey_create(ctx, d, cs, table_stride, out);
}
extern "C" int32_t g16_pkey_create(g16_ctx* ctx, const g16_pkey_desc* d, g16_pkey** out) {
  return g16_pkey_create_lean(ctx, d, 0, out);
}

extern "C" int32_t g16_pkey_create_zkey_lean(g16_ctx* ctx, const g16_pkey_desc* d, const void* section4,
                                             size_t section4_bytes, uint32_t table_stride, g16_pkey** out) {
  if (!ctx) return G16_EINVAL;
  if (!d || !out || !section4 || section4_bytes < 4 || d->coeffs || d->ncoeffs) {
    ctx->err = "bad argument (section 4 of the .zkey in, desc.coeffs = NULL, desc.ncoeffs = 0)";
    return G16_EINVAL;
  }
  *out = nullptr;
  const unsigned char* p = (const unsigned char*)section4;
  const size_t count = rd32(p);
  if (section4_bytes != 4 + count * 44) {
    ctx->err = "unexpected length of the coefficient section (4 + 44 * count bytes)";
    return G16_EINVAL;
  }
  CoeffSource cs;
  cs.base = p + 4, cs.count = count, cs.stride = 44, cs.value_off = 12, cs.values_r2 = true;
  return pkey_create(ctx, d, cs, table_stride, out);
}
extern "C" int32_t g16_pkey_create_zkey(g16_ctx* ctx, const g16_pkey_desc* d, const void* section4, size_t section4_bytes,
                                        g16_pkey** out) {
  return g16_pkey_create_zkey_lean(ctx, d, section4, section4_bytes, 0, out);
}
```

nim_groth16_amd/csrc/pkey.hpp:

```cpp
#pragma once
#include "g16_internal.hpp"
#include "ec.cuh"

struct g16_pkey {
  int device = 0;
  uint32_t nvars = 0, npubs = 0, log2n = 0, flavour = 1;
  uint32_t shard_index = 0, shard_count = 1;
  g16::KeyRange w{0, 0};
  g16::KeyRange h{0, 0};
  g16_points *A1 = nullptr, *B1 = nullptr, *B2 = nullptr, *C1 = nullptr, *H1 = nullptr;
  g16_spmat* abc = nullptr;
  size_t ncoeffs = 0;
  g16::g1_aff alpha1, beta1, delta1;
  g16::g2_aff beta2, delta2;
  const uint32_t* liveA = nullptr;
  DevMem<uint32_t> liveB;
  size_t deadB = 0;
  int b1_form = g16::B1_PLAIN;
  size_t b1_inf = 0;
  size_t live_b1 = 0, live_delta = 0;
  static constexpr size_t B1_VIEW_WORDS = 16;
  DevMem<uint32_t> b1_sparse;
  uint32_t b1_nlive = 0;
};
```

nim_groth16_amd/csrc/prover.hip:

```cpp
#include "pkey.hpp"
#include "host_curve.hpp"

using namespace g16;

static int32_t build_abc_device(g16_ctx* ctx, const g16_pkey* k, const u256* d_wit, uint32_t wit_mont, u256* d_abc,
                                bool need_cz = true) {
  return g16_spmat_apply(ctx, k->abc, d_wit, wit_mont, d_abc, need_cz);
}

extern "C" int32_t g16_build_abc(g16_ctx* ctx, const g16_pkey* k, const void* witness, uint32_t flags, void* out_abc) {
  if (!ctx) return G16_EINVAL;
  if (!k || !witness || !out_abc || k->device != ctx->device) {
    ctx->err = "bad argument";
    return G16_EINVAL;
  }
  CTX_ENTER(ctx);
  const size_t n = size_t(1) << k->log2n;
  int32_t rc;
  if ((rc = ensure(ctx, ctx->prove, ((size_t)k->nvars + 4 * n) * 32))) return rc;
  u256* d_w = (u256*)ctx->prove.p();
  u256* d_abc = d_w + k->nvars;
  HIPCHK(ctx, hipMemcpyAsync(d_w, witness, (size_t)k->nvars * 32, hipMemcpyHostToDevice, ctx->stream));
  if ((rc = build_abc_device(ctx, k, d_w, (flags & G16_SCALARS_MONT) ? 1u : 0u, d_abc))) return rc;
  HIPCHK(ctx, hipMemcpyAsync(out_abc, d_abc, 3 * n * 32, hipMemcpyDeviceToHost, ctx->stream));
  HIPCHK(ctx, hipStreamSynchronize(ctx->stream));
  return G16_OK;
}

static constexpr size_t PART_A = 0, PART_B1 = 128, PART_B2 = 256, PART_H = 512, PART_C = 640, PART_BYTES = G16_PARTIALS_BYTES;
static_assert(PART_C + sizeof(g1_acc) == PART_BYTES && PART_BYTES <= STAGE_O_RESULT_BYTES, "record layout");

static ProofShape proof_shape(const g16_pkey* k) {
  return ProofShape{k->w.size(), k->h.size(), k->log2n, k->liveA != nullptr, (bool)k->liveB,
                    k->C1->cfg() == k->H1->cfg(), k->b1_form};
}

struct ProofArgs {
  const void* witness = nullptr;
  uint32_t flags = 0;
  u256* task_out = nullptr;
  const void *d_a1 = nullptr, *d_b1 = nullptr, *d_c1 = nullptr;
  bool qs_is_slice = false;
  void* out_partials = nullptr;
};

static int32_t run_plan(g16_ctx* ctx, const g16_pkey* k, ProofEntry entry, uint32_t task_mask, bool host_sync,
                        const ProofArgs& a) {
  ProofPlan plan;
  if (!proof_plan_build(plan, g16_env(), entry, task_mask, host_sync, proof_shape(k))) {
    ctx->err = "proof launch plan exceeds its capacity";
    return G16_EINVAL;
  }
  const size_t n = size_t(1) << k->log2n, nw = k->w.size(), nh = k->h.size();
  int32_t rc;
  if ((rc = ensure(ctx, ctx->prove, ((size_t)k->nvars + 4 * n) * 32))) return rc;
  if ((rc = ensure_stage_o(ctx))) return rc;
  u256* const d_w = (u256*)ctx->prove.p();
  u256* const d_abc = d_w + k->nvars;
  u256* const d_qs = d_abc + 3 * n;
  char* const slots = stage_o_at(ctx, STAGE_O_RESULT);
  const u256* const d_wr = d_w + k->w.lo;
  const u256* const d_qs_slice = a.qs_is_slice ? d_qs : d_qs + k->h.lo;
  const uint32_t wit_mont = (a.flags & G16_SCALARS_MONT) ? 1u : 0u;
  g16_ctx::MsmLane* L = ctx->lane;
  const g16_points* const sets[RUN_COUNT] = {k->A1, k->B1, k->C1, k->B2, k->H1};
  g16_msm_run runs[RUN_COUNT] = {
      {&ctx->sort[plan.sort_a], &L[0].acc, k->A1->d_tables.get(), nullptr, slots + PART_A, nullptr},
      {&ctx->sort[plan.sort_b1], &L[2].acc, k->b1_form == B1_EMPTY ? nullptr : k->B1->d_tables.get(), nullptr,
       slots + PART_B1, nullptr},
      {&ctx->sort[SORT_W], &L[3].acc, k->C1->d_tables.get(), nullptr, slots + PART_C, nullptr},
      {&ctx->sort[plan.sort_b], &L[1].acc, k->B2->d_tables.get(), nullptr, slots + PART_B2, nullptr},
      {&ctx->sort[SORT_H], &L[4].acc, k->H1->d_tables.get(), nullptr, slots + PART_H, nullptr}};
  g16_msm_sparse b1_sparse{d_wr, nullptr, k->b1_nlive, k->b1_sparse.get()};
  if (k->b1_sparse) {
    b1_sparse.d_wires = k->b1_sparse.get() + g16_pkey::B1_VIEW_WORDS;
    runs[RUN_B1].sparse = &b1_sparse;
  }
  auto event = [&](int e) { return e == EV_NONE ? nullptr : e < EV_COUNT ? ctx->ev[e].get() : L[e - EV_DONE0].done.get(); };
  for (int i = 0; i < plan.count; ++i) {
    const ProofStep& s = plan.steps[i];
    rc = G16_OK;
    hipStream_t st = s.stream == PS_MAIN ? ctx->stream : L[s.stream].stream.get();
    switch (s.op) {
      case OP_UPLOAD:
        HIPCHK(ctx, hipMemcpyAsync(d_w, a.witness, (size_t)k->nvars * 32,
                                   (a.flags & G16_SCALARS_DEVICE) ? hipMemcpyDeviceToDevice : hipMemcpyHostToDevice, st));
        HIPCHK(ctx, hipMemsetAsync(slots, 0, PART_BYTES, st));
        break;
      case OP_WAIT: HIPCHK(ctx, hipStreamWaitEvent(st, event(s.a), 0)); break;
      case OP_RECORD: HIPCHK(ctx, hipEventRecord(event(s.a), st)); break;
      case OP_SORT_W:
        ctx->sort[s.a].narrow_tail = plan.narrow_tail;
        rc = g16_msm_sort(ctx, st, d_wr, wit_mont ? G16_SCALARS_MONT : 0u, nw, sets[s.c]->cfg(), ctx->sort[s.a],
                          s.b == 0 ? nullptr : s.b == 1 ? k->liveA : k->liveB.get());
        break;
      case OP_SORT_H:
        ctx->sort[SORT_H].narrow_tail = plan.narrow_tail;
        rc = g16_msm_sort(ctx, st, d_qs_slice, G16_SCALARS_MONT, nh, k->H1->cfg(), ctx->sort[SORT_H]);
        break;
      case OP_BUILD_ABC: rc = build_abc_device(ctx, k, d_w, wit_mont, d_abc, s.a != 0); break;
      case OP_QUOTIENT:
        rc = g16_quotient_device(ctx, d_abc, d_abc + n, d_abc + 2 * n, k->log2n, (int)k->flavour, d_qs, s.a);
        break;
      case OP_COSET: {
        const int at = __builtin_popcount(task_mask & ((1u << s.a) - 1));
        rc = g16_coset_pipeline_device(ctx, d_abc + s.a * n, k->log2n, a.task_out + at * n);
        break;
      }
      case OP_POINTWISE: rc = g16_abc_pointwise_device(ctx, a.d_a1, a.d_b1, a.d_c1, nh, d_qs); break;
      case OP_MSM:
        runs[RUN_H].init_partial = s.e ? g16_msm_partial_ptr(L[3].acc) : nullptr;
        rc = g16_msm_batch(ctx, st, s.a == RUN_B2 ? 2 : 1, &runs[s.a], s.b, s.c, event(s.d));
        break;
      case OP_COPY_OUT:
        HIPCHK(ctx, hipMemcpyAsync(a.out_partials, slots, PART_BYTES,
                                   (a.flags & G16_OUT_DEVICE) ? hipMemcpyDeviceToDevice : hipMemcpyDeviceToHost, st));
        break;
      case OP_HOST_SYNC: HIPCHK(ctx, hipStreamSynchronize(st)); break;
    }
    if (rc) return rc;
  }
  return G16_OK;
}

extern "C" int32_t g16_prove_partials(g16_ctx* ctx, const g16_pkey* k, const void* witness, uint32_t flags,
                                      void* out_partials) {
  if (!ctx) return G16_EINVAL;
  if (!k || !witness || !out_partials || k->device != ctx->device) {
    ctx->err = "bad argument";
    return G16_EINVAL;
  }
  CTX_ENTER(ctx);
  ProofArgs a;
  a.witness = witness, a.flags = flags, a.out_partials = out_partials;
  const bool host_sync = !((flags & G16_NO_HOST_SYNC) && (flags & G16_OUT_DEVICE));
  const int32_t rc = run_plan(ctx, k, PROOF_WHOLE, 0, host_sync, a);
  if (rc != G16_OK) ctx_quiesce(ctx);
  return rc;
}

extern "C" int32_t g16_prove_partials_begin(g16_ctx* ctx, const g16_pkey* k, const void* witness, uint32_t flags,
                                            uint32_t task_mask, void* d_task_out) {
  if (!ctx) return G16_EINVAL;
  if (!k || !witness || k->device != ctx->device || task_mask > 7 || (task_mask && !d_task_out)) {
    ctx->err = "bad argument";
    return G16_EINVAL;
  }
  if (k->flavour != G16_FLAVOUR_SNARKJS) {
    ctx->err = "the task-parallel quotient serves snarkjs-flavour keys (JensGroth needs a 7th transform of the whole "
               "vector: use g16_prove_partials)";
    return G16_EINVAL;
  }
  CTX_ENTER(ctx);
  ProofArgs a;
  a.witness = witness, a.flags = flags, a.task_out = (u256*)d_task_out;
  const int32_t rc = run_plan(ctx, k, PROOF_BEGIN, task_mask, !(flags & G16_NO_HOST_SYNC), a);
  if (rc != G16_OK) {
    ctx_quiesce(ctx);
    return rc;
  }
  ctx->shard_begun = k;
  return G16_OK;
}

extern "C" int32_t g16_prove_partials_end(g16_ctx* ctx, const g16_pkey* k, const void* d_a1, const void* d_b1,
                                          const void* d_c1, uint32_t flags, void* out_partials) {
  if (!ctx) return G16_EINVAL;
  const size_t nh = k ? k->h.size() : 0;
  if (!k || !out_partials || k->device != ctx->device || (nh && (!d_a1 || !d_b1 || !d_c1))) {
    ctx->err = "bad argument";
    return G16_EINVAL;
  }
  if (ctx->shard_begun != k) {
    ctx->err = "g16_prove_partials_end without a matching g16_prove_partials_begin on this context";
    return G16_EINVAL;
  }
  CTX_ENTER_KEEP(ctx);
  ctx->shard_begun = nullptr;
  ProofArgs a;
  a.flags = flags, a.d_a1 = d_a1, a.d_b1 = d_b1, a.d_c1 = d_c1, a.qs_is_slice = true, a.out_partials = out_partials;
  const int32_t rc = run_plan(ctx, k, PROOF_END, 0, !((flags & G16_NO_HOST_SYNC) && (flags & G16_OUT_DEVICE)), a);
  if (rc != G16_OK) ctx_quiesce(ctx);
  return rc;
}

static __global__ void prove_combine_kernel(const unsigned char* __restrict__ gathered, uint32_t count, uint32_t fold_b1,
                                            unsigned char* __restrict__ out) {
  if (threadIdx.x != 0) return;
  const uint32_t b = blockIdx.x;
  if (b == 2) {
    g2_acc r = G2::acc_inf();
    for (uint32_t i = 0; i < count; ++i) G2::add(r, *(const g2_acc*)(gathered + (size_t)i * PART_BYTES + PART_B2));
    *(g2_aff*)(out + 128) = G2::to_affine(r);
  } else {
    const size_t src = b == 0 ? PART_A : b == 1 ? PART_B1 : b == 3 ? PART_H : PART_C;
    const size_t dst = b == 0 ? 0 : b == 1 ? 64 : b == 3 ? 256 : 320;
    g1_acc r = G1::acc_inf();
    for (uint32_t i = 0; i < count; ++i) G1::add(r, *(const g1_acc*)(gathered + (size_t)i * PART_BYTES + src));
    if (b == 1 && fold_b1)
      for (uint32_t i = 0; i < count; ++i) G1::add(r, *(const g1_acc*)(gathered + (size_t)i * PART_BYTES + PART_A));
    *(g1_aff*)(out + dst) = G1::to_affine(r);
  }
}

static_assert(sizeof(CombineRes) == G16_COMBINE_RES_BYTES, "slot layout");
static_assert(sizeof(CombinePre) == sizeof(g16_combine_pre), "g16_combine_pre layout");

int32_t g16_combine_enqueue(g16_ctx* ctx, const g16_pkey* k, const void* partials, size_t count, uint32_t flags,
                            const void* mask_r, const void* mask_s, void* res_host, hipEvent_t done,
                            g16_combine_pre* pre_out) {
  int32_t rc;
  if ((rc = ensure(ctx, ctx->stage_p, count * PART_BYTES))) return rc;
  if ((rc = ensure_stage_o(ctx))) return rc;
  HIPCHK(ctx, hipMemcpyAsync(ctx->stage_p.p(), partials, count * PART_BYTES,
                             (flags & G16_SCALARS_DEVICE) ? hipMemcpyDeviceToDevice : hipMemcpyHostToDevice,
                             ctx->stream));
  unsigned char* d_res = (unsigned char*)stage_o_at(ctx, STAGE_O_COMBINE);
  KLAUNCH(ctx, "prove_combine", prove_combine_kernel, 5, 64, 0, (const unsigned char*)ctx->stage_p.p(), (uint32_t)count,
          k->b1_form != B1_PLAIN ? 1u : 0u, d_res);

  u256 r = Fr::zero(), s = Fr::zero();
  if (mask_r) memcpy(&r, mask_r, 32);
  if (mask_s) memcpy(&s, mask_s, 32);
  const CombinePre pre = host_combine_pre(k->alpha1, k->beta1, k->delta1, k->beta2, k->delta2, r, s);
  memcpy(pre_out, &pre, sizeof pre);
  HIPCHK(ctx, hipMemcpyAsync(res_host, d_res, sizeof(CombineRes), hipMemcpyDeviceToHost, ctx->stream));
  if (done) HIPCHK(ctx, hipEventRecord(done, ctx->stream));
  return G16_OK;
}

void g16_combine_finish(const g16_combine_pre* pre_in, const void* res_host, g16_proof* out) {
  CombinePre pre;
  CombineRes res;
  memcpy(&pre, pre_in, sizeof pre);
  memcpy(&res, res_host, sizeof res);
  g1_aff pi_a, pi_c;
  g2_aff pi_b;
  host_combine_finish(pre, res, pi_a, pi_b, pi_c);
  memcpy(out->pi_a, &pi_a, 64);
  memcpy(out->pi_b, &pi_b, 128);
  memcpy(out->pi_c, &pi_c, 64);
}

extern "C" int32_t g16_prove_combine(g16_ctx* ctx, const g16_pkey* k, const void* partials, size_t count,
                                     uint32_t flags, const void* mask_r, const void* mask_s, g16_proof* out) {
  if (!ctx) return G16_EINVAL;
  if (!k || !partials || !out || k->device != ctx->device || count == 0 || count > 1024) {
    ctx->err = "bad argument";
    return G16_EINVAL;
  }
  CTX_ENTER(ctx);
  int32_t rc;
  CombineRes res;
  g16_combine_pre pre;
  if ((rc = g16_combine_enqueue(ctx, k, partials, count, flags, mask_r, mask_s, &res, nullptr, &pre))) return rc;
  HIPCHK(ctx, hipStreamSynchronize(ctx->stream));
  g16_combine_finish(&pre, &res, out);
  return G16_OK;
}

extern "C" int32_t g16_prove(g16_ctx* ctx, const g16_pkey* k, const void* witness, uint32_t flags, const void* mask_r,
                             const void* mask_s, g16_proof* out) {
  if (!ctx) return G16_EINVAL;
  if (!k || !witness || !out || k->device != ctx->device) {
    ctx->err = "bad argument";
    return G16_EINVAL;
  }
  if (k->shard_count != 1) {
    ctx->err = "g16_prove needs an unsharded key; use g16_prove_partials + g16_prove_combine";
    return G16_EINVAL;
  }
  CTX_ENTER(ctx);
  int32_t rc;
  if ((rc = ensure_stage_o(ctx))) return rc;
  if ((rc = ensure(ctx, ctx->stage_s, PART_BYTES))) return rc;
  unsigned char* d_part = (unsigned char*)ctx->stage_s.p();
  if ((rc = g16_prove_partials(ctx, k, witness, flags | G16_OUT_DEVICE | G16_NO_HOST_SYNC, d_part))) return rc;
  rc = g16_prove_combine(ctx, k, d_part, 1, G16_SCALARS_DEVICE, mask_r, mask_s, out);
  if (rc != G16_OK) ctx_quiesce(ctx);
  return rc;
}

extern "C" int32_t g16_quotient(g16_ctx* ctx, const void* Az, const void* Bz, const void* Cz, uint32_t log2n,
                                uint32_t flavour, void* out) {
  if (!ctx) return G16_EINVAL;
  if (!Az || !Bz || !Cz || !out || log2n > 27 || flavour > 1) {
    ctx->err = "bad argument";
    return G16_EINVAL;
  }
  CTX_ENTER(ctx);
  const size_t n = size_t(1) << log2n;
  int32_t rc;
  if ((rc = ensure(ctx, ctx->prove, 4 * n * 32))) return rc;
  u256* d = (u256*)ctx->prove.p();
  HIPCHK(ctx, hipMemcpyAsync(d, Az, n * 32, hipMemcpyHostToDevice, ctx->stream));
  HIPCHK(ctx, hipMemcpyAsync(d + n, Bz, n * 32, hipMemcpyHostToDevice, ctx->stream));
  HIPCHK(ctx, hipMemcpyAsync(d + 2 * n, Cz, n * 32, hipMemcpyHostToDevice, ctx->stream));
  if ((rc = g16_quotient_device(ctx, d, d + n, d + 2 * n, log2n, (int)flavour, d + 3 * n))) return rc;
  HIPCHK(ctx, hipMemcpyAsync(out, d + 3 * n, n * 32, hipMemcpyDeviceToHost, ctx->stream));
  HIPCHK(ctx, hipStreamSynchronize(ctx->stream));
  return G16_OK;
}
extern "C" int32_t g16_quotient_dev(g16_ctx* ctx, const void* d_Az, const void* d_Bz, const void* d_Cz, uint32_t log2n,
                                    uint32_t flavour, void* d_out) {
  if (!ctx) return G16_EINVAL;
  if (!d_Az || !d_Bz || !d_Cz || !d_out || log2n > 27 || flavour > 1) {
    ctx->err = "bad argument";
    return G16_EINVAL;
  }
  CTX_ENTER(ctx);
  return g16_quotient_device(ctx, d_Az, d_Bz, d_Cz, log2n, (int)flavour, d_out);
}
```

Measured before the change: 136.5 proofs/s.

## Derive C-vector coset evaluation from A and B when key rows differ rarely

At key creation the code compares the A and B coefficient rows and records up to eight rows where they differ, which covers squaring-chain circuits. When that holds, the quotient runs a two-vector coset NTT instead of three. It rebuilds B on the coset from A plus a small correction using a precomputed inverse table u, and takes the difference from Az−Bz at those rows. This removes one of the three batched NTTs, and with it their memory traffic, per proof. In exchange it adds an n-sized u table, a per-element loop over the differing rows, and host-side sorting at key creation.

```diff
diff --git a/include/g16hip.h b/include/g16hip.h
--- a/include/g16hip.h
+++ b/include/g16hip.h
@@ -115,6 +115,10 @@
                      void* out);
 int32_t g16_quotient_dev(g16_ctx* ctx, const void* d_Az, const void* d_Bz, const void* d_Cz, uint32_t log2n,
                          uint32_t flavour, void* d_out);
+int32_t g16_quotient_rows(g16_ctx* ctx, const void* Az, const void* Bz, const uint32_t* rows, size_t nrows,
+                          uint32_t log2n, uint32_t flavour, void* out);
+int32_t g16_quotient_rows_dev(g16_ctx* ctx, const void* d_Az, const void* d_Bz, const uint32_t* rows, size_t nrows,
+                              uint32_t log2n, uint32_t flavour, void* d_out);
 
 typedef struct g16_pkey g16_pkey;
 typedef struct {
@@ -153,6 +157,7 @@
 int32_t g16_pkey_inf_counts(const g16_pkey* key, size_t out[8]);
 int32_t g16_pkey_b1_fold(const g16_pkey* key, size_t out[3]);
 int32_t g16_pkey_b1_sparse(const g16_pkey* key, size_t out[3]);
+int32_t g16_pkey_quotient_rows(const g16_pkey* key, size_t out[10]);
 int32_t g16_prove(g16_ctx* ctx, const g16_pkey* key, const void* witness, uint32_t flags, const void* mask_r,
                   const void* mask_s, g16_proof* out);
 #define G16_PARTIALS_BYTES 768
diff --git a/nim_groth16_amd/_lib.py b/nim_groth16_amd/_lib.py
--- a/nim_groth16_amd/_lib.py
+++ b/nim_groth16_amd/_lib.py
@@ -33,6 +33,7 @@
     "g16_setup_log2_domain", "g16_fake_setup", "g16_lagrange_fr", "g16_powers_fr",
     "g16_points_audit_g1", "g16_points_audit_g2", "g16_points_pairs_check", "g16_key_audit",
     "g16_pkey_b1_fold", "g16_pkey_b1_sparse", "g16_circuit_audit",
+    "g16_pkey_quotient_rows", "g16_quotient_rows", "g16_quotient_rows_dev",
     "g16_points_intt_g1", "g16_points_intt_g2", "g16_circuit_setup",
     "g16_points_scale_g1", "g16_points_scale_g2", "g16_points_scale_each_g1", "g16_points_scale_each_g2",
     "g16_key_contribute", "g16_contributions_verify", "g16_ptau_contribute", "g16_ptau_verify",
@@ -458,6 +459,7 @@
     lib.g16_points_inf_count.restype = sz
     lib.g16_pkey_inf_counts.argtypes = [vp, ctypes.POINTER(sz)]
     lib.g16_pkey_b1_fold.argtypes = [vp, ctypes.POINTER(sz)]
+    lib.g16_pkey_quotient_rows.argtypes = [vp, ctypes.POINTER(sz)]
     lib.g16_pkey_b1_sparse.argtypes = [vp, ctypes.POINTER(sz)]
     lib.g16_points_info.argtypes = [vp, ctypes.POINTER(u32), ctypes.POINTER(u32)]
     lib.g16_msm_points.argtypes = [vp, vp, vp, u32, vp]
@@ -467,6 +469,8 @@
     lib.g16_fixed_base_g2.argtypes = [vp, vp, u32, sz, vp]
     lib.g16_quotient.argtypes = [vp, vp, vp, vp, u32, u32, vp]
     lib.g16_quotient_dev.argtypes = [vp, vp, vp, vp, u32, u32, vp]
+    lib.g16_quotient_rows.argtypes = [vp, vp, vp, ctypes.POINTER(u32), sz, u32, u32, vp]
+    lib.g16_quotient_rows_dev.argtypes = [vp, vp, vp, ctypes.POINTER(u32), sz, u32, u32, vp]
     lib.g16_pkey_create.argtypes = [vp, ctypes.POINTER(PkeyDesc), ctypes.POINTER(vp)]
     lib.g16_pkey_create_zkey.argtypes = [vp, ctypes.POINTER(PkeyDesc), vp, sz, ctypes.POINTER(vp)]
     lib.g16_pkey_destroy.argtypes = [vp]
@@ -935,6 +939,15 @@
         self._check(self._lib.g16_quotient(self._h, _buf(Az), _buf(Bz), _buf(Cz), log2n, flavour, res))
         return res.raw
 
+    def quotient_rows(self, Az, Bz, rows, log2n: int, flavour: int, out=None, device: bool = False):
+        arr = (ctypes.c_uint32 * max(1, len(rows)))(*rows)
+        if device:
+            self._check(self._lib.g16_quotient_rows_dev(self._h, _buf(Az), _buf(Bz), arr, len(rows), log2n, flavour, _buf(out)))
+            return None
+        res = ctypes.create_string_buffer(32 << log2n)
+        self._check(self._lib.g16_quotient_rows(self._h, _buf(Az), _buf(Bz), arr, len(rows), log2n, flavour, res))
+        return res.raw
+
     def sum_partials(self, group: int, xyzz: bytes, count: int) -> bytes:
         psz = 64 if group == 1 else 128
         out = ctypes.create_string_buffer(psz)
@@ -1060,6 +1073,11 @@
         self.ctx._check(self.ctx._lib.g16_pkey_b1_fold(self._h, out))
         return {"form": ("PLAIN", "EMPTY", "DELTA")[out[0]], "live_b1": out[1], "live_delta": out[2]}
 
+    def quotient_rows(self) -> dict:
+        out = (ctypes.c_size_t * 10)()
+        self.ctx._check(self.ctx._lib.g16_pkey_quotient_rows(self._h, out))
+        return {"form": ("PLAIN", "ROWS")[out[0]], "ndiff": out[1], "rows": list(out[2: 2 + min(out[1], 8)])}
+
     def b1_sparse(self) -> dict:
         out = (ctypes.c_size_t * 3)()
         self.ctx._check(self.ctx._lib.g16_pkey_b1_sparse(self._h, out))
diff --git a/nim_groth16_amd/csrc/coeff_rows.hpp b/nim_groth16_amd/csrc/coeff_rows.hpp
--- /dev/null
+++ b/nim_groth16_amd/csrc/coeff_rows.hpp
@@ -0,0 +1,45 @@
+#pragma once
+#include <stddef.h>
+#include <stdint.h>
+#include <string.h>
+
+#include <algorithm>
+#include <vector>
+
+namespace g16 {
+
+inline std::vector<uint32_t> quotient_differing_rows(const uint32_t* vrow, const unsigned char* cols, size_t col_stride,
+                                                     const unsigned char* vals, size_t val_stride, size_t count, size_t n,
+                                                     size_t limit) {
+  std::vector<uint32_t> rows;
+  std::vector<size_t> start(2 * n + 1, 0);
+  for (size_t e = 0; e < count; ++e) ++start[(size_t)vrow[e] + 1];
+  for (size_t i = 0; i < 2 * n; ++i) start[i + 1] += start[i];
+  std::vector<size_t> order(count), fill(start.begin(), start.end() - 1);
+  for (size_t e = 0; e < count; ++e) order[fill[vrow[e]]++] = e;
+  auto wire = [&](size_t e) {
+    uint32_t w;
+    memcpy(&w, cols + e * col_stride, 4);
+    return w;
+  };
+  auto before = [&](size_t x, size_t y) {
+    const uint32_t wx = wire(x), wy = wire(y);
+    return wx != wy ? wx < wy : memcmp(vals + x * val_stride, vals + y * val_stride, 32) < 0;
+  };
+  for (size_t r = 0; r < n && rows.size() <= limit; ++r) {
+    const size_t a0 = start[2 * r], b0 = start[2 * r + 1], b1 = start[2 * r + 2];
+    bool equal = b0 - a0 == b1 - b0;
+    if (equal && b0 != a0) {
+      std::sort(order.begin() + a0, order.begin() + b0, before);
+      std::sort(order.begin() + b0, order.begin() + b1, before);
+      for (size_t i = 0; i < b0 - a0 && equal; ++i) {
+        const size_t x = order[a0 + i], y = order[b0 + i];
+        equal = wire(x) == wire(y) && memcmp(vals + x * val_stride, vals + y * val_stride, 32) == 0;
+      }
+    }
+    if (!equal) rows.push_back((uint32_t)r);
+  }
+  return rows;
+}
+
+}
diff --git a/nim_groth16_amd/csrc/g16_env.hpp b/nim_groth16_amd/csrc/g16_env.hpp
--- a/nim_groth16_amd/csrc/g16_env.hpp
+++ b/nim_groth16_amd/csrc/g16_env.hpp
@@ -24,4 +24,5 @@
   int abc_dict = 1;
   int g2_first = -1;
   int b1_fold = 1;
+  int quot_rows = 1;
 };
diff --git a/nim_groth16_amd/csrc/g16_internal.hpp b/nim_groth16_amd/csrc/g16_internal.hpp
--- a/nim_groth16_amd/csrc/g16_internal.hpp
+++ b/nim_groth16_amd/csrc/g16_internal.hpp
@@ -61,6 +61,8 @@
   Buf ntt_tw;
   Buf ntt_tmp;
   Buf coset[2];
+  Buf quot_u;
+  Buf quot_rows;
   Buf quot;
   Buf prove;
   Buf fb_table[2];
@@ -69,6 +71,7 @@
   const void* shard_begun = nullptr;
   uint32_t tw_log2n = 0xffffffffu;
   uint32_t coset_log2n[2] = {0xffffffffu, 0xffffffffu};
+  uint32_t quot_u_log2n = 0xffffffffu;
   bool profiling = false;
   bool prof_accum_only = false;
   std::vector<ProfEntry> prof;
@@ -270,7 +273,8 @@
                         bool need_cz = true);
 int32_t g16_ntt_device(g16_ctx* ctx, const void* d_src, void* d_dst, uint32_t log2n, int inverse);
 int32_t g16_quotient_device(g16_ctx* ctx, const void* d_a, const void* d_b, const void* d_c, uint32_t log2n,
-                            int flavour, void* d_out, int c_from_ab = 0);
+                            int flavour, void* d_out, int c_from_ab = 0, const uint32_t* d_rows = nullptr,
+                            int nrows = -1);
 int32_t g16_coset_pipeline_device(g16_ctx* ctx, const void* d_in, uint32_t log2n, void* d_out);
 int32_t g16_abc_pointwise_device(g16_ctx* ctx, const void* d_a, const void* d_b, const void* d_c, size_t count,
                                  void* d_out);
diff --git a/nim_groth16_amd/csrc/g16hip.hip b/nim_groth16_amd/csrc/g16hip.hip
--- a/nim_groth16_amd/csrc/g16hip.hip
+++ b/nim_groth16_amd/csrc/g16hip.hip
@@ -29,6 +29,7 @@
   if (const char* v = getenv("G16_TAIL_QUAD")) e.tail_quad = v[0] != '0';
   if (const char* v = getenv("G16_G2_FIRST")) e.g2_first = v[0] == '2' ? 2 : v[0] != '0';
   if (const char* v = getenv("G16_B1_FOLD")) e.b1_fold = v[0] != '0';
+  if (const char* v = getenv("G16_QUOT_ROWS")) e.quot_rows = v[0] != '0';
   if (const char* v = getenv("G16_MTAB")) e.mtab = v[0] == '1' ? 1 : 2;
   if (const char* v = getenv("G16_NTT_TILE")) e.ntt_tile = atoi(v) == 1024 ? 1024 : atoi(v) == 4096 ? 4096 : 2048;
   if (const char* v = getenv("G16_MSM_SORT")) e.msm_sort = v[0];
diff --git a/nim_groth16_amd/csrc/ntt.cuh b/nim_groth16_amd/csrc/ntt.cuh
--- a/nim_groth16_amd/csrc/ntt.cuh
+++ b/nim_groth16_amd/csrc/ntt.cuh
@@ -118,6 +118,7 @@
                                                       const u256* __restrict__ scale, int mul_src) {
   extern __shared__ __align__(16) unsigned char smem[];
   u256* lds = reinterpret_cast<u256*>(smem);
+  const u256* const x0 = x;
   x += xstride * blockIdx.y;
   y += ystride * blockIdx.y;
   const uint32_t R = 1u << rho, B = 1u << log2b;
@@ -128,9 +129,9 @@
 
   u256* twl = lds + tile;
   for (uint32_t t = tid; t < (R >> 1); t += BLOCK) twl[t] = ntt_tw(tw, t << (log2n - rho), log2n, inverse);
-  if (mul_src && blockIdx.y == 2) {
-    const u256* xa = x - 2 * xstride;
-    const u256* xb = x - xstride;
+  if (mul_src && blockIdx.y == (uint32_t)mul_src) {
+    const u256* xa = x0;
+    const u256* xb = x0 + (size_t(1) << log2n);
     for (uint32_t e = tid; e < tile; e += BLOCK) {
       uint32_t b = e & (B - 1), r = e >> log2b;
       const size_t gi = (size_t)base0 + b + (size_t)nR * r;
@@ -166,11 +167,13 @@
   }
 }
 
-template <int BLOCK, int TILE>
+template <int BLOCK, int TILE, bool ROWS = false>
 static __global__ void __launch_bounds__(BLOCK) ntt_last_pass_abc(const u256* __restrict__ x, u256* __restrict__ out,
                                                                const u256* __restrict__ tw, uint32_t log2n,
                                                                uint32_t log2s, uint32_t rho, uint32_t log2b,
-                                                               size_t xstride, int mul_invz) {
+                                                               size_t xstride, int mul_invz,
+                                                               const u256* __restrict__ u, const u256* __restrict__ ab,
+                                                               const uint32_t* __restrict__ rows, uint32_t nrows) {
   extern __shared__ __align__(16) unsigned char smem[];
   u256* lds = reinterpret_cast<u256*>(smem);
   constexpr int PER = TILE / BLOCK;
@@ -182,8 +185,9 @@
   u256* twl = lds + tile;
   for (uint32_t t = tid; t < (R >> 1); t += BLOCK) twl[t] = ntt_tw(tw, t << (log2n - rho), log2n, 0);
   u256 acc[PER];
+  const uint32_t s_mask = (1u << log2s) - 1;
 #pragma unroll 1
-  for (int v = 0; v < 3; ++v) {
+  for (int v = 0; v < (ROWS ? 2 : 3); ++v) {
     const u256* xv = x + xstride * v;
     for (uint32_t e = tid; e < tile; e += BLOCK) {
       uint32_t b = e & (B - 1), r = e >> log2b;
@@ -197,12 +201,33 @@
       if (e < tile) {
         uint32_t b = e & (B - 1), q = e >> log2b;
         u256 z = lds[(bitrev(q, rho) << log2b) | b];
-        acc[i] = v == 0 ? z : v == 1 ? Fr::mul(acc[i], z) : Fr::sub(acc[i], z);
-      }
-    }
-    __syncthreads();
-  }
-  const uint32_t s_mask = (1u << log2s) - 1;
+        if (ROWS) acc[i] = v == 0 ? z : Fr::sub(acc[i], z);
+        else acc[i] = v == 0 ? z : v == 1 ? Fr::mul(acc[i], z) : Fr::sub(acc[i], z);
+      }
+    }
+    __syncthreads();
+    if (ROWS && v == 0) {
+      const uint32_t n = 1u << log2n;
+      if (tid < nrows) {
+        const uint32_t k = rows[tid];
+        lds[tid] = Fr::neg(Fr::dbl(Fr::mul(tw[n >> 1], Fr::sub(ab[k], ab[(size_t)n + k]))));
+      }
+      __syncthreads();
+#pragma unroll
+      for (int i = 0; i < PER; ++i) {
+        const uint32_t e = tid + i * BLOCK;
+        if (e < tile) {
+          const uint32_t b = e & (B - 1), q = e >> log2b;
+          const uint32_t base = base0 + b;
+          const uint32_t oi = (base & s_mask) + ((((base >> log2s) << rho) + q) << log2s);
+          u256 b1 = acc[i];
+          for (uint32_t k = 0; k < nrows; ++k) b1 = Fr::sub(b1, Fr::mul(lds[k], u[(oi - rows[k]) & (n - 1)]));
+          acc[i] = Fr::mul(acc[i], b1);
+        }
+      }
+      __syncthreads();
+    }
+  }
 #pragma unroll
   for (int i = 0; i < PER; ++i) {
     const uint32_t e = tid + i * BLOCK;
@@ -218,7 +243,8 @@
   }
 }
 
-static __global__ void __launch_bounds__(256) ntt_make_coset_table(u256* __restrict__ tab, uint32_t log2n, int mode) {
+static __global__ void __launch_bounds__(256) ntt_make_coset_table(u256* __restrict__ tab, uint32_t log2n, int mode,
+                                                                   u256* __restrict__ u) {
   uint32_t i = blockIdx.x * 256 + threadIdx.x;
   const uint32_t n = 1u << log2n;
   if (i >= n) return;
@@ -227,6 +253,7 @@
   u256 eta = ntt_omega(log2n + 1);
   uint32_t e = mode ? (2 * n - i) % (2 * n) : i;
   tab[i] = Fr::mul(fr_pow_u32(eta, e), ninv);
+  if (u) u[i] = Fr::inv(Fr::sub(fr_pow_u32(eta, 2 * i + 1), Fr::one()));
 }
 
 static __global__ void __launch_bounds__(256) fr_abc_pointwise(const u256* __restrict__ a, const u256* __restrict__ b,
diff --git a/nim_groth16_amd/csrc/ntt.hip b/nim_groth16_amd/csrc/ntt.hip
--- a/nim_groth16_amd/csrc/ntt.hip
+++ b/nim_groth16_amd/csrc/ntt.hip
@@ -4,6 +4,7 @@
 #include "g16_internal.hpp"
 #include "ntt.cuh"
 #include "ntt_plan.hpp"
+#include "quotient_plan.hpp"
 
 using namespace g16;
 
@@ -43,6 +44,10 @@
                                   hipFuncAttributeMaxDynamicSharedMemorySize, max_shmem));
   HIPCHK(ctx, hipFuncSetAttribute(reinterpret_cast<const void*>(&ntt_last_pass_abc<NTT_BLOCK_MID, NTT_TILE_MID>),
                                   hipFuncAttributeMaxDynamicSharedMemorySize, max_shmem));
+  HIPCHK(ctx, hipFuncSetAttribute(reinterpret_cast<const void*>(&ntt_last_pass_abc<NTT_BLOCK, NTT_TILE, true>),
+                                  hipFuncAttributeMaxDynamicSharedMemorySize, max_shmem));
+  HIPCHK(ctx, hipFuncSetAttribute(reinterpret_cast<const void*>(&ntt_last_pass_abc<NTT_BLOCK_MID, NTT_TILE_MID, true>),
+                                  hipFuncAttributeMaxDynamicSharedMemorySize, max_shmem));
   done.store(true, std::memory_order_release);
   return G16_OK;
 }
@@ -51,16 +56,26 @@
   uint32_t block;
   decltype(&ntt_last_pass_abc<NTT_BLOCK, NTT_TILE>) last_pass_abc;
   decltype(&ntt_pass<NTT_BLOCK>) pass;
+  decltype(&ntt_last_pass_abc<NTT_BLOCK, NTT_TILE, true>) last_pass_rows;
 };
 static const NttKernels ntt_kernels[3] = {
-    {NTT_BLOCK_SMALL, ntt_last_pass_abc<NTT_BLOCK_SMALL, NTT_TILE_SMALL>, ntt_pass<NTT_BLOCK_SMALL>},
-    {NTT_BLOCK_MID, ntt_last_pass_abc<NTT_BLOCK_MID, NTT_TILE_MID>, ntt_pass<NTT_BLOCK_MID>},
-    {NTT_BLOCK, ntt_last_pass_abc<NTT_BLOCK, NTT_TILE>, ntt_pass<NTT_BLOCK>},
+    {NTT_BLOCK_SMALL, ntt_last_pass_abc<NTT_BLOCK_SMALL, NTT_TILE_SMALL>, ntt_pass<NTT_BLOCK_SMALL>,
+     ntt_last_pass_abc<NTT_BLOCK_SMALL, NTT_TILE_SMALL, true>},
+    {NTT_BLOCK_MID, ntt_last_pass_abc<NTT_BLOCK_MID, NTT_TILE_MID>, ntt_pass<NTT_BLOCK_MID>,
+     ntt_last_pass_abc<NTT_BLOCK_MID, NTT_TILE_MID, true>},
+    {NTT_BLOCK, ntt_last_pass_abc<NTT_BLOCK, NTT_TILE>, ntt_pass<NTT_BLOCK>, ntt_last_pass_abc<NTT_BLOCK, NTT_TILE, true>},
+};
+
+struct QuotRows {
+  const u256* u;
+  const u256* ab;
+  const uint32_t* rows;
+  uint32_t nrows;
 };
 
 static int32_t ntt_batched(g16_ctx* ctx, const u256* in, size_t in_stride, u256* out, size_t out_stride,
                            uint32_t batch, uint32_t log2n, int inverse, const u256* scale, int fuse_abc = 0,
-                           int c_from_ab = 0) {
+                           int mul_src = 0, const QuotRows* rows = nullptr) {
   const size_t n = size_t(1) << log2n;
   int32_t rc;
   if ((rc = ensure_twiddles(ctx, log2n))) return rc;
@@ -86,15 +101,21 @@
     const NttPass plan = ntt_pass_plan(geom, log2n, p);
     const bool last = p + 1 == npass;
     if (last && fuse_abc) {
-      KLAUNCH(ctx, "ntt_last_pass_abc", K.last_pass_abc, plan.ntiles, K.block, plan.shmem, src, out,
-              (const u256*)ctx->ntt_tw.p(), log2n, plan.log2s, plan.rho, plan.log2b, src_stride, fuse_abc == 2 ? 1 : 0);
+      if (rows)
+        KLAUNCH(ctx, "ntt_last_pass_abc", K.last_pass_rows, plan.ntiles, K.block, plan.shmem, src, out,
+                (const u256*)ctx->ntt_tw.p(), log2n, plan.log2s, plan.rho, plan.log2b, src_stride, fuse_abc == 2 ? 1 : 0,
+                rows->u, rows->ab, rows->rows, rows->nrows);
+      else
+        KLAUNCH(ctx, "ntt_last_pass_abc", K.last_pass_abc, plan.ntiles, K.block, plan.shmem, src, out,
+                (const u256*)ctx->ntt_tw.p(), log2n, plan.log2s, plan.rho, plan.log2b, src_stride, fuse_abc == 2 ? 1 : 0,
+                (const u256*)nullptr, (const u256*)nullptr, (const uint32_t*)nullptr, 0u);
       break;
     }
     u256* dst = last ? out : ((p & 1) ? tmpB : tmpA);
     const size_t dst_stride = last ? out_stride : n;
     KLAUNCH(ctx, inverse ? "ntt_pass_inv" : "ntt_pass_fwd", K.pass, dim3(plan.ntiles, batch), K.block, plan.shmem, src, dst,
             (const u256*)ctx->ntt_tw.p(), log2n, plan.log2s, plan.rho, plan.log2b, inverse, last ? 1 : 0, src_stride,
-            dst_stride, last ? scale : (const u256*)nullptr, p == 0 ? c_from_ab : 0);
+            dst_stride, last ? scale : (const u256*)nullptr, p == 0 ? mul_src : 0);
     src = dst;
     src_stride = dst_stride;
   }
@@ -113,22 +134,61 @@
   return ntt_batched(ctx, (const u256*)d_src, 0, (u256*)d_dst, 0, 1, log2n, inverse, nullptr);
 }
 
-static int32_t ensure_coset(g16_ctx* ctx, uint32_t log2n, int mode) {
-  if (ctx->coset_log2n[mode] == log2n) return G16_OK;
+static int32_t ensure_coset(g16_ctx* ctx, uint32_t log2n, int mode, bool with_u = false) {
+  if (ctx->coset_log2n[mode] == log2n && (!with_u || ctx->quot_u_log2n == log2n)) return G16_OK;
   const size_t n = size_t(1) << log2n;
   int32_t rc;
   if ((rc = ensure(ctx, ctx->coset[mode], n * 32))) return rc;
+  if (with_u && (rc = ensure(ctx, ctx->quot_u, n * 32))) return rc;
   KLAUNCH(ctx, "ntt_coset_table", ntt_make_coset_table, (uint32_t)((n + 255) / 256), 256, 0,
-          (u256*)ctx->coset[mode].p(), log2n, mode);
+          (u256*)ctx->coset[mode].p(), log2n, mode, with_u ? (u256*)ctx->quot_u.p() : (u256*)nullptr);
   ctx->coset_log2n[mode] = log2n;
+  if (with_u) ctx->quot_u_log2n = log2n;
+  return G16_OK;
+}
+
+static int32_t quotient_rows_device(g16_ctx* ctx, const void* d_a, const void* d_b, const void* d_c, uint32_t log2n,
+                                    int flavour, void* d_out, int c_from_ab, const uint32_t* d_rows, uint32_t nrows) {
+  const size_t n = size_t(1) << log2n;
+  const u256* in = (const u256*)d_a;
+  const bool in_place = (const u256*)d_b == in + n && (c_from_ab || (const u256*)d_c == in + 2 * n);
+  int32_t rc;
+  if ((rc = ensure(ctx, ctx->quot, (in_place ? 4 : 7) * n * 32))) return rc;
+  if ((rc = ensure_coset(ctx, log2n, 0, true))) return rc;
+  u256* X = (u256*)ctx->quot.p();
+  u256* Y = X + 3 * n;
+  if (!in_place) {
+    u256* S = X + 4 * n;
+    HIPCHK(ctx, hipMemcpyAsync(S, d_a, n * 32, hipMemcpyDeviceToDevice, ctx->stream));
+    HIPCHK(ctx, hipMemcpyAsync(S + n, d_b, n * 32, hipMemcpyDeviceToDevice, ctx->stream));
+    if (!c_from_ab) HIPCHK(ctx, hipMemcpyAsync(S + 2 * n, d_c, n * 32, hipMemcpyDeviceToDevice, ctx->stream));
+    in = S;
+  }
+  if ((rc = ntt_batched(ctx, in, 2 * n, X, n, 2, log2n, 1, (const u256*)ctx->coset[0].p(), 0, c_from_ab ? 1 : 0))) return rc;
+  const QuotRows qr{(const u256*)ctx->quot_u.p(), in, d_rows, nrows};
+  if (flavour == 1) {
+    if ((rc = ntt_batched(ctx, X, n, (u256*)d_out, 0, 2, log2n, 0, nullptr, 1, 0, &qr))) return rc;
+  } else {
+    if ((rc = ensure_coset(ctx, log2n, 1))) return rc;
+    if ((rc = ntt_batched(ctx, X, n, Y, 0, 2, log2n, 0, nullptr, 2, 0, &qr))) return rc;
+    if ((rc = ntt_batched(ctx, Y, n, (u256*)d_out, n, 1, log2n, 1, (const u256*)ctx->coset[1].p()))) return rc;
+  }
+  HIPCHK(ctx, hipGetLastError());
   return G16_OK;
 }
 
 int32_t g16_quotient_device(g16_ctx* ctx, const void* d_a, const void* d_b, const void* d_c, uint32_t log2n,
-                            int flavour, void* d_out, int c_from_ab) {
+                            int flavour, void* d_out, int c_from_ab, const uint32_t* d_rows, int nrows) {
   if (log2n > 27) {
     ctx->err = "quotient needs the 2n domain: log2n <= 27";
     return G16_EINVAL;
+  }
+  if (nrows >= 0) {
+    if (log2n == 0 || (size_t)nrows > QUOT_ROWS_MAX || (nrows && !d_rows)) {
+      ctx->err = "quotient on two vectors: log2n >= 1 and at most QUOT_ROWS_MAX rows";
+      return G16_EINVAL;
+    }
+    return quotient_rows_device(ctx, d_a, d_b, d_c, log2n, flavour, d_out, c_from_ab, d_rows, (uint32_t)nrows);
   }
   const size_t n = size_t(1) << log2n;
   int32_t rc;
@@ -152,7 +212,7 @@
       in = (const u256*)ctx->ntt_tmp.p();
     }
   }
-  if ((rc = ntt_batched(ctx, in, n, X, n, 3, log2n, 1, (const u256*)ctx->coset[0].p(), 0, c_from_ab))) return rc;
+  if ((rc = ntt_batched(ctx, in, n, X, n, 3, log2n, 1, (const u256*)ctx->coset[0].p(), 0, c_from_ab ? 2 : 0))) return rc;
   if (flavour == 1) {
     if ((rc = ntt_batched(ctx, X, n, (u256*)d_out, 0, 3, log2n, 0, nullptr, 1))) return rc;
   } else {
diff --git a/nim_groth16_amd/csrc/pkey.hip b/nim_groth16_amd/csrc/pkey.hip
--- a/nim_groth16_amd/csrc/pkey.hip
+++ b/nim_groth16_amd/csrc/pkey.hip
@@ -4,6 +4,7 @@
 
 #include "pkey.hpp"
 #include "b1_fold.cuh"
+#include "coeff_rows.hpp"
 
 using namespace g16;
 
@@ -33,6 +34,14 @@
 extern "C" int32_t g16_pkey_b1_sparse(const g16_pkey* k, size_t out[3]) {
   if (!k || !out) return G16_EINVAL;
   out[0] = k->b1_sparse ? 1 : 0, out[1] = k->b1_nlive, out[2] = B1_SPARSE_MAX;
+  return G16_OK;
+}
+
+extern "C" int32_t g16_pkey_quotient_rows(const g16_pkey* k, size_t out[10]) {
+  static_assert(QUOT_ROWS_MAX == 8, "g16hip.h documents out[10]");
+  if (!k || !out) return G16_EINVAL;
+  out[0] = (size_t)k->quot_form, out[1] = k->quot_ndiff;
+  for (size_t i = 0; i < QUOT_ROWS_MAX; ++i) out[2 + i] = i < k->quot_ndiff ? k->quot_rows[i] : 0;
   return G16_OK;
 }
 
@@ -219,6 +228,29 @@
   return G16_OK;
 }
 
+static int32_t quotient_rows_of_key(g16_ctx* ctx, const g16_pkey_desc* d, const CoeffSource& cs,
+                                    const std::vector<uint32_t>& vrow, g16_pkey* k) {
+  if (!g16_env().quot_rows || d->log2_domain == 0) return G16_OK;
+  std::vector<uint32_t> rows;
+  try {
+    rows = quotient_differing_rows(vrow.data(), cs.count ? cs.base + 8 : nullptr, cs.stride,
+                                   cs.count ? cs.base + cs.value_off : nullptr, cs.stride, cs.count,
+                                   size_t(1) << d->log2_domain, QUOT_ROWS_MAX);
+  } catch (const std::bad_alloc&) {
+    ctx->err = "out of host memory";
+    return G16_ENOMEM;
+  }
+  k->quot_ndiff = (uint32_t)rows.size();
+  k->quot_form = quotient_form(rows.size(), d->log2_domain, g16_env());
+  for (size_t i = 0; i < rows.size() && i < QUOT_ROWS_MAX; ++i) k->quot_rows[i] = rows[i];
+  if (k->quot_form == QUOT_ROWS && !rows.empty()) {
+    HIPCHK(ctx, dev_alloc(k->d_quot_rows, rows.size() * 4));
+    HIPCHK(ctx, hipMemcpyAsync(k->d_quot_rows.get(), k->quot_rows, rows.size() * 4, hipMemcpyHostToDevice, ctx->stream));
+    HIPCHK(ctx, hipStreamSynchronize(ctx->stream));
+  }
+  return G16_OK;
+}
+
 static int32_t bin_coefficients(g16_ctx* ctx, const g16_pkey_desc* d, const CoeffSource& cs, g16_pkey* k) {
   const size_t n = size_t(1) << d->log2_domain;
   std::vector<uint32_t> vrow;
@@ -238,6 +270,7 @@
     vrow[e] = 2 * row + matrix;
   }
   k->ncoeffs = cs.count;
+  if (int32_t rc = quotient_rows_of_key(ctx, d, cs, vrow, k)) return rc;
   return g16_spmat_create(ctx, 2, (uint32_t)n, cs.count, vrow.data(), 4, (const uint32_t*)(cs.count ? cs.base + 8 : nullptr),
                           cs.stride, cs.count ? cs.base + cs.value_off : nullptr, cs.stride, &k->abc, cs.values_r2);
 }
diff --git a/nim_groth16_amd/csrc/pkey.hpp b/nim_groth16_amd/csrc/pkey.hpp
--- a/nim_groth16_amd/csrc/pkey.hpp
+++ b/nim_groth16_amd/csrc/pkey.hpp
@@ -1,6 +1,7 @@
 #pragma once
 #include "g16_internal.hpp"
 #include "ec.cuh"
+#include "quotient_plan.hpp"
 
 struct g16_pkey {
   int device = 0;
@@ -22,4 +23,8 @@
   static constexpr size_t B1_VIEW_WORDS = 16;
   DevMem<uint32_t> b1_sparse;
   uint32_t b1_nlive = 0;
+  int quot_form = g16::QUOT_PLAIN;
+  uint32_t quot_ndiff = 0;
+  uint32_t quot_rows[g16::QUOT_ROWS_MAX] = {};
+  DevMem<uint32_t> d_quot_rows;
 };
diff --git a/nim_groth16_amd/csrc/prover.hip b/nim_groth16_amd/csrc/prover.hip
--- a/nim_groth16_amd/csrc/prover.hip
+++ b/nim_groth16_amd/csrc/prover.hip
@@ -100,7 +100,8 @@
         break;
       case OP_BUILD_ABC: rc = build_abc_device(ctx, k, d_w, wit_mont, d_abc, s.a != 0); break;
       case OP_QUOTIENT:
-        rc = g16_quotient_device(ctx, d_abc, d_abc + n, d_abc + 2 * n, k->log2n, (int)k->flavour, d_qs, s.a);
+        rc = g16_quotient_device(ctx, d_abc, d_abc + n, d_abc + 2 * n, k->log2n, (int)k->flavour, d_qs, s.a,
+                                 k->d_quot_rows.get(), k->quot_form == QUOT_ROWS ? (int)k->quot_ndiff : -1);
         break;
       case OP_COSET: {
         const int at = __builtin_popcount(task_mask & ((1u << s.a) - 1));
@@ -311,3 +312,48 @@
   CTX_ENTER(ctx);
   return g16_quotient_device(ctx, d_Az, d_Bz, d_Cz, log2n, (int)flavour, d_out);
 }
+
+static int32_t quotient_rows_args(g16_ctx* ctx, const void* a, const void* b, const uint32_t* rows, size_t nrows,
+                                  uint32_t log2n, uint32_t flavour, const void* out) {
+  bool ok = a && b && out && (rows || !nrows) && log2n >= 1 && log2n <= 27 && flavour <= 1 && nrows <= QUOT_ROWS_MAX;
+  for (size_t i = 0; ok && i < nrows; ++i) ok = rows[i] < (uint32_t(1) << log2n) && (i == 0 || rows[i - 1] < rows[i]);
+  if (!ok) ctx->err = "bad argument (1 <= log2n <= 27, at most 8 rows, ascending and inside the domain)";
+  return ok ? G16_OK : G16_EINVAL;
+}
+static int32_t upload_quotient_rows(g16_ctx* ctx, const uint32_t* rows, size_t nrows) {
+  int32_t rc;
+  if ((rc = ensure(ctx, ctx->quot_rows, QUOT_ROWS_MAX * 4))) return rc;
+  if (nrows) {
+    HIPCHK(ctx, hipMemcpyAsync(ctx->quot_rows.p(), rows, nrows * 4, hipMemcpyHostToDevice, ctx->stream));
+  }
+  return G16_OK;
+}
+extern "C" int32_t g16_quotient_rows(g16_ctx* ctx, const void* Az, const void* Bz, const uint32_t* rows, size_t nrows,
+                                     uint32_t log2n, uint32_t flavour, void* out) {
+  if (!ctx) return G16_EINVAL;
+  int32_t rc;
+  if ((rc = quotient_rows_args(ctx, Az, Bz, rows, nrows, log2n, flavour, out))) return rc;
+  CTX_ENTER(ctx);
+  const size_t n = size_t(1) << log2n;
+  if ((rc = ensure(ctx, ctx->prove, 4 * n * 32))) return rc;
+  if ((rc = upload_quotient_rows(ctx, rows, nrows))) return rc;
+  u256* d = (u256*)ctx->prove.p();
+  HIPCHK(ctx, hipMemcpyAsync(d, Az, n * 32, hipMemcpyHostToDevice, ctx->stream));
+  HIPCHK(ctx, hipMemcpyAsync(d + n, Bz, n * 32, hipMemcpyHostToDevice, ctx->stream));
+  if ((rc = g16_quotient_device(ctx, d, d + n, d + 2 * n, log2n, (int)flavour, d + 3 * n, 1,
+                                (const uint32_t*)ctx->quot_rows.p(), (int)nrows)))
+    return rc;
+  HIPCHK(ctx, hipMemcpyAsync(out, d + 3 * n, n * 32, hipMemcpyDeviceToHost, ctx->stream));
+  HIPCHK(ctx, hipStreamSynchronize(ctx->stream));
+  return G16_OK;
+}
+extern "C" int32_t g16_quotient_rows_dev(g16_ctx* ctx, const void* d_Az, const void* d_Bz, const uint32_t* rows,
+                                         size_t nrows, uint32_t log2n, uint32_t flavour, void* d_out) {
+  if (!ctx) return G16_EINVAL;
+  int32_t rc;
+  if ((rc = quotient_rows_args(ctx, d_Az, d_Bz, rows, nrows, log2n, flavour, d_out))) return rc;
+  CTX_ENTER(ctx);
+  if ((rc = upload_quotient_rows(ctx, rows, nrows))) return rc;
+  return g16_quotient_device(ctx, d_Az, d_Bz, nullptr, log2n, (int)flavour, d_out, 1, (const uint32_t*)ctx->quot_rows.p(),
+                             (int)nrows);
+}
diff --git a/nim_groth16_amd/csrc/quotient_plan.hpp b/nim_groth16_amd/csrc/quotient_plan.hpp
--- /dev/null
+++ b/nim_groth16_amd/csrc/quotient_plan.hpp
@@ -0,0 +1,16 @@
+#pragma once
+#include <stddef.h>
+#include <stdint.h>
+
+#include "g16_env.hpp"
+
+namespace g16 {
+
+enum QuotForm : int { QUOT_PLAIN = 0, QUOT_ROWS = 1 };
+constexpr size_t QUOT_ROWS_MAX = 8;
+inline QuotForm quotient_form(size_t ndiff, uint32_t log2n, const G16Env& env) {
+  if (!env.quot_rows || log2n == 0) return QUOT_PLAIN;
+  return ndiff <= QUOT_ROWS_MAX ? QUOT_ROWS : QUOT_PLAIN;
+}
+
+}
```

Measured after the change: 140.3 proofs/s, median of 6. 2.8% higher.
